# zhuker/lamejs

Hardware: NVIDIA H100
Metric: encoded audio seconds/sec (44.1kHz stereo 128kbps CBR) (higher is better)
Workload: dtype f64

## Files before the change

include/mp3b200.h:

```cpp
#ifndef MP3B200_H
#define MP3B200_H
#include <stdint.h>

#ifdef __cplusplus
extern "C" {
#endif

#define MP3B200_OK 0
#define MP3B200_ERR_CONFIG (-1)
#define MP3B200_ERR_BUFFER (-1)
#define MP3B200_ERR_HANDLE (-3)
#define MP3B200_ERR_CUDA (-100)

typedef struct mp3b200_encoder mp3b200_encoder;

int mp3b200_set_device(int device);

int mp3b200_create(int channels, int samplerate, int kbps, mp3b200_encoder** out);

#define MP3B200_RESAMPLE 1
int mp3b200_create_ex(int channels, int samplerate, int kbps, int flags, mp3b200_encoder** out);
int mp3b200_out_samplerate(int channels, int samplerate, int kbps);

int mp3b200_encode(mp3b200_encoder* h, const int16_t* left, const int16_t* right, int nsamples, uint8_t* out, int cap);

int mp3b200_flush(mp3b200_encoder* h, uint8_t* out, int cap);

void mp3b200_destroy(mp3b200_encoder* h);

int mp3b200_encode_batch(mp3b200_encoder* const* handles, const int16_t* const* left, const int16_t* const* right,
                         const int* nsamples, uint8_t* const* out, const int* cap, int nstreams, int* out_bytes);
int mp3b200_flush_batch(mp3b200_encoder* const* handles, uint8_t* const* out, const int* cap, int nstreams, int* out_bytes);

int mp3b200_encode_device(mp3b200_encoder* h, const int16_t* d_left, const int16_t* d_right, int nsamples, uint8_t* out, int cap);
int mp3b200_encode_device_f32(mp3b200_encoder* h, const float* d_left, const float* d_right, int nsamples, uint8_t* out, int cap);
int mp3b200_encode_batch_device(mp3b200_encoder* const* handles, const int16_t* const* d_left, const int16_t* const* d_right,
                                const int* nsamples, uint8_t* const* out, const int* cap, int nstreams, int* out_bytes);
int mp3b200_encode_batch_device_f32(mp3b200_encoder* const* handles, const float* const* d_left, const float* const* d_right,
                                    const int* nsamples, uint8_t* const* out, const int* cap, int nstreams, int* out_bytes);
int mp3b200_encoder_device(const mp3b200_encoder* h);

int mp3b200_export_state(mp3b200_encoder* h, void* buf, int cap);
int mp3b200_import_state(mp3b200_encoder* h, const void* buf, int len);
int mp3b200_seek(mp3b200_encoder* h, int64_t frame, const int16_t* left_hist, const int16_t* right_hist, int nhist);


int64_t mp3b200_stream_bytes(int channels, int samplerate, int kbps, int64_t nsamples);
int64_t mp3b200_stream_bytes_ex(int channels, int samplerate, int kbps, int flags, int64_t nsamples);
int64_t mp3b200_stream_frames(int64_t nsamples);
int64_t mp3b200_stream_frames_cfg(int channels, int samplerate, int kbps, int64_t nsamples);
int mp3b200_granules_per_frame(int channels, int samplerate, int kbps);
int64_t mp3b200_stream_frames_ex(int channels, int samplerate, int kbps, int flags, int64_t nsamples);
int mp3b200_granules_per_frame_ex(int channels, int samplerate, int kbps, int flags);

int mp3b200_encode_streams(int channels, int samplerate, int kbps, int nstreams, const int16_t* const* left,
                           const int16_t* const* right, const int64_t* nsamples, uint8_t* const* out,
                           const int64_t* cap, int64_t* out_bytes);
int mp3b200_encode_streams_ex(int channels, int samplerate, int kbps, int flags, int nstreams, const int16_t* const* left,
                              const int16_t* const* right, const int64_t* nsamples, uint8_t* const* out,
                              const int64_t* cap, int64_t* out_bytes);

int mp3b200_encode_streams_device(int channels, int samplerate, int kbps, int nstreams, const int16_t* d_pcm,
                                  const int64_t* pcm_off, const int64_t* nsamples, uint8_t* d_out,
                                  const int64_t* out_off, float* timings_ms);
int mp3b200_encode_streams_device_ex(int channels, int samplerate, int kbps, int flags, int nstreams, const int16_t* d_pcm,
                                     const int64_t* pcm_off, const int64_t* nsamples, uint8_t* d_out,
                                     const int64_t* out_off, float* timings_ms);

int mp3b200_set_write_vbr_tag(mp3b200_encoder* h, int on);
int mp3b200_get_lametag_frame(mp3b200_encoder* h, uint8_t* buf, int cap);
int mp3b200_music_crc(mp3b200_encoder* h);
int64_t mp3b200_bytes_written(mp3b200_encoder* h);
int mp3b200_lametag_size(int channels, int samplerate, int kbps);
int mp3b200_lametag_size_ex(int channels, int samplerate, int kbps, int flags);
int mp3b200_lametag_build(int channels, int samplerate, int kbps, int64_t nframes, int64_t music_bytes, int music_crc,
                          int encoder_padding, uint8_t* buf, int cap);
int mp3b200_encode_streams_tagged(int channels, int samplerate, int kbps, int nstreams, const int16_t* const* left,
                                  const int16_t* const* right, const int64_t* nsamples, uint8_t* const* out,
                                  const int64_t* cap, int64_t* out_bytes);

#define MP3B200_REPLAYGAIN 2
int mp3b200_encode_streams_tagged_ex(int channels, int samplerate, int kbps, int flags, int nstreams, const int16_t* const* left,
                                     const int16_t* const* right, const int64_t* nsamples, uint8_t* const* out,
                                     const int64_t* cap, int64_t* out_bytes, double* title_db, double* album_db);
int mp3b200_encode_streams_tagged_device(int channels, int samplerate, int kbps, int flags, int nstreams, const int16_t* d_pcm,
                                         const int64_t* pcm_off, const int64_t* nsamples, uint8_t* d_out, const int64_t* out_off,
                                         int64_t* out_bytes, double* title_db, double* album_db);
int mp3b200_encode_streams_tagged_device_f32(int channels, int samplerate, int kbps, int flags, int nstreams, const float* d_pcm,
                                             const int64_t* pcm_off, const int64_t* nsamples, uint8_t* d_out, const int64_t* out_off,
                                             int64_t* out_bytes, double* title_db, double* album_db);
int mp3b200_set_find_replay_gain(mp3b200_encoder* h, int on);
int mp3b200_get_replay_gain(mp3b200_encoder* h, double* title_db, int* radio_gain);
int mp3b200_album_gain(mp3b200_encoder* const* handles, int n, double* album_db);
int mp3b200_lametag_build_ex(int channels, int samplerate, int kbps, int flags, int64_t nframes, int64_t music_bytes, int music_crc,
                             int encoder_padding, int radio_gain, uint8_t* buf, int cap);
int mp3b200_replaygain_streams(int channels, int samplerate, int kbps, int flags, int nstreams, const int16_t* const* left,
                               const int16_t* const* right, const int64_t* nsamples, double* title_db, double* album_db);
int mp3b200_replaygain_streams_f32(int channels, int samplerate, int kbps, int flags, int nstreams, const float* const* left,
                                   const float* const* right, const int64_t* nsamples, double* title_db, double* album_db);
int mp3b200_replaygain_streams_device(int channels, int samplerate, int kbps, int flags, int nstreams, const int16_t* d_pcm,
                                      const int64_t* pcm_off, const int64_t* nsamples, double* title_db, double* album_db);
int mp3b200_replaygain_streams_device_f32(int channels, int samplerate, int kbps, int flags, int nstreams, const float* d_pcm,
                                          const int64_t* pcm_off, const int64_t* nsamples, double* title_db, double* album_db);
int mp3b200_finish_tags_device(int channels, int samplerate, int kbps, int flags, int nstreams, uint8_t* d_files,
                               const int64_t* file_off, const int64_t* nsamples, const double* title_db, int64_t* file_bytes);
int mp3b200_debug_replaygain(int channels, int samplerate, int kbps, int flags, const int16_t* left, const int16_t* right,
                             int64_t nsamples, double* win_sums, int32_t* win_idx, int64_t nwin_cap, int32_t* hist,
                             double* title_db, int32_t* stats);

typedef struct mp3b200_vbr_tag_data {
  int32_t h_id, samprate, flags, frames, bytes, vbr_scale, headersize, enc_delay, enc_padding;
  uint8_t toc[100];
} mp3b200_vbr_tag_data;
int mp3b200_put_vbr_tag(mp3b200_encoder* h, uint8_t* stream, int64_t len);
int mp3b200_get_vbr_tag(const uint8_t* frame, int64_t len, mp3b200_vbr_tag_data* out);
int mp3b200_crc16_combine(int crc_a, int crc_b, int64_t len_b);

#define MP3B200_ID3_ADD_V2 2
#define MP3B200_ID3_V1_ONLY 4
#define MP3B200_ID3_V2_ONLY 8
#define MP3B200_ID3_SPACE_V1 16
#define MP3B200_ID3_PAD_V2 32
typedef struct mp3b200_id3tag {
  const char *title, *artist, *album, *year, *comment, *track, *genre;
  int flags, padding;
  int64_t num_samples;
  int samplerate;
} mp3b200_id3tag;
int mp3b200_id3v2_tag(const mp3b200_id3tag* t, uint8_t* buf, int cap);
int mp3b200_id3v1_tag(const mp3b200_id3tag* t, uint8_t* buf, int cap);
const char* mp3b200_id3_genre_name(int index);

int mp3b200_debug_music_crc(const uint8_t* d_buf, const int64_t* off, const int64_t* len, int nranges, uint32_t* crc, float* ms);

typedef struct mp3b200_wav_header { int64_t data_offset, data_len; int32_t channels; uint32_t sample_rate; } mp3b200_wav_header;
int mp3b200_wav_read_header(const uint8_t* data, int64_t len, mp3b200_wav_header* out);

int mp3b200_debug_stages(int channels, int samplerate, int kbps, const int16_t* left, const int16_t* right,
                         int64_t nsamples, const int32_t* force_blocktype, float* xr, int32_t* blocktype,
                         float* en_l, float* thm_l, float* en_s, float* thm_s, double* ath_adjust,
                         int32_t* l3_enc, int32_t* ginfo, uint8_t* bytes_out, int64_t bytes_cap);

typedef struct mp3b200_debug_taps {
  int32_t size, channels, samplerate, kbps;
  const int16_t *left, *right;
  int64_t nsamples;
  const int32_t* force_blocktype;
  float* xr; int32_t* blocktype; float *en_l, *thm_l, *en_s, *thm_s; double* ath_adjust;
  int32_t *l3_enc, *ginfo; uint8_t* bytes_out; int64_t bytes_cap;
  int32_t *scalefac, *subblock_gain; float* xmin; int32_t* max_nonzero_coeff; double* xrpow_max;
  int32_t *scfsi, *old_value, *cur_step;
  int32_t flags;
} mp3b200_debug_taps;
int mp3b200_debug_stages_ex(const mp3b200_debug_taps* t);

int mp3b200_debug_resample(int channels, int samplerate, int kbps, const int16_t* left, const int16_t* right, int64_t nsamples,
                           float* y, int64_t ny);

int mp3b200_encode_f32(mp3b200_encoder* h, const float* left, const float* right, int nsamples, uint8_t* out, int cap);
int mp3b200_encode_batch_f32(mp3b200_encoder* const* handles, const float* const* left, const float* const* right,
                             const int* nsamples, uint8_t* const* out, const int* cap, int nstreams, int* out_bytes);
int mp3b200_seek_f32(mp3b200_encoder* h, int64_t frame, const float* left_hist, const float* right_hist, int nhist);
int mp3b200_encode_streams_f32(int channels, int samplerate, int kbps, int flags, int nstreams, const float* const* left,
                               const float* const* right, const int64_t* nsamples, uint8_t* const* out,
                               const int64_t* cap, int64_t* out_bytes);
int mp3b200_encode_streams_tagged_f32(int channels, int samplerate, int kbps, int flags, int nstreams, const float* const* left,
                                      const float* const* right, const int64_t* nsamples, uint8_t* const* out,
                                      const int64_t* cap, int64_t* out_bytes, double* title_db, double* album_db);
int mp3b200_encode_streams_device_f32(int channels, int samplerate, int kbps, int flags, int nstreams, const float* d_pcm,
                                      const int64_t* pcm_off, const int64_t* nsamples, uint8_t* d_out,
                                      const int64_t* out_off, float* timings_ms);
int mp3b200_debug_stages_f32(const mp3b200_debug_taps* t, const float* left, const float* right);
int mp3b200_debug_resample_f32(int channels, int samplerate, int kbps, const float* left, const float* right, int64_t nsamples,
                               float* y, int64_t ny);
int mp3b200_debug_replaygain_f32(int channels, int samplerate, int kbps, int flags, const float* left, const float* right,
                                 int64_t nsamples, double* win_sums, int32_t* win_idx, int64_t nwin_cap, int32_t* hist,
                                 double* title_db, int32_t* stats);

#define MP3B200_SESSION_SLOTS 4
typedef struct mp3b200_session mp3b200_session;
int mp3b200_session_create(void* cuda_stream, mp3b200_session** out);
int mp3b200_session_destroy(mp3b200_session* s);
int mp3b200_encode_streams_async(mp3b200_session* s, int channels, int samplerate, int kbps, int flags, int nstreams,
                                 const int16_t* d_pcm, const int64_t* pcm_off, const int64_t* nsamples, uint8_t* d_out,
                                 const int64_t* out_off, int32_t* d_status);
int mp3b200_encode_streams_async_f32(mp3b200_session* s, int channels, int samplerate, int kbps, int flags, int nstreams,
                                     const float* d_pcm, const int64_t* pcm_off, const int64_t* nsamples, uint8_t* d_out,
                                     const int64_t* out_off, int32_t* d_status);
int mp3b200_check_status(const int32_t* status);

int mp3b200_encode_streams_tagged_async(mp3b200_session* s, int channels, int samplerate, int kbps, int flags, int nstreams,
                                        const int16_t* d_pcm, const int64_t* pcm_off, const int64_t* nsamples, uint8_t* d_out,
                                        const int64_t* out_off, int64_t* out_bytes, double* d_gain, int32_t* d_status);
int mp3b200_encode_streams_tagged_async_f32(mp3b200_session* s, int channels, int samplerate, int kbps, int flags, int nstreams,
                                            const float* d_pcm, const int64_t* pcm_off, const int64_t* nsamples, uint8_t* d_out,
                                            const int64_t* out_off, int64_t* out_bytes, double* d_gain, int32_t* d_status);

int mp3b200_session_encode_batch(mp3b200_session* s, mp3b200_encoder* const* handles, const int16_t* const* d_left,
                                 const int16_t* const* d_right, const int* nsamples, int n, uint8_t* d_out, const int64_t* out_off,
                                 int* out_bytes, int32_t* d_status);
int mp3b200_session_encode_batch_f32(mp3b200_session* s, mp3b200_encoder* const* handles, const float* const* d_left,
                                     const float* const* d_right, const int* nsamples, int n, uint8_t* d_out, const int64_t* out_off,
                                     int* out_bytes, int32_t* d_status);
int mp3b200_session_flush_batch(mp3b200_session* s, mp3b200_encoder* const* handles, int n, uint8_t* d_out, const int64_t* out_off,
                                int* out_bytes, int32_t* d_status);
int mp3b200_encode_bytes(const mp3b200_encoder* h, int nsamples);
int mp3b200_encode_bytes_schedule(int channels, int samplerate, int kbps, int flags, int write_vbr_tag, const int* nsamples, int n,
                                  int* out_bytes);
int mp3b200_session_release(mp3b200_session* s, mp3b200_encoder* const* handles, int n);
int64_t mp3b200_session_tail_capacity(int channels, int samplerate, int kbps, int flags);

int mp3b200_session_encode_batch_tagged(mp3b200_session* s, mp3b200_encoder* const* handles, const int16_t* const* d_left,
                                        const int16_t* const* d_right, const int* nsamples, int n, uint8_t* d_out, const int64_t* out_off,
                                        int* out_bytes, int32_t* d_status);
int mp3b200_session_encode_batch_tagged_f32(mp3b200_session* s, mp3b200_encoder* const* handles, const float* const* d_left,
                                            const float* const* d_right, const int* nsamples, int n, uint8_t* d_out,
                                            const int64_t* out_off, int* out_bytes, int32_t* d_status);
int mp3b200_session_flush_batch_tagged(mp3b200_session* s, mp3b200_encoder* const* handles, int n, uint8_t* d_out,
                                       const int64_t* out_off, int* out_bytes, int32_t* d_status);
int mp3b200_session_lametag_frames(mp3b200_session* s, mp3b200_encoder* const* handles, int n, uint8_t* d_out, const int64_t* out_off,
                                   int* out_bytes, int32_t* d_status);
int mp3b200_session_album_gain(mp3b200_session* s, mp3b200_encoder* const* handles, int n, double* d_album, int32_t* d_status);
int64_t mp3b200_session_graph_instantiations(mp3b200_session* s);

const char* mp3b200_last_error(void);
int64_t mp3b200_launch_count(void);

#ifdef __cplusplus
}
#endif
#endif
```

lamejs_b200/__init__.py:

```python
from .encoder import Mp3Encoder, WavHeader, id3v1_tag, id3v2_tag, ID3_ADD_V2, ID3_V1_ONLY, ID3_V2_ONLY, ID3_SPACE_V1, ID3_PAD_V2, lametag_size, lametag_build, get_vbr_tag, crc16_combine, encode_streams_tagged, debug_music_crc, encode_batch, flush_batch, encode_streams, encode_streams_device, encode_streams_device_tagged, debug_stages, debug_resample, lib, stream_bytes, stream_frames, granules_per_frame, out_samplerate, RESAMPLE, Mp3B200Error
from .encoder import REPLAYGAIN, GAIN_NOT_ENOUGH_SAMPLES, radio_gain, lametag_build_ex, debug_replaygain, encode_streams_replaygain, album_gain
from .encoder import DOMAIN_SITES, debug_domain_hits
from .encoder import EncodeSession, check_status
from .encoder import replay_gain_streams, replay_gain_streams_device, finish_tags_device
```

lamejs_b200/csrc/k_psy.cuh:

```cuda
#ifndef MP3B200_K_PSY_CUH
#define MP3B200_K_PSY_CUH
#include "mp3_device.cuh"
#include "mp3_tables.h"

#ifndef PSY_THREADS
#define PSY_THREADS 128
#endif
#define MASK_THREADS 128

struct PsyUnit {
  double ecb_s[3][MP3_CBANDS];
  float eb_s[3][MP3_CBANDS];
  float eb_l[MP3_CBANDS];
  float peaks[9];
  float loudness;
  unsigned char mask_idx[MP3_CBANDS];
  unsigned char attack[4];
  unsigned char pad_;
};
struct PsyRatioDev { float en_l[22], thm_l[22], en_s[13][3], thm_s[13][3]; };

__constant__ unsigned char c_fft_rv[128];
__device__ double c_tab[9];
__device__ double c_table1[25];
__device__ double c_table2[10];
__device__ double c_table3[14];
__constant__ double c_fircoef[10];

static int psy_upload_constants() {
  static const double tab[9] = {1.0, 0.79433, 0.63096, 0.63096, 0.63096, 0.63096, 0.63096, 0.25119, 0.11749};
  static const double r1[25] = {3.3246, 3.23837, 3.15437, 3.00412, 2.86103, 2.65407, 2.46209, 2.284, 2.11879, 1.96552, 1.82335,
    1.69146, 1.56911, 1.46658, 1.37074, 1.31036, 1.25264, 1.20648, 1.16203, 1.12765, 1.09428, 1.0659, 1.03826, 1.01895, 1};
  static const double r2[10] = {1.33352, 1.35879, 1.38454, 1.39497, 1.40548, 1.3537, 1.30382, 1.22321, 1.14758, 1};
  static const double r3[14] = {2.35364, 2.29259, 2.23313, 2.12675, 2.02545, 1.87894, 1.74303, 1.61695, 1.49999, 1.39148,
    1.29083, 1.19746, 1.11084, 1.03826};
  static const double fir_half[10] = {-8.65163e-18, -0.00851586, -6.74764e-18, 0.0209036, -3.36639e-17, -0.0438162,
    -1.54175e-17, 0.0931738, -5.52212e-17, -0.313819};
  double t1[25], t2[10], t3[14], fir[10];
  for (int i = 0; i < 25; i++) t1[i] = r1[i] * r1[i];
  for (int i = 0; i < 10; i++) t2[i] = r2[i] * r2[i];
  for (int i = 0; i < 14; i++) t3[i] = r3[i] * r3[i];
  for (int i = 0; i < 10; i++) fir[i] = fir_half[i] * 2;
  if (cudaMemcpyToSymbol(c_fft_rv, MP3_FFT_RV, 128) != cudaSuccess) return -100;
  if (cudaMemcpyToSymbol(c_tab, tab, sizeof tab) != cudaSuccess) return -100;
  if (cudaMemcpyToSymbol(c_table1, t1, sizeof t1) != cudaSuccess) return -100;
  if (cudaMemcpyToSymbol(c_table2, t2, sizeof t2) != cudaSuccess) return -100;
  if (cudaMemcpyToSymbol(c_table3, t3, sizeof t3) != cudaSuccess) return -100;
  if (cudaMemcpyToSymbol(c_fircoef, fir, sizeof fir) != cudaSuccess) return -100;
  return 0;
}

struct f32w {
  float v;
  __device__ __forceinline__ operator double() const {
#ifdef PSY_ALU_WIDEN
    const unsigned u = __float_as_uint(v);
    const unsigned hi = (u & 0x7fffffffu) ? ((u & 0x80000000u) | (((u >> 3) & 0x0fffffffu) + 0x38000000u)) : u;
    return __hiloint2double((int)hi, (int)(u << 29));
#else
    return (double)v;
  }
  __device__ __forceinline__ f32w& operator=(double d) { v = (float)d; return *this; }
};
#endif

#define FHT_PAD(i) ((i) + ((i) >> 4))
__device__ __forceinline__ void fht_task(f32w* fz, int stage, int task, const double* __restrict__ tw, const int* tw_off) {
  const int k1 = 4 << (2 * stage);
  const int kx = k1 >> 1, k2 = k1 << 1, k3 = k2 + k1, k4 = k2 << 1;
  const int g = task >> (2 * stage + 1), i = task & (kx - 1);
  if (i == 0) {
    {
      const int fi = g * k4;
      double f0, f1, f2, f3;
      f1 = fz[FHT_PAD(fi + 0)] - fz[FHT_PAD(fi + k1)];
      f0 = fz[FHT_PAD(fi + 0)] + fz[FHT_PAD(fi + k1)];
      f3 = fz[FHT_PAD(fi + k2)] - fz[FHT_PAD(fi + k3)];
      f2 = fz[FHT_PAD(fi + k2)] + fz[FHT_PAD(fi + k3)];
      fz[FHT_PAD(fi + k2)] = f0 - f2;
      fz[FHT_PAD(fi + 0)] = f0 + f2;
      fz[FHT_PAD(fi + k3)] = f1 - f3;
      fz[FHT_PAD(fi + k1)] = f1 + f3;
    }
    {
      const int gi = g * k4 + kx;
      double f0, f1, f2, f3;
      f1 = fz[FHT_PAD(gi + 0)] - fz[FHT_PAD(gi + k1)];
      f0 = fz[FHT_PAD(gi + 0)] + fz[FHT_PAD(gi + k1)];
      f3 = (SQRT2_D * fz[FHT_PAD(gi + k3)]);
      f2 = (SQRT2_D * fz[FHT_PAD(gi + k2)]);
      fz[FHT_PAD(gi + k2)] = f0 - f2;
      fz[FHT_PAD(gi + 0)] = f0 + f2;
      fz[FHT_PAD(gi + k3)] = f1 - f3;
      fz[FHT_PAD(gi + k1)] = f1 + f3;
    }
    return;
  }
  const double* e = tw + 4 * (tw_off[stage] + i);
  const double c1 = e[0], s1 = e[1], c2 = e[2], s2 = e[3];
  const int fi = g * k4 + i, gi = g * k4 + k1 - i;
  double a, b, g0, f0, f1, g1, f2, g2, f3, g3;
  b = s2 * fz[FHT_PAD(fi + k1)] - c2 * fz[FHT_PAD(gi + k1)];
  a = c2 * fz[FHT_PAD(fi + k1)] + s2 * fz[FHT_PAD(gi + k1)];
  f1 = fz[FHT_PAD(fi + 0)] - a;
  f0 = fz[FHT_PAD(fi + 0)] + a;
  g1 = fz[FHT_PAD(gi + 0)] - b;
  g0 = fz[FHT_PAD(gi + 0)] + b;
  b = s2 * fz[FHT_PAD(fi + k3)] - c2 * fz[FHT_PAD(gi + k3)];
  a = c2 * fz[FHT_PAD(fi + k3)] + s2 * fz[FHT_PAD(gi + k3)];
  f3 = fz[FHT_PAD(fi + k2)] - a;
  f2 = fz[FHT_PAD(fi + k2)] + a;
  g3 = fz[FHT_PAD(gi + k2)] - b;
  g2 = fz[FHT_PAD(gi + k2)] + b;
  b = s1 * f2 - c1 * g3;
  a = c1 * f2 + s1 * g3;
  fz[FHT_PAD(fi + k2)] = f0 - a;
  fz[FHT_PAD(fi + 0)] = f0 + a;
  fz[FHT_PAD(gi + k3)] = g1 - b;
  fz[FHT_PAD(gi + k1)] = g1 + b;
  b = c1 * g2 - s1 * f3;
  a = s1 * g2 + c1 * f3;
  fz[FHT_PAD(gi + k2)] = g0 - a;
  fz[FHT_PAD(gi + 0)] = g0 + a;
  fz[FHT_PAD(fi + k3)] = f1 - b;
  fz[FHT_PAD(fi + k1)] = f1 + b;
}

__device__ __forceinline__ size_t psy_row(const StreamDesc& sd, int z, int u) { return (size_t)sd.unit_base + z + u + 1; }

#ifndef PSY_MIN_BLOCKS
#define PSY_MIN_BLOCKS 12
#endif
template <bool F32_PCM>
__global__ void __launch_bounds__(PSY_THREADS, PSY_MIN_BLOCKS)
k_psy_analysis(const Mp3Tables* __restrict__ T, const StreamDesc* __restrict__ streams, PsyUnit* __restrict__ out,
               int chunk, int nchunks, int u_base) {
  const int z = blockIdx.z;
  const StreamDesc& sd = streams[z];
  const int u = (int)blockIdx.x + u_base;
  if (u >= T->mode_gr * sd.nframes) return;
  const int ch = blockIdx.y;
  const int nch = T->nch;
  const long long c = (long long)T->mode_gr * sd.frame0 + u;
  if (nchunks > 1) {
    const long long n = sd.pcm_end - sd.pcm_base;
    long long last = 576 * c - 224 + 1023 - sd.pcm_base;
    if (last > n - 1) last = n - 1;
    int mine = 0;
    while (mine < nchunks - 1 && last >= n * (mine + 1) / nchunks) mine++;
    if (mine != chunk) return;
  }
  PsyUnit* o = out + psy_row(sd, z, u) * nch + ch;
  const int tid = threadIdx.x;

  if (c < 0) {
    for (int i = tid; i < 3 * MP3_CBANDS; i += PSY_THREADS) { (&o->ecb_s[0][0])[i] = 1.0; (&o->eb_s[0][0])[i] = 0.0f; }
    if (tid < MP3_CBANDS) { o->eb_l[tid] = 0.0f; o->mask_idx[tid] = 0; }
    if (tid < 9) o->peaks[tid] = 10.0f;
    if (tid == 0) o->loudness = 0.0f;
    if (tid < 4) o->attack[tid] = 0;
    return;
  }

  __shared__ __align__(16) unsigned char s_u[sizeof(double) * 1024];
  double* const xs = reinterpret_cast<double*>(s_u);
  f32s* const fe = reinterpret_cast<f32s*>(s_u);
  f32s (*const fes)[129] = reinterpret_cast<f32s (*)[129]>(s_u + 2064);
  f32s* const s_max = reinterpret_cast<f32s*>(s_u + 2064 + 1552);
  f32s* const s_avg = s_max + MP3_CBANDS;
  f32s (*const s_ebs)[MP3_CBANDS] = reinterpret_cast<f32s (*)[MP3_CBANDS]>(s_avg + MP3_CBANDS);
  static_assert(2064 + 1552 + 2 * 4 * MP3_CBANDS + 3 * 4 * MP3_CBANDS <= (int)sizeof(s_u), "energies must fit the PCM span");
  constexpr int PROD_HI_OFF = 2064 + 1552 + 2 * 4 * MP3_CBANDS + 3 * 4 * MP3_CBANDS;
  static_assert(PROD_HI_OFF % 8 == 0 && PROD_HI_OFF + 256 * 8 <= (int)sizeof(s_u), "second half of the loudness terms");
  double* const prod_hi = reinterpret_cast<double*>(s_u + PROD_HI_OFF);
  __shared__ f32w wl[1024 + 64];
  __shared__ f32w wsh[3][256 + 16];
  __shared__ __align__(8) f32s hp[576];
  double* const prod_lo = reinterpret_cast<double*>(hp);
  static_assert(sizeof(f32s) * 576 >= 256 * 8, "first half of the loudness terms");
  __shared__ int s_peak[9];
  if (tid < 9) s_peak[tid] = __float_as_int(1.0f);

  const int scale_applied = T->scale_applied;
  const double scale = T->scale;
  const long long x0 = 576 * c - 224;
  {
    using Sample = pcm_sample_t<F32_PCM>;
    const Sample* __restrict__ pbuf = static_cast<const Sample*>(sd.pcm[ch]);
    const long long pbase = sd.pcm_base, pend = sd.pcm_end;
    constexpr int NB = (1024 + PSY_THREADS - 1) / PSY_THREADS;
    Sample v[NB];
#pragma unroll
    for (int k = 0; k < NB; k++) {
      const int j = tid + k * PSY_THREADS;
      const long long i = x0 + j;
      v[k] = (j < 1024 && i >= 0 && i < pend) ? __ldg(&pbuf[i - pbase]) : (Sample)0;
    }
#pragma unroll
    for (int k = 0; k < NB; k++) {
      const int j = tid + k * PSY_THREADS;
      if (j < 1024) xs[j] = pcm_value(v[k], scale_applied, scale);
    }
  }
  __syncthreads();

  for (int i = tid; i < 576; i += PSY_THREADS) {
    const double* fb = xs + 397 + i;
    double sum1 = fb[10], sum2 = 0.0;
#pragma unroll
    for (int j = 0; j < 9; j += 2) {
      sum1 += c_fircoef[j] * (fb[j] + fb[21 - j]);
      sum2 += c_fircoef[j + 1] * (fb[j + 1] + fb[21 - j - 1]);
    }
    hp[i] = sum1 + sum2;
  }
  for (int vt = tid; vt < 128 + 96; vt += PSY_THREADS) {
  if (vt < 128) {
    const int jj = vt, i = c_fft_rv[jj], x = 4 * jj;
    const float* w = T->fft_window;
    double f0, f1, f2, f3, wv;
    f0 = (double)w[i] * (double)xs[i];
    wv = (double)w[i + 0x200] * (double)xs[i + 0x200];
    f1 = f0 - wv; f0 = f0 + wv;
    f2 = (double)w[i + 0x100] * (double)xs[i + 0x100];
    wv = (double)w[i + 0x300] * (double)xs[i + 0x300];
    f3 = f2 - wv; f2 = f2 + wv;
    wl[FHT_PAD(x + 0)] = f0 + f2; wl[FHT_PAD(x + 2)] = f0 - f2; wl[FHT_PAD(x + 1)] = f1 + f3; wl[FHT_PAD(x + 3)] = f1 - f3;
    f0 = (double)w[i + 0x001] * (double)xs[i + 0x001];
    wv = (double)w[i + 0x201] * (double)xs[i + 0x201];
    f1 = f0 - wv; f0 = f0 + wv;
    f2 = (double)w[i + 0x101] * (double)xs[i + 0x101];
    wv = (double)w[i + 0x301] * (double)xs[i + 0x301];
    f3 = f2 - wv; f2 = f2 + wv;
    wl[FHT_PAD(x + 512 + 0)] = f0 + f2; wl[FHT_PAD(x + 512 + 2)] = f0 - f2; wl[FHT_PAD(x + 512 + 1)] = f1 + f3; wl[FHT_PAD(x + 512 + 3)] = f1 - f3;
  } else {
    const int q = vt - 128, b = q >> 5, j = q & 31;
    const int i = c_fft_rv[j << 2], x = 4 * j, k = 192 * (b + 1);
    const float* w = T->fft_window_s;
    const double* bx = xs + i + k;
    double f0, f1, f2, f3, wv;
    f0 = (double)w[i] * (double)bx[0];
    wv = (double)w[0x7f - i] * (double)bx[0x80];
    f1 = f0 - wv; f0 = f0 + wv;
    f2 = (double)w[i + 0x40] * (double)bx[0x40];
    wv = (double)w[0x3f - i] * (double)bx[0xc0];
    f3 = f2 - wv; f2 = f2 + wv;
    wsh[b][FHT_PAD(x + 0)] = f0 + f2; wsh[b][FHT_PAD(x + 2)] = f0 - f2; wsh[b][FHT_PAD(x + 1)] = f1 + f3; wsh[b][FHT_PAD(x + 3)] = f1 - f3;
    f0 = (double)w[i + 0x01] * (double)bx[0x01];
    wv = (double)w[0x7e - i] * (double)bx[0x81];
    f1 = f0 - wv; f0 = f0 + wv;
    f2 = (double)w[i + 0x41] * (double)bx[0x41];
    wv = (double)w[0x3e - i] * (double)bx[0xc1];
    f3 = f2 - wv; f2 = f2 + wv;
    wsh[b][FHT_PAD(x + 128 + 0)] = f0 + f2; wsh[b][FHT_PAD(x + 128 + 2)] = f0 - f2; wsh[b][FHT_PAD(x + 128 + 1)] = f1 + f3; wsh[b][FHT_PAD(x + 128 + 3)] = f1 - f3;
  }
  }
  __syncthreads();

  for (int i = tid; i < 576; i += PSY_THREADS) atomicMax(&s_peak[i >> 6], __float_as_int(fabsf(hp[i].v)));
#pragma unroll
  for (int stage = 0; stage < 4; stage++) {
    const int nt = 128 + (stage < 3 ? 96 : 0);
    for (int t = tid; t < nt; t += PSY_THREADS) {
      if (t < 128) fht_task(wl, stage, t, T->tw, T->tw_off);
      else fht_task(wsh[(t - 128) >> 5], stage, (t - 128) & 31, T->tw, T->tw_off);
    }
    __syncthreads();
  }

  for (int j = tid; j < 512; j += PSY_THREADS) {
    const double re = wl[FHT_PAD(512 - j)], im = wl[FHT_PAD(512 + j)];
    f32s e; e = (re * re + im * im) * 0.5;
    fe[512 - j] = (double)e;
    const int k = 512 - j;
    if (k < 512) { const double p = (double)e * (double)T->eql_w[k]; if (k < 256) prod_lo[k] = p; else prod_hi[k - 256] = p; }
  }
  if (tid == 0) { f32s t0; t0 = (double)wl[0]; t0 *= (double)t0; fe[0] = (double)t0; prod_lo[0] = (double)t0 * (double)T->eql_w[0]; }
  for (int t = tid; t < 3 * 128; t += PSY_THREADS) {
    const int b = t >> 7, j = t & 127;
    const double re = wsh[b][FHT_PAD(128 - j)], im = wsh[b][FHT_PAD(128 + j)];
    fes[b][128 - j] = (re * re + im * im) * 0.5;
  }
  if (tid < 3) { f32s t0; t0 = (double)wsh[tid][0]; t0 *= (double)t0; fes[tid][0] = (double)t0; }
  __syncthreads();

  const int npl = T->npart_l, nps = T->npart_s;
  for (int vt = tid; vt < 256; vt += PSY_THREADS) {
  if (vt < npl) {
    double ebb = 0, m = 0;
    const int l0 = T->line0_l[vt], l1 = T->line0_l[vt + 1];
    for (int j = l0; j < l1; j++) { const double el = fe[j]; ebb += el; if (m < el) m = el; }
    o->eb_l[vt] = (float)ebb;
    s_max[vt] = m;
    s_avg[vt] = ebb * (double)T->rnumlines_l[vt];
  } else if (vt >= 64 && vt < 64 + 3 * 64) {
    const int q = vt - 64, sb = q >> 6, b = q & 63;
    if (b < nps) {
      double ebb = 0;
      const int l0 = T->line0_s[b], l1 = T->line0_s[b + 1];
      for (int j = l0; j < l1; j++) ebb += (double)fes[sb][j];
      s_ebs[sb][b] = ebb;
      o->eb_s[sb][b] = (float)ebb;
    }
  }
  }
  double loud = 0.0;
  if (tid == PSY_THREADS - 1) {
#pragma unroll 8
    for (int i = 0; i < 256; ++i) loud += prod_lo[i];
  }
  if (tid < 9) o->peaks[tid] = __int_as_float(s_peak[tid]);
  __syncthreads();

  for (int vt = tid; vt < 256; vt += PSY_THREADS) {
  if (vt < npl) {
    const int b = vt;
    const int lo = b > 0 ? b - 1 : b, hi = b < npl - 1 ? b + 1 : b;
    double a = 0; double m = 0; int lines = 0;
    for (int q = lo; q <= hi; q++) {
      if (q == lo) { a = (double)s_avg[q]; m = (double)s_max[q]; }
      else { a = a + (double)s_avg[q]; if (m < (double)s_max[q]) m = (double)s_max[q]; }
      lines += T->numlines_l[q];
    }
    int k = 0;
    if (a > 0.0) {
      const double cnt = (double)(hi - lo + 1);
      a = 20.0 * (m * cnt - a) / (a * (lines - 1));
      k = js_trunc<DOM_TRUNC_MASK_IDX>(a);
      if (k > 8) k = 8;
    }
    o->mask_idx[b] = (unsigned char)k;
  } else if (vt >= 64 && vt < 64 + 3 * 64) {
    const int q = vt - 64, sb = q >> 6, b = q & 63;
    if (b < nps) {
      int kk = T->s3lo_s[b];
      int j = T->s3off_s[b];
      double ecb = (double)T->s3_ss[j++] * (double)s_ebs[sb][kk];
      ++kk;
      while (kk <= T->s3hi_s[b]) { ecb += (double)T->s3_ss[j] * (double)s_ebs[sb][kk]; ++j; ++kk; }
      o->ecb_s[sb][b] = ecb;
    }
  }
  }
  if (tid == PSY_THREADS - 1) {
#pragma unroll 8
    for (int i = 0; i < 256; ++i) loud += prod_hi[i];
    loud *= (1. / (14752. * 14752.) / 512);
    o->loudness = (float)loud;
  }
}

struct ScanIn { unsigned attack4; float loudness; };

__global__ void k_attack_prepass(const Mp3Tables* __restrict__ T, const StreamDesc* __restrict__ streams, PsyUnit* __restrict__ psy,
                                 ScanIn* __restrict__ sin) {
  const int z = blockIdx.z;
  const StreamDesc& sd = streams[z];
  const int u = blockIdx.x * blockDim.x + threadIdx.x;
  if (u >= T->mode_gr * sd.nframes) return;
  const int nch = T->nch;
  const double thr = T->attack_threshold;
  for (int ch = 0; ch < nch; ch++) {
    PsyUnit* cur = psy + psy_row(sd, z, u) * nch + ch;
    const PsyUnit* prev = psy + psy_row(sd, z, u - 1) * nch + ch;
    f32s en_subshort[12], attack_intensity[12];
    double en_short[4] = {0, 0, 0, 0};
    int a[4] = {0, 0, 0, 0};
    for (int i = 0; i < 3; i++) {
      en_subshort[i] = (double)prev->peaks[i + 6];
      attack_intensity[i] = (double)en_subshort[i] / (double)prev->peaks[i + 4];
      en_short[0] += (double)en_subshort[i];
    }
    for (int i = 0; i < 9; i++) {
      double p = (double)cur->peaks[i];
      en_subshort[i + 3] = p;
      if (i % 3 == 0) en_short[1 + i / 3] += p;
      if (p > (double)en_subshort[i + 3 - 2]) p = p / (double)en_subshort[i + 3 - 2];
      else if ((double)en_subshort[i + 3 - 2] > p * 10.0) p = (double)en_subshort[i + 3 - 2] / (p * 10.0);
      else p = 0.0;
      attack_intensity[i + 3] = p;
    }
    for (int i = 0; i < 12; i += 3)
      if ((double)attack_intensity[i] > thr) a[i / 3] = 1;
    for (int i = 1; i < 4; i++) {
      double ratio;
      if (en_short[i - 1] > en_short[i]) ratio = en_short[i - 1] / en_short[i];
      else ratio = en_short[i] / en_short[i - 1];
      if (ratio < 1.7) { a[i] = 0; if (i == 1) a[0] = 0; }
    }
    for (int i = 0; i < 4; i++) cur->attack[i] = (unsigned char)a[i];
    ScanIn si;
    si.attack4 = (unsigned)a[0] | ((unsigned)a[1] << 8) | ((unsigned)a[2] << 16) | ((unsigned)a[3] << 24);
    si.loudness = cur->loudness;
    sin[psy_row(sd, z, u) * nch + ch] = si;
    if (u == 0) { si.attack4 = 0; si.loudness = prev->loudness; sin[psy_row(sd, z, -1) * nch + ch] = si; }
  }
}

#define SCAN_FRAMES 16
#define SCAN_THREADS 1024
#ifndef SCAN_GUESS_LA
#define SCAN_GUESS_LA 0
#endif
#ifndef SCAN_GUESS_BT
#define SCAN_GUESS_BT BT_NORM
#endif
#ifndef SCAN_GUESS_ATH
#define SCAN_GUESS_ATH 1.0
#endif
struct ScanChunk { int fsm_in, fsm_out, dirty_fsm, dirty_ath; double ath_in[2], ath_out[2]; };

__device__ __forceinline__ int fsm_pack(int la0, int la1, int o0, int o1) { return la0 | (la1 << 2) | (o0 << 4) | (o1 << 6); }

__device__ void scan_fsm_chunk(const Mp3Tables* T, const StreamDesc& sd, int z, const ScanIn* sin, signed char* bt_final,
                               signed char* bt_prev, int f0, int f1, ScanChunk* ck) {
  const int nch = T->nch, coupled = T->coupled_short_blocks;
  int la[2] = {ck->fsm_in & 3, (ck->fsm_in >> 2) & 3};
  int old[2] = {(ck->fsm_in >> 4) & 3, (ck->fsm_in >> 6) & 3};
  const int G = T->mode_gr;
  for (int u = G * f0; u < G * f1; u++) {
    int uselong[2] = {1, 1};
    for (int ch = 0; ch < nch; ch++) {
      const unsigned av = sin[psy_row(sd, z, u) * nch + ch].attack4;
      int a0 = av & 0xff, a1 = (av >> 8) & 0xff, a2 = (av >> 16) & 0xff, a3 = (av >> 24) & 0xff;
      if (a0 != 0 && la[ch] != 0) a0 = 0;
      if (la[ch] == 3 || (a0 + a1 + a2 + a3) != 0) {
        uselong[ch] = 0;
        if (a1 != 0 && a0 != 0) a1 = 0;
        if (a2 != 0 && a1 != 0) a2 = 0;
        if (a3 != 0 && a2 != 0) a3 = 0;
      }
      la[ch] = a2;
    }
    if (coupled && !(uselong[0] != 0 && uselong[1] != 0)) uselong[0] = uselong[1] = 0;
    const size_t row = (size_t)(sd.unit_base + u) * 2;
    for (int ch = 0; ch < nch; ch++) {
      bt_prev[row + ch] = (signed char)old[ch];
      int bt = BT_NORM;
      if (uselong[ch] != 0) {
        if (old[ch] == BT_SHORT) bt = BT_STOP;
      } else {
        bt = BT_SHORT;
        if (old[ch] == BT_NORM) old[ch] = BT_START;
        if (old[ch] == BT_STOP) old[ch] = BT_SHORT;
      }
      bt_final[row + ch] = (signed char)old[ch];
      old[ch] = bt;
    }
  }
  ck->fsm_out = fsm_pack(la[0], la[1], old[0], old[1]);
}

__device__ void scan_ath_chunk(const Mp3Tables* T, const StreamDesc& sd, int z, const ScanIn* sin, double* ath_psy,
                               double* ath_q, int f0, int f1, ScanChunk* ck) {
  const int nch = T->nch;
  double adjust = ck->ath_in[0], limit = ck->ath_in[1];
  const double sens = T->aa_sensitivity_p;
  const int G = T->mode_gr;
  for (int f = f0; f < f1; f++) {
    ath_psy[sd.frame_base + f] = adjust;
    const ScanIn* r0 = sin + psy_row(sd, z, G * f - 1) * nch;
    double max_pow = (double)r0[0].loudness;
    if (nch == 2) max_pow += (double)r0[1].loudness;
    else max_pow += max_pow;
    if (G == 2) {
      const ScanIn* r1 = sin + psy_row(sd, z, G * f) * nch;
      double gr2_max = (double)r1[0].loudness;
      if (nch == 2) gr2_max += (double)r1[1].loudness;
      else gr2_max += gr2_max;
      max_pow = js_dmax(max_pow, gr2_max);
    }
    max_pow *= 0.5;
    max_pow *= sens;
    if (max_pow > 0.03125) {
      if (adjust >= 1.0) adjust = 1.0;
      else if (adjust < limit) adjust = limit;
      limit = 1.0;
    } else {
      const double adj_lim_new = 31.98 * max_pow + 0.000625;
      if (adjust >= adj_lim_new) {
        adjust *= adj_lim_new * 0.075 + 0.925;
        if (adjust < adj_lim_new) adjust = adj_lim_new;
      } else {
        if (limit >= adj_lim_new) adjust = adj_lim_new;
        else if (adjust < limit) adjust = limit;
      }
      limit = adj_lim_new;
    }
    ath_q[sd.frame_base + f] = adjust;
  }
  ck->ath_out[0] = adjust; ck->ath_out[1] = limit;
}

__global__ void __launch_bounds__(SCAN_THREADS)
k_stream_scan(const Mp3Tables* __restrict__ T, StreamDesc* __restrict__ streams, int nstreams,
              const ScanIn* __restrict__ sin, signed char* __restrict__ bt_final,
              signed char* __restrict__ bt_prev, double* __restrict__ ath_psy, double* __restrict__ ath_q,
              ScanChunk* __restrict__ scratch) {
  asm volatile("griddepcontrol.launch_dependents;" ::: "memory");
  const int z = blockIdx.x;
  if (z >= nstreams) return;
  const StreamDesc& sd = streams[z];
  const int nchunks = (sd.nframes + SCAN_FRAMES - 1) / SCAN_FRAMES;
  ScanChunk* ck = scratch + sd.scan_base;
  const int tid = threadIdx.x;
  for (int c = tid; c < nchunks; c += SCAN_THREADS) {
    ck[c].fsm_in = c == 0 ? fsm_pack(sd.last_attacks[0], sd.last_attacks[1], sd.blocktype_old[0], sd.blocktype_old[1])
                          : fsm_pack(SCAN_GUESS_LA, SCAN_GUESS_LA, SCAN_GUESS_BT, SCAN_GUESS_BT);
    ck[c].ath_in[0] = c == 0 ? sd.ath_adjust : SCAN_GUESS_ATH;
    ck[c].ath_in[1] = c == 0 ? sd.ath_adjust_limit : SCAN_GUESS_ATH;
    ck[c].dirty_fsm = ck[c].dirty_ath = 1;
  }
  for (;;) {
    for (int c = tid; c < nchunks; c += SCAN_THREADS) {
      const int f0 = c * SCAN_FRAMES, f1 = min(sd.nframes, f0 + SCAN_FRAMES);
      if (ck[c].dirty_fsm) scan_fsm_chunk(T, sd, z, sin, bt_final, bt_prev, f0, f1, &ck[c]);
      if (ck[c].dirty_ath) scan_ath_chunk(T, sd, z, sin, ath_psy, ath_q, f0, f1, &ck[c]);
    }
    __syncthreads();
    int any = 0;
    for (int c = tid; c < nchunks; c += SCAN_THREADS) {
      ck[c].dirty_fsm = ck[c].dirty_ath = 0;
      if (c == 0) continue;
      if (ck[c].fsm_in != ck[c - 1].fsm_out) { ck[c].fsm_in = ck[c - 1].fsm_out; ck[c].dirty_fsm = 1; any = 1; }
      if (ck[c].ath_in[0] != ck[c - 1].ath_out[0] || ck[c].ath_in[1] != ck[c - 1].ath_out[1]) {
        ck[c].ath_in[0] = ck[c - 1].ath_out[0]; ck[c].ath_in[1] = ck[c - 1].ath_out[1]; ck[c].dirty_ath = 1; any = 1;
      }
    }
    if (!__syncthreads_or(any)) break;
  }
  if (tid == 0 && nchunks > 0) {
    const ScanChunk& l = ck[nchunks - 1];
    streams[z].last_attacks[0] = l.fsm_out & 3; streams[z].last_attacks[1] = (l.fsm_out >> 2) & 3;
    streams[z].blocktype_old[0] = (l.fsm_out >> 4) & 3; streams[z].blocktype_old[1] = (l.fsm_out >> 6) & 3;
    streams[z].ath_adjust = l.ath_out[0]; streams[z].ath_adjust_limit = l.ath_out[1];
  }
}

__device__ __noinline__ double psy_log10(double x) { return m3_log10(x); }
__device__ __forceinline__ int log10_times16_trunc(const Mp3Tables* T, double ratio) {
  if (!T->l16_ok) return js_trunc<DOM_TRUNC_LOG16>(psy_log10(ratio) * 16.0);
  DOMAIN_MISS(DOM_LOG16_TABLE, !(ratio >= 1.0 && ratio < 31.622776601683793));
  int i = 0;
#pragma unroll
  for (int k = 1; k <= 24; k++) i += ratio >= T->l16_thr[k] ? 1 : 0;
  return i;
}

__device__ __forceinline__ double mask_add_dev(double m1, double m2, int kk, int b, const Mp3Tables* T, double ath_adjust) {
  double ratio;
  if (m2 > m1) {
    if (m2 < (m1 * T->ma_max_i2)) ratio = m2 / m1;
    else return (m1 + m2);
  } else {
    if (m1 >= (m2 * T->ma_max_i2)) return (m1 + m2);
    ratio = m1 / m2;
  }
  m1 += m2;
  if ((b + 3) <= 3 + 3) {
    if (ratio >= T->ma_max_i1) return m1;
    const int i = log10_times16_trunc(T, ratio);
    return m1 * c_table2[i];
  }
  const int i = log10_times16_trunc(T, ratio);
  m2 = (double)T->ath_cb_l[kk] * ath_adjust;
  if (m1 < T->ma_max_m * m2) {
    if (m1 > m2) {
      double f = 1.0, r;
      if (i <= 13) f = c_table3[i];
      r = psy_log10(m1 / m2) * (10.0 / 15.0);
      return m1 * ((c_table1[i] - f) * r + f);
    }
    if (i > 13) return m1;
    return m1 * c_table3[i];
  }
  return m1 * c_table1[i];
}

__global__ void __launch_bounds__(MASK_THREADS)
k_psy_masking(const Mp3Tables* __restrict__ T, const StreamDesc* __restrict__ streams, const PsyUnit* __restrict__ psy,
              const signed char* __restrict__ bt_prev, const double* __restrict__ ath_psy, PsyRatioDev* __restrict__ ratio) {
  const int z = blockIdx.z;
  const StreamDesc& sd = streams[z];
  const int u = (int)blockIdx.x - 1;
  if (u >= T->mode_gr * sd.nframes) return;
  const int nch = T->nch;
  const long long c = (long long)T->mode_gr * sd.frame0 + u;
  const int tid = threadIdx.x, ch = tid >> 6, b = tid & 63;
  PsyRatioDev* out = ratio + psy_row(sd, z, u) * nch;
  if (u < 0) {
    if (c < 0) {
      const float big = (float)1e20;
      for (int i = tid; i < nch * 122; i += MASK_THREADS) (&out[0].en_l[0])[i] = big;
    }
    else if (sd.halo_in) {
      for (int i = tid; i < nch * 122; i += MASK_THREADS) (&out[0].en_l[0])[i] = sd.halo_in[i];
    }
    return;
  }
  __shared__ f32s s_thr[2][MP3_CBANDS + 2], s_eb[2][MP3_CBANDS + 2];
  __shared__ f32s s_thr_s[2][3][MP3_CBANDS + 2];
  __shared__ PsyRatioDev s_out[2];
  const int npl = T->npart_l, nps = T->npart_s;
  const PsyUnit* pu = (ch < nch) ? psy + psy_row(sd, z, u) * nch + ch : nullptr;
  const PsyUnit* pp = (ch < nch) ? psy + psy_row(sd, z, u - 1) * nch + ch : nullptr;
  const double ath_adjust = ath_psy[sd.frame_base + u / T->mode_gr];

  if (ch < nch) {
    if (b < npl) {
      int kk = T->s3lo_l[b];
      int k = T->s3off_l[b];
      double eb2 = (double)pu->eb_l[kk] * c_tab[pu->mask_idx[kk]];
      double ecb = (double)T->s3_ll[k++] * eb2;
      while (++kk <= T->s3hi_l[b]) {
        eb2 = (double)pu->eb_l[kk] * c_tab[pu->mask_idx[kk]];
        ecb = mask_add_dev(ecb, (double)T->s3_ll[k++] * eb2, kk, kk - b, T, ath_adjust);
      }
      ecb *= 0.158489319246111;
      s_thr[ch][b] = ecb;
      s_eb[ch][b] = (double)pu->eb_l[b];
    } else { s_thr[ch][b] = 0.0; s_eb[ch][b] = 0.0; }
    const int prev_short = bt_prev[(size_t)(sd.unit_base + u) * 2 + ch] == BT_SHORT;
    for (int sb = 0; sb < 3; sb++) {
      if (b < nps) {
        const double ecb = pu->ecb_s[sb][b];
        const float nb1 = sb >= 1 ? (float)pu->ecb_s[sb - 1][b] : (float)pp->ecb_s[2][b];
        const float nb2 = sb == 2 ? (float)pu->ecb_s[0][b] : (sb == 1 ? (float)pp->ecb_s[2][b] : (float)pp->ecb_s[1][b]);
        f32s t;
        t = js_dmin(ecb, 2 * (double)nb1);
        if (prev_short) { const double x = 16 * (double)nb2, y = (double)t; t = js_dmin(x, y); }
        s_thr_s[ch][sb][b] = (double)t;
      } else s_thr_s[ch][sb][b] = 0.0;
    }
  }
  __syncthreads();

  if (ch < nch && b < 22) {
    const int sbi = b;
    f32s* en = reinterpret_cast<f32s*>(s_out[ch].en_l);
    f32s* thm = reinterpret_cast<f32s*>(s_out[ch].thm_l);
    const int init = T->conv_l.init[sbi];
    if (init == -2) { en[sbi] = 0.0; thm[sbi] = 0.0; }
    else {
      double enn = 0.0, thmm = 0.0;
      if (init >= 0) {
        const double w_next = 1.0 - (double)T->bo_l_weight[sbi - 1];
        enn = w_next * (double)s_eb[ch][init];
        thmm = w_next * (double)s_thr[ch][init];
      }
      const int p1 = T->conv_l.end[sbi];
      for (int p = T->conv_l.start[sbi]; p < p1; p++) { enn += (double)s_eb[ch][p]; thmm += (double)s_thr[ch][p]; }
      en[sbi] = enn; thm[sbi] = thmm;
      const int bd = T->conv_l.bound[sbi];
      if (bd >= 0) {
        const double w_curr = (double)T->bo_l_weight[sbi];
        en[sbi] += w_curr * (double)s_eb[ch][bd];
        thm[sbi] += w_curr * (double)s_thr[ch][bd];
      }
    }
  } else if (ch < nch && b >= 22 && b < 22 + 39) {
    const int q = b - 22, sbi = q / 3, sblock = q - 3 * sbi;
    f32s(*en)[3] = reinterpret_cast<f32s(*)[3]>(s_out[ch].en_s);
    f32s(*thm)[3] = reinterpret_cast<f32s(*)[3]>(s_out[ch].thm_s);
    const int init = T->conv_s.init[sbi];
    if (init == -2) { en[sbi][sblock] = 0.0; thm[sbi][sblock] = 0.0; }
    else {
      double enn = 0.0, thmm = 0.0;
      if (init >= 0) {
        const double w_next = 1.0 - (double)T->bo_s_weight[sbi - 1];
        enn = w_next * (double)pu->eb_s[sblock][init];
        thmm = w_next * (double)s_thr_s[ch][sblock][init];
      }
      const int p1 = T->conv_s.end[sbi];
      for (int p = T->conv_s.start[sbi]; p < p1; p++) { enn += (double)pu->eb_s[sblock][p]; thmm += (double)s_thr_s[ch][sblock][p]; }
      en[sbi][sblock] = enn; thm[sbi][sblock] = thmm;
      const int bd = T->conv_s.bound[sbi];
      if (bd >= 0) {
        const double w_curr = (double)T->bo_s_weight[sbi];
        en[sbi][sblock] += w_curr * (double)pu->eb_s[sblock][bd];
        thm[sbi][sblock] += w_curr * (double)s_thr_s[ch][sblock][bd];
      }
    }
    const double e3 = (double)pu->peaks[sblock * 3 + 0], e4 = (double)pu->peaks[sblock * 3 + 1], e5 = (double)pu->peaks[sblock * 3 + 2];
    double t = (double)thm[sbi][sblock];
    t *= 0.8;
    const double enn2 = e3 + e4 + e5;
    if (e5 * 6 < enn2) { t *= 0.5; if (e4 * 6 < enn2) t *= 0.5; }
    thm[sbi][sblock] = t;
  }
  __syncthreads();
  if (nch == 2 && T->interch_ratio > 0.0 && tid < 22 + 39) {
    const double r = T->interch_ratio;
    f32s* t0 = reinterpret_cast<f32s*>(tid < 22 ? &s_out[0].thm_l[tid] : &s_out[0].thm_s[0][0] + (tid - 22));
    f32s* t1 = reinterpret_cast<f32s*>(tid < 22 ? &s_out[1].thm_l[tid] : &s_out[1].thm_s[0][0] + (tid - 22));
    const double l = (double)*t0, rr = (double)*t1;
    *t0 += rr * r;
    *t1 += l * r;
  }
  __syncthreads();
  for (int i = tid; i < nch * 122; i += MASK_THREADS) (&out[0].en_l[0])[i] = (&s_out[0].en_l[0])[i];
  if (sd.halo_out && u == T->mode_gr * sd.nframes - 1)
    for (int i = tid; i < nch * 122; i += MASK_THREADS) sd.halo_out[i] = (&s_out[0].en_l[0])[i];
}

#endif
```

lamejs_b200/csrc/mp3_encoder.cu:

```cuda
#include <cuda_runtime.h>
#include <math.h>
#include <stdio.h>
#include <algorithm>
#include <array>
#include <stdlib.h>
#include <string.h>
#include <atomic>
#include <map>
#include <mutex>
#include <string>
#include <tuple>
#include <vector>

#include "../../include/mp3b200.h"
#include "mp3_config.h"
#include "mp3_device.cuh"
#include "mp3_tables.h"
#include "k_filterbank.cuh"
#include "k_psy.cuh"
#include "k_quant.cuh"
#include "k_tag.cuh"
#include "k_resample.cuh"
#include "k_replaygain.cuh"
#include "k_stage.cuh"
#include "k_handle.cuh"
#include "mp3_tag.h"

namespace {

thread_local std::string g_err;
std::mutex g_mu;
int g_device = 0;
std::atomic<long long> g_launches{0};
enum { MP3_MAX_DEVICES = 64 };
bool g_consts_ready[MP3_MAX_DEVICES] = {};
bool g_fb_attr_done[MP3_MAX_DEVICES][2] = {};

#define CK(call)                                                                                  \
  do {                                                                                            \
    cudaError_t e_ = (call);                                                                      \
    if (e_ != cudaSuccess) {                                                                      \
      char b_[512];                                                                               \
      snprintf(b_, sizeof b_, "%s:%d %s -> %s", __FILE__, __LINE__, #call, cudaGetErrorString(e_)); \
      g_err = b_;                                                                                 \
      return MP3B200_ERR_CUDA;                                                                    \
    }                                                                                             \
  } while (0)

struct Config {
  Mp3Tables host;
  Mp3Resample rs;
  Mp3TagParams tag;
  bool encodable;
  Mp3Tables* dev[MP3_MAX_DEVICES];
};
std::map<std::tuple<int, int, int, int>, Config*> g_configs;

Config* find_config(int ch, int sr, int kbps, int flags) {
  if (flags & ~MP3B200_RESAMPLE) { g_err = "unknown flags"; return nullptr; }
  if (flags && mp3_out_samplerate(ch, sr, kbps) == sr) flags = 0;
  const auto key = std::make_tuple(ch, sr, kbps, flags);
  auto it = g_configs.find(key);
  if (it == g_configs.end()) {
    Config* c = new Config();
    if (mp3_build_config(ch, sr, kbps, flags, &c->host, &c->rs, &c->tag) == 0) c->encodable = c->rs.ratio <= RS_MAX_RATIO;
    else { delete c; c = nullptr; }
    it = g_configs.emplace(key, c).first;
  }
  if (!it->second) g_err = "unsupported configuration";
  return it->second;
}

const Config* host_config(int ch, int sr, int kbps, int flags) {
  std::lock_guard<std::mutex> lk(g_mu);
  return find_config(ch, sr, kbps, flags);
}

const Config* encodable_config(int ch, int sr, int kbps, int flags) {
  const Config* c = host_config(ch, sr, kbps, flags);
  return c && c->encodable ? c : nullptr;
}

int ensure_device(int dev) {
  int n = 0;
  cudaError_t e = cudaGetDeviceCount(&n);
  if (e != cudaSuccess || n <= 0) { g_err = "no CUDA device available (libmp3b200 has no CPU fallback)"; return MP3B200_ERR_CUDA; }
  if (dev < 0 || dev >= n || dev >= MP3_MAX_DEVICES) { g_err = "invalid CUDA device"; return MP3B200_ERR_CUDA; }
  CK(cudaSetDevice(dev));
  if (!g_consts_ready[dev]) {
    CK(cudaMemcpyToSymbol(c_enwindow, MP3_ENWINDOW, sizeof(double) * 285));
    CK(cudaMemcpyToSymbol(c_mdct_win, MP3_MDCT_WIN, sizeof(double) * 144));
    CK(cudaMemcpyToSymbol(c_sb_order, MP3_SB_ORDER, sizeof(int) * 32));
    CK(cudaMemcpyToSymbol(c_rg_yule, RG_YULE, sizeof RG_YULE));
    CK(cudaMemcpyToSymbol(c_rg_butter, RG_BUTTER, sizeof RG_BUTTER));
    int rc = psy_upload_constants();
    if (rc) return rc;
    rc = quant_upload_constants();
    if (rc) return rc;
    g_consts_ready[dev] = true;
  }
  return 0;
}

struct FifoFlush { long long frames, zeros; int end_padding; };
struct LameFifo {
  static constexpr long long ENC_POST_DELAY = 576 + 1152;
  long long framesize, mf_size = 576 - 48, mf_samples_to_encode = ENC_POST_DELAY;
  int ratio = 1;
  long long in_fed = 0;
  std::vector<long long>* pieces = nullptr;
  explicit LameFifo(int mode_gr, int r = 1) : framesize(576LL * mode_gr), ratio(r) {}
  long long outputs(long long p) const {
    if (ratio == 1) return p;
    return p > MP3_RS_HALF ? (p - MP3_RS_HALF + ratio - 1) / ratio : 0;
  }
  long long feed(long long n) {
    if (n <= 0) return 0;
    const long long k = outputs(in_fed + n) - outputs(in_fed);
    in_fed += n;
    if (pieces)
      for (long long i = 0; i < k; i += framesize) pieces->push_back(k - i < framesize ? k - i : framesize);
    const long long need = framesize + 752;
    const long long frames = mf_size + k >= need ? (mf_size + k - need) / framesize + 1 : 0;
    if (mf_samples_to_encode < 1) mf_samples_to_encode = ENC_POST_DELAY;
    mf_size += k - frames * framesize;
    mf_samples_to_encode += k - frames * framesize;
    return frames;
  }
  FifoFlush flush() {
    FifoFlush r = {0, 0, 0};
    if (mf_samples_to_encode < 1) return r;
    double samples_to_encode = (double)(mf_samples_to_encode - 1152);
    if (ratio > 1) samples_to_encode += 16. / ratio;
    double end_padding = framesize - fmod(samples_to_encode, (double)framesize);
    if (end_padding < 576) end_padding += framesize;
    r.end_padding = (int)end_padding;
    double frames_left = (samples_to_encode + end_padding) / framesize;
    while (frames_left > 0) {
      double bunch = (double)(framesize + 752 - mf_size);
      bunch *= ratio;
      if (bunch > 1152) bunch = 1152;
      if (bunch < 1) bunch = 1;
      const long long got = feed((long long)bunch);
      r.zeros += (long long)bunch;
      r.frames += got;
      frames_left -= got > 0 ? 1 : 0;
    }
    mf_samples_to_encode = 0;
    return r;
  }
};

long long frames_for(long long n, int mode_gr, int ratio = 1) {
  LameFifo f(mode_gr, ratio);
  const long long fed = f.feed(n);
  return fed + f.flush().frames;
}

long long bytes_of_frames(const Mp3Tables& g, long long k0, long long n) {
  return n * g.frame_bytes_nopad + pad_count(k0 + n - 1, g.frac_SpF, g.samplerate) - pad_count(k0 - 1, g.frac_SpF, g.samplerate);
}

template <class T, bool Pinned = false> struct Buf {
  T* p = nullptr;
  size_t cap = 0;
  void release() {
    if (Pinned) cudaFreeHost(p); else cudaFree(p);
    p = nullptr; cap = 0;
  }
  int fit(size_t n) {
    if (n <= cap) return 0;
    if (n < 2 * cap) n = 2 * cap;
    release();
    CK(Pinned ? cudaMallocHost((void**)&p, sizeof(T) * n) : cudaMalloc((void**)&p, sizeof(T) * n));
    cap = n;
    return 0;
  }
};

struct Workspace {
  Buf<StreamDesc> streams;
  Buf<signed char> bt_final;
  Buf<signed char> bt_prev;
  Buf<float> xr;
  Buf<float> slab;
  Buf<PsyUnit> psy;
  Buf<ScanIn> scan_in;
  Buf<PsyRatioDev> ratio;
  Buf<double> ath_psy;
  Buf<double> ath_q;
  Buf<QuantFrameState> qstate;
  Buf<GranuleInfoDev> ginfo;
  Buf<short> l3enc;
  Buf<float> xrq;
  Buf<float> xrpow;
  Buf<unsigned> neg;
  Buf<GcPrep> prep;
  Buf<int> dirty;
  Buf<int> counter;
  Buf<ScanChunk> scan;
  Buf<ResampleDesc> rs_desc;
  Buf<float> rs_y;
  Buf<StageDesc> st_desc;
  Buf<float> st_y;
  Buf<int> refusals;
  int fit(int S, int nch, long long U, long long F) {
    const size_t gc = (size_t)U * nch, rows = (size_t)(U + S) * nch, f = (size_t)F + 1;
    const bool failed = streams.fit(S) || bt_final.fit((size_t)U * 2 + 16) || bt_prev.fit((size_t)U * 2 + 16) ||
                        xr.fit(gc * 576) || slab.fit(rows * 576) || psy.fit(rows) || scan_in.fit(rows) || ratio.fit(rows) ||
                        ath_psy.fit(f) || ath_q.fit(f) || qstate.fit(f) || ginfo.fit(gc) || l3enc.fit(gc * 576) ||
                        xrq.fit(gc * 576) || xrpow.fit(gc * 576) || neg.fit(gc * 18) || prep.fit(gc) || dirty.fit(3 * f) ||
                        counter.fit(Q_NCOUNTERS) || scan.fit((size_t)(F / SCAN_FRAMES + S + 1));
    return failed ? MP3B200_ERR_CUDA : 0;
  }
  size_t generation() const {
    return streams.cap + qstate.cap + ginfo.cap + l3enc.cap + xrq.cap + xrpow.cap + neg.cap + prep.cap + dirty.cap + counter.cap +
           refusals.cap;
  }
  void release() {
    streams.release(); bt_final.release(); bt_prev.release(); xr.release(); slab.release(); psy.release(); scan_in.release();
    ratio.release(); ath_psy.release(); ath_q.release(); qstate.release(); ginfo.release(); l3enc.release(); xrq.release();
    xrpow.release(); neg.release(); prep.release(); dirty.release(); counter.release(); scan.release();
    rs_desc.release(); rs_y.release(); st_desc.release(); st_y.release(); refusals.release();
  }
};

struct PinnedArena { uint8_t* p = nullptr; size_t cap = 0, used = 0; };

enum { MP3_MAX_PCM_CHUNKS = 8 };
enum { MP3_MAX_LAUNCH_STREAMS = 65535 };
struct ThreadCtx {
  int device = -1;
  bool session = false;
  PinnedArena* arena = nullptr;
  cudaStream_t st = nullptr, up_st = nullptr, aux_st = nullptr;
  cudaEvent_t ev[8] = {}, evq[QE_COUNT] = {}, ev_in = nullptr, ev_fork = nullptr, ev_join = nullptr, ready[MP3_MAX_PCM_CHUNKS] = {};
  cudaEvent_t ev_rs[2] = {};
  Workspace ws;
  int evq_pred[QE_COUNT] = {};
  Buf<uint8_t> pcm;
  Buf<uint8_t> out;
  Buf<uint8_t, true> pin;
  Buf<long long> crc_ranges;
  Buf<unsigned> crc;
  Buf<uint8_t> tags;
  cudaStream_t rg_st = nullptr;
  cudaEvent_t ev_rg[3] = {};
  Buf<RgTitle> rg_titles;
  Buf<long long> rg_piece;
  Buf<double> rg_sum, rg_gain;
  Buf<RgState> rg_wstate, rg_cstart;
  Buf<RgEnd> rg_end_a, rg_end_b;
  Buf<RgCarry> rg_carry;
  Buf<int> rg_idx, rg_hist, rg_count;
  size_t rg_generation() const {
    return rg_titles.cap + rg_sum.cap + rg_wstate.cap + rg_cstart.cap + rg_end_a.cap + rg_end_b.cap + rg_count.cap + ws.refusals.cap;
  }
  void release() {
    if (device < 0) return;
    cudaSetDevice(device);
    ws.release(); pcm.release(); out.release(); pin.release(); crc_ranges.release(); crc.release(); tags.release();
    rg_titles.release(); rg_piece.release(); rg_sum.release(); rg_gain.release(); rg_wstate.release(); rg_cstart.release();
    rg_end_a.release(); rg_end_b.release(); rg_carry.release(); rg_idx.release(); rg_hist.release(); rg_count.release();
    for (auto& e : ev_rg) if (e) { cudaEventDestroy(e); e = nullptr; }
    if (rg_st) { cudaStreamDestroy(rg_st); rg_st = nullptr; }
    for (auto& e : ev) if (e) { cudaEventDestroy(e); e = nullptr; }
    for (auto& e : evq) if (e) { cudaEventDestroy(e); e = nullptr; }
    for (auto& e : ready) if (e) { cudaEventDestroy(e); e = nullptr; }
    for (auto& e : ev_rs) if (e) { cudaEventDestroy(e); e = nullptr; }
    if (ev_in) { cudaEventDestroy(ev_in); ev_in = nullptr; }
    if (ev_fork) { cudaEventDestroy(ev_fork); ev_fork = nullptr; }
    if (ev_join) { cudaEventDestroy(ev_join); ev_join = nullptr; }
    if (aux_st) { cudaStreamDestroy(aux_st); aux_st = nullptr; }
    if (st && !session) cudaStreamDestroy(st);
    st = nullptr;
    if (up_st) { cudaStreamDestroy(up_st); up_st = nullptr; }
    device = -1;
  }
  ~ThreadCtx() { release(); }
  int use(int dev) {
    CK(cudaSetDevice(dev));
    if (device == dev) return 0;
    release();
    CK(cudaStreamCreateWithFlags(&st, cudaStreamNonBlocking));
    return create(dev);
  }
  int bind(int dev, cudaStream_t s) {
    release();
    session = true;
    st = s;
    return create(dev);
  }
  int create(int dev) {
    CK(cudaStreamCreateWithFlags(&up_st, cudaStreamNonBlocking));
    CK(cudaStreamCreateWithFlags(&rg_st, cudaStreamNonBlocking));
    for (auto& e : ev_rg) CK(cudaEventCreate(&e));
    for (auto& e : ev) CK(cudaEventCreate(&e));
    for (auto& e : evq) CK(cudaEventCreate(&e));
    for (auto& e : ready) CK(cudaEventCreateWithFlags(&e, cudaEventDisableTiming));
    for (auto& e : ev_rs) CK(cudaEventCreate(&e));
    CK(cudaEventCreateWithFlags(&ev_in, cudaEventDisableTiming));
    CK(cudaEventCreateWithFlags(&ev_fork, cudaEventDisableTiming));
    CK(cudaEventCreateWithFlags(&ev_join, cudaEventDisableTiming));
    {
      int lo = 0, hi = 0;
      CK(cudaDeviceGetStreamPriorityRange(&lo, &hi));
      CK(cudaStreamCreateWithPriority(&aux_st, cudaStreamNonBlocking, hi));
    }
    device = dev;
    return 0;
  }
};
thread_local ThreadCtx t_ctx;

int config_on(int dev, int ch, int sr, int kbps, int flags, Config** out);

int get_config(int ch, int sr, int kbps, int flags, Config** out) {
  int dev = 0;
  {
    std::lock_guard<std::mutex> lk(g_mu);
    dev = g_device;
  }
  const int rc = config_on(dev, ch, sr, kbps, flags, out);
  return rc ? rc : t_ctx.use(dev);
}

int config_on(int dev, int ch, int sr, int kbps, int flags, Config** out) {
  if (flags & ~MP3B200_RESAMPLE) { g_err = "unknown flags"; return MP3B200_ERR_CONFIG; }
  {
    std::lock_guard<std::mutex> lk(g_mu);
    int rc = ensure_device(dev);
    if (rc) return rc;
    Config* c = find_config(ch, sr, kbps, flags);
    if (!c || !c->encodable) { g_err = "unsupported configuration"; return MP3B200_ERR_CONFIG; }
    if (!c->dev[dev]) {
      if (c->rs.ratio > 1)
        CK(cudaMemcpyToSymbol(c_rs_h, c->rs.h, sizeof(float) * MP3_RS_TAPS, sizeof(float) * MP3_RS_TAPS * c->rs.ratio));
      Mp3Tables* d = nullptr;
      CK(cudaMalloc(&d, sizeof(Mp3Tables)));
      CK(cudaMemcpy(d, &c->host, sizeof(Mp3Tables), cudaMemcpyHostToDevice));
      c->dev[dev] = d;
    }
    *out = c;
  }
  return 0;
}

bool debug_sync() { static int v = -1; if (v < 0) { const char* e = getenv("MP3B200_DEBUG_SYNC"); v = (e && e[0] == '1') ? 1 : 0; } return v == 1; }
#define DBG(name)                                                                           \
  do {                                                                                      \
    if (debug_sync()) {                                                                     \
      cudaError_t e_ = cudaStreamSynchronize(st);                                           \
      if (e_ == cudaSuccess) e_ = cudaGetLastError();                                       \
      if (e_ != cudaSuccess) { g_err = std::string(name) + ": " + cudaGetErrorString(e_); return MP3B200_ERR_CUDA; } \
    }                                                                                       \
  } while (0)

struct Timings { float psy = 0, scan = 0, mask = 0, fb = 0, q1 = 0, qn = 0, total = 0; int passes = 0;
                 float q_prepare = 0, q_search = 0, q_outer = 0, q_finish = 0, q_pack = 0, q_mid = 0; };

struct PcmArrival { int chunks = 1; cudaEvent_t* ready = nullptr; };

thread_local bool t_over_budget = false;

int refusal_error(int refused, int over_budget, int fault) {
  if (refused) { g_err = "non-finite input sample (or one beyond 2^40 once scaled)"; return MP3B200_ERR_CONFIG; }
  if (over_budget) { g_err = "frame over its bit budget (input too loud to encode)"; return MP3B200_ERR_CONFIG; }
  if (fault == RG_FAULT) { g_err = "ReplayGain repair did not converge"; return MP3B200_ERR_CUDA; }
  if (fault) { g_err = "quantizer stage failed: the fixed-point loop did not converge"; return MP3B200_ERR_CUDA; }
  return 0;
}

int check_refusals(ThreadCtx& c) {
  int r[2] = {0, 0};
  CK(cudaMemcpyAsync(r, c.ws.refusals.p, sizeof r, cudaMemcpyDeviceToHost, c.st));
  CK(cudaStreamSynchronize(c.st));
  if (!r[0] && r[1]) t_over_budget = true;
  return refusal_error(r[0], r[1], 0);
}

struct LaunchOpts {
  const int32_t* force_bt = nullptr;
  bool stop_after_mdct = false;
  const PcmArrival* arrival = nullptr;
  float* timings_ms = nullptr;
  bool sync = true;
  StreamDesc* committed = nullptr;
  struct RgJob* rg = nullptr;
  bool f32_in = false;
  struct LoopGraphs* loops = nullptr;
  const struct HandleCarry* carry = nullptr;
  int* rg_loop = nullptr;
  bool analyse_only = false;
};

struct HandleCarry { HandleRecord* const* recs; float* halo_scratch; };

enum { MP3_RG_GRAPHS = 32 };
struct LoopGraphs {
  cudaStream_t capture = nullptr;
  size_t generation = 0, rg_generation = 0;
  long long instantiated = 0;
  unsigned long long rg_tick = 0;
  std::map<std::tuple<const Config*, int, long long, int>, cudaGraphExec_t> exec;
  struct RgGraph { cudaGraphExec_t exec = nullptr; unsigned long long used = 0; };
  std::map<std::tuple<const Config*, bool, int, int, long long, const int*>, RgGraph> rg_exec;
  void clear_rg() { for (auto& e : rg_exec) cudaGraphExecDestroy(e.second.exec); rg_exec.clear(); }
  void clear() { for (auto& e : exec) cudaGraphExecDestroy(e.second); exec.clear(); }
};

int upload(ThreadCtx& c, void* dst, const void* src, size_t n, cudaStream_t on = nullptr) {
  if (c.arena) {
    PinnedArena& a = *c.arena;
    const size_t at = (a.used + 255) & ~(size_t)255;
    if (at + n > a.cap) { g_err = "descriptor staging overflow"; return MP3B200_ERR_CUDA; }
    memcpy(a.p + at, src, n);
    a.used = at + n;
    src = a.p + at;
  }
  CK(cudaMemcpyAsync(dst, src, n, cudaMemcpyHostToDevice, on ? on : c.st));
  return 0;
}

int wait_legacy(ThreadCtx& c) {
  if (c.session) return 0;
  CK(cudaEventRecord(c.ev_in, cudaStreamLegacy));
  CK(cudaStreamWaitEvent(c.st, c.ev_in, 0));
  return 0;
}

struct Rows { bool f32; int scale_applied; };
constexpr Rows SCALED_F32 = {true, 0};

int run_pipeline(ThreadCtx& c, Config* cfg, StreamDesc* h_streams, int S, uint8_t* d_out, const LaunchOpts& o,
                 const PcmArrival* arrival, Rows rows, Timings* tm) {
  cudaStream_t st = c.st;
  cudaEvent_t* ev = c.ev;
  Workspace& ws = c.ws;

  const Mp3Tables* const tab = cfg->dev[c.device];
  const int nch = cfg->host.nch;
  const bool f32_pcm = rows.f32;
  int max_frames = 0;
  long long total_frames = 0;
  int scan_rows = 0;
  int streams_with_frames = 0;
  for (int i = 0; i < S; i++) {
    StreamDesc& s = h_streams[i];
    max_frames = s.nframes > max_frames ? s.nframes : max_frames;
    total_frames += s.nframes;
    streams_with_frames += s.nframes > 0 ? 1 : 0;
    s.scan_base = scan_rows;
    scan_rows += (s.nframes + SCAN_FRAMES - 1) / SCAN_FRAMES;
  }
  int rc = wait_legacy(c);
  if (rc || (rc = upload(c, ws.streams.p, h_streams, sizeof(StreamDesc) * S))) return rc;
  if (o.carry) {
    k_handle_carry_in<<<(S + 127) / 128, 128, 0, st>>>(ws.streams.p, S, o.carry->recs, o.carry->halo_scratch);
    g_launches++;
    DBG("k_handle_carry_in");
  }
  CK(cudaEventRecord(ev[0], st));

  {
    const int nchunks = arrival ? arrival->chunks : 1;
    int u_lo[MP3_MAX_PCM_CHUNKS], u_hi[MP3_MAX_PCM_CHUNKS];
    const int G = cfg->host.mode_gr;
    for (int j = 0; j < nchunks; j++) { u_lo[j] = G * max_frames; u_hi[j] = -1; }
    if (nchunks > 1) {
      for (int s = 0; s < S; s++) {
        const StreamDesc& sd = h_streams[s];
        const long long n = sd.pcm_end - sd.pcm_base;
        for (int u = -1; u < G * sd.nframes; u++) {
          long long last = 576 * ((long long)G * sd.frame0 + u) - 224 + 1023 - sd.pcm_base;
          if (last > n - 1) last = n - 1;
          int mine = 0;
          while (mine < nchunks - 1 && last >= n * (mine + 1) / nchunks) mine++;
          if (u < u_lo[mine]) u_lo[mine] = u;
          if (u + 1 > u_hi[mine]) u_hi[mine] = u + 1;
        }
      }
    } else { u_lo[0] = -1; u_hi[0] = G * max_frames; }
    for (int j = 0; j < nchunks; j++) {
      if (arrival) CK(cudaStreamWaitEvent(st, arrival->ready[j], 0));
      if (u_hi[j] <= u_lo[j]) continue;
      dim3 gridj(u_hi[j] - u_lo[j], nch, S);
      if (f32_pcm) k_psy_analysis<true><<<gridj, PSY_THREADS, 0, st>>>(tab, ws.streams.p, ws.psy.p, j, nchunks, u_lo[j]);
      else k_psy_analysis<false><<<gridj, PSY_THREADS, 0, st>>>(tab, ws.streams.p, ws.psy.p, j, nchunks, u_lo[j]);
      g_launches++;
      DBG("k_psy_analysis");
    }
  }
  CK(cudaEventRecord(ev[1], st));
  {
    dim3 grid((cfg->host.mode_gr * max_frames + 127) / 128, 1, S);
    k_attack_prepass<<<grid, 128, 0, st>>>(tab, ws.streams.p, ws.psy.p, ws.scan_in.p);
    DBG("k_attack_prepass");
    k_stream_scan<<<S, SCAN_THREADS, 0, st>>>(tab, ws.streams.p, S, ws.scan_in.p, ws.bt_final.p, ws.bt_prev.p, ws.ath_psy.p, ws.ath_q.p, ws.scan.p);
    g_launches += 2;
    DBG("k_stream_scan");
    {
      const int G = cfg->host.mode_gr;
      const size_t smem = sizeof(double) * FB_PCM_WORDS + sizeof(float) * (FB_SLABS * 18 * FB_SLAB_STRIDE);
      void (*const k_fb)(const Mp3Tables*, const StreamDesc*, float*) = f32_pcm ? k_subband_analysis<true> : k_subband_analysis<false>;
      {
        std::lock_guard<std::mutex> lk(g_mu);
        if (!g_fb_attr_done[c.device][f32_pcm]) { CK(cudaFuncSetAttribute(k_fb, cudaFuncAttributeMaxDynamicSharedMemorySize, (int)smem)); g_fb_attr_done[c.device][f32_pcm] = true; }
      }
      cudaLaunchConfig_t lc = {};
      lc.gridDim = dim3((G * max_frames + 1 + FB_SLABS - 1) / FB_SLABS, nch, S);
      lc.blockDim = dim3(FB_THREADS); lc.dynamicSmemBytes = smem; lc.stream = st;
      cudaLaunchAttribute at[1];
      at[0].id = cudaLaunchAttributeProgrammaticStreamSerialization;
      at[0].val.programmaticStreamSerializationAllowed = 1;
      lc.attrs = at; lc.numAttrs = 1;
      CK(cudaLaunchKernelEx(&lc, k_fb, tab, (const StreamDesc*)ws.streams.p, ws.slab.p));
      g_launches++;
      DBG("k_subband_analysis");
    }
  }
  CK(cudaEventRecord(ev[2], st));
  if (o.force_bt) {
    const long long units = (long long)cfg->host.mode_gr * total_frames;
    std::vector<signed char> bt((size_t)units * 2, 0);
    for (long long u = 0; u < units; u++)
      for (int c = 0; c < nch; c++) bt[u * 2 + c] = (signed char)o.force_bt[u * nch + c];
    CK(cudaMemcpyAsync(ws.bt_final.p, bt.data(), bt.size(), cudaMemcpyHostToDevice, st));
    CK(cudaStreamSynchronize(st));
  }
  {
    dim3 grid(cfg->host.mode_gr * max_frames + 1, 1, S);
    k_psy_masking<<<grid, MASK_THREADS, 0, st>>>(tab, ws.streams.p, ws.psy.p, ws.bt_prev.p, ws.ath_psy.p, ws.ratio.p);
    g_launches++;
    DBG("k_psy_masking");
  }
  CK(cudaEventRecord(ev[3], st));
  {
    dim3 grid((cfg->host.mode_gr * max_frames + FB_G - 1) / FB_G, nch, S);
    k_mdct<<<grid, FB_G * 32, 0, st>>>(tab, ws.streams.p, ws.slab.p, ws.bt_final.p, ws.xr.p);
    g_launches++;
    DBG("k_mdct");
  }
  CK(cudaEventRecord(ev[4], st));
  int passes = 0;
  if (!o.stop_after_mdct) {
    QuantBuffers qb;
    qb.xr = ws.xr.p; qb.ratio = ws.ratio.p; qb.bt = ws.bt_final.p; qb.ath_q = ws.ath_q.p; qb.qs = ws.qstate.p; qb.ginfo = ws.ginfo.p;
    qb.l3enc = ws.l3enc.p; qb.xrq = ws.xrq.p; qb.xrpow = ws.xrpow.p; qb.neg = ws.neg.p; qb.prep = ws.prep.p; qb.list = ws.dirty.p; qb.counter = ws.counter.p;
    qb.over_budget = ws.refusals.p + 1;
    QuantLoop dloop;
    cudaGraphExec_t* cached = nullptr;
    if (o.loops) {
      LoopGraphs& lg = *o.loops;
      if (lg.generation != ws.generation()) { lg.clear(); lg.generation = ws.generation(); }
      cached = &lg.exec[std::make_tuple((const Config*)cfg, S, total_frames, max_frames)];
      dloop.capture = lg.capture; dloop.st = ws.refusals.p + 2; dloop.exec = *cached;
    }
    rc = quant_run(tab, cfg->host, ws.streams.p, S, streams_with_frames, max_frames, total_frames, qb, d_out, st, c.aux_st, c.ev_fork, c.ev_join, ev[5], c.evq, c.evq_pred, &passes, &g_launches,
                   o.loops ? &dloop : nullptr);
    if (cached) {
      if (!*cached && dloop.exec) o.loops->instantiated++;
      *cached = dloop.exec;
      if (!dloop.exec) o.loops->exec.erase(std::make_tuple((const Config*)cfg, S, total_frames, max_frames));
    }
    if (rc) { g_err = "quantizer stage failed: " + std::string(cudaGetErrorString(cudaGetLastError())); return rc; }
  } else {
    CK(cudaEventRecord(ev[5], st));
  }
  CK(cudaEventRecord(ev[6], st));
  if (!o.sync) return 0;
  CK(cudaStreamSynchronize(st));
  CK(cudaGetLastError());
  if (tm) {
    cudaEventElapsedTime(&tm->psy, ev[0], ev[1]);
    cudaEventElapsedTime(&tm->scan, ev[1], ev[2]);
    cudaEventElapsedTime(&tm->mask, ev[2], ev[3]);
    cudaEventElapsedTime(&tm->fb, ev[3], ev[4]);
    cudaEventElapsedTime(&tm->q1, ev[4], ev[5]);
    cudaEventElapsedTime(&tm->qn, ev[5], ev[6]);
    cudaEventElapsedTime(&tm->total, ev[0], ev[6]);
    tm->passes = passes;
    if (!o.stop_after_mdct && passes > 0) {
      auto span = [&](int slot) { float v = 0; const int p = c.evq_pred[slot]; if (p >= 0) cudaEventElapsedTime(&v, c.evq[p], c.evq[slot]); return v; };
      tm->q_prepare = span(QE_PREP);
      tm->q_search = span(QE_S0) + span(QE_S1);
      tm->q_outer = span(QE_O0) + span(QE_O1);
      tm->q_finish = span(QE_F0) + span(QE_F1);
      tm->q_pack = span(QE_PK);
      tm->q_mid = span(QE_MID);
    }
  }
  return 0;
}

void init_stream_state(StreamDesc& sd) {
  sd.ath_adjust = 0.01; sd.ath_adjust_limit = 1.0;
  sd.blocktype_old[0] = sd.blocktype_old[1] = BT_NORM;
  sd.last_attacks[0] = sd.last_attacks[1] = 0;
  sd.old_value[0] = sd.old_value[1] = 180;
  sd.current_step[0] = sd.current_step[1] = 4;
}

long long hist_base_at(int mode_gr, long long frame) {
  const long long b = 576LL * mode_gr * frame - 1104;
  return b > 0 ? b : 0;
}

int stage_streams(ThreadCtx& c, Config* cfg, StreamDesc* sds, int S) {
  const int nch = cfg->host.nch;
  Workspace& ws = c.ws;
  std::vector<StageDesc> d((size_t)S);
  long long tot = 0, max_n = 0;
  for (int i = 0; i < S; i++) {
    const long long n = sds[i].pcm_end > sds[i].pcm_base ? sds[i].pcm_end - sds[i].pcm_base : 0;
    for (int c = 0; c < 2; c++) d[i].x[c] = static_cast<const float*>(sds[i].pcm[c]);
    d[i].n = n;
    tot += n * nch;
    max_n = n > max_n ? n : max_n;
  }
  int rc = ws.st_desc.fit((size_t)S);
  if (rc) return rc;
  rc = ws.st_y.fit((size_t)tot + 1);
  if (rc) return rc;
  long long off = 0;
  for (int i = 0; i < S; i++) {
    d[i].y[0] = ws.st_y.p + off; d[i].y[1] = nch == 2 ? d[i].y[0] + d[i].n : d[i].y[0];
    off += d[i].n * nch;
    for (int c = 0; c < 2; c++) sds[i].pcm[c] = d[i].y[c];
  }
  cudaStream_t st = c.st;
  if ((rc = wait_legacy(c)) || (rc = upload(c, ws.st_desc.p, d.data(), sizeof(StageDesc) * S))) return rc;
  if (max_n > 0) {
    const long long per = (long long)STAGE_THREADS * STAGE_PER_THREAD;
    dim3 grid((unsigned)((max_n + per - 1) / per), nch, S);
    k_stage_f32<<<grid, STAGE_THREADS, 0, st>>>(ws.st_desc.p, cfg->host.scale_applied, cfg->host.scale, ws.refusals.p);
    g_launches++;
    DBG("k_stage_f32");
  }
  return 0;
}

int queue_resample(ThreadCtx& c, const Config* cfg, const ResampleDesc* rd, int S, long long max_ny, Rows in) {
  Workspace& ws = c.ws;
  cudaStream_t st = c.st;
  int rc = ws.rs_desc.fit((size_t)S);
  if (rc || (rc = upload(c, ws.rs_desc.p, rd, sizeof(ResampleDesc) * S))) return rc;
  CK(cudaEventRecord(c.ev_rs[0], st));
  if (max_ny > 0) {
    dim3 grid((unsigned)((max_ny + RS_THREADS - 1) / RS_THREADS), cfg->host.nch, S);
    if (in.f32) k_resample<float><<<grid, RS_THREADS, 0, st>>>(ws.rs_desc.p, cfg->rs.ratio, in.scale_applied, cfg->host.scale);
    else k_resample<int16_t><<<grid, RS_THREADS, 0, st>>>(ws.rs_desc.p, cfg->rs.ratio, in.scale_applied, cfg->host.scale);
    g_launches++;
    DBG("k_resample");
  }
  CK(cudaEventRecord(c.ev_rs[1], st));
  return 0;
}

int resample_streams(ThreadCtx& c, Config* cfg, StreamDesc* sds, int S, Rows in) {
  const int r = cfg->rs.ratio, nch = cfg->host.nch;
  Workspace& ws = c.ws;
  std::vector<ResampleDesc> rd((size_t)S);
  long long tot = 0, max_ny = 0;
  for (int i = 0; i < S; i++) {
    const StreamDesc& sd = sds[i];
    const long long yb = hist_base_at(cfg->host.mode_gr, sd.frame0);
    const long long xb = r * yb - MP3_RS_HALF > 0 ? r * yb - MP3_RS_HALF : 0;
    if (sd.pcm_base > xb) { g_err = "resampler input starts after the first sample it reads"; return MP3B200_ERR_HANDLE; }
    long long ye = (sd.pcm_end + MP3_RS_HALF - 1) / r + 1;
    if (sd.nframes == 0 || ye < yb) ye = yb;
    ResampleDesc& d = rd[i];
    d.x[0] = sd.pcm[0]; d.x[1] = sd.pcm[1]; d.x_base = sd.pcm_base; d.x_end = sd.pcm_end;
    d.y_base = yb; d.ny = ye - yb;
    tot += d.ny * nch;
    max_ny = d.ny > max_ny ? d.ny : max_ny;
  }
  int rc = ws.rs_y.fit((size_t)tot + 1);
  if (rc) return rc;
  long long off = 0;
  for (int i = 0; i < S; i++) {
    ResampleDesc& d = rd[i];
    d.y[0] = ws.rs_y.p + off; d.y[1] = nch == 2 ? d.y[0] + d.ny : d.y[0];
    off += d.ny * nch;
    for (int c = 0; c < 2; c++) sds[i].pcm[c] = d.y[c];
    sds[i].pcm_base = d.y_base; sds[i].pcm_end = d.y_base + d.ny;
  }
  if ((rc = wait_legacy(c))) return rc;
  return queue_resample(c, cfg, rd.data(), S, max_ny, in);
}

struct RgSpec {
  int stream = 0;
  std::vector<long long> pieces;
  long long t0 = 0, g0 = 0;
  RgCarry* carry = nullptr;
  int* hist = nullptr;
  int* hist_b = nullptr;
  int title_end = 1;
};
struct RgJob {
  std::vector<RgSpec> specs;
  std::vector<double> title_db;
  double album_db = 0;
  int passes = 0, reruns = 0;
  float ms = 0;
  bool want_windows = false;
  std::vector<double> win_sum;
  std::vector<int> win_idx;
  std::vector<int> hist0;
  long long chunk_rows = 0;
  int max_chunks = 0, max_win = 0, nwin0 = 0;
  RgParams prm;
};

int rg_req_index(int sr) {
  static const int rates[9] = {48000, 44100, 32000, 24000, 22050, 16000, 12000, 11025, 8000};
  for (int i = 0; i < 9; i++) if (rates[i] == sr) return i;
  return -1;
}

int rg_queue(ThreadCtx& c, Config* cfg, const StreamDesc* sds, RgJob& job, const PcmArrival* arrival, Rows rows) {
  const int sr = cfg->host.samplerate, W = (sr + 19) / 20, nch = cfg->host.nch, req = rg_req_index(sr);
  if (req < 0) { g_err = "no ReplayGain filter for this rate"; return MP3B200_ERR_CONFIG; }
  const int T = (int)job.specs.size();
  std::vector<RgTitle> t((size_t)T);
  long long npiece = 0, nwin = 0, nchunk = 0;
  for (const RgSpec& sp : job.specs) npiece += (long long)sp.pieces.size();
  int rc = 0;
  if ((rc = c.rg_piece.fit((size_t)npiece + 1)) || (rc = c.rg_carry.fit((size_t)T + 1)) || (rc = c.rg_hist.fit((size_t)(T + 1) * RG_HIST)))
    return rc;
  std::vector<long long> starts((size_t)npiece + 1);
  long long po = 0;
  job.max_chunks = job.max_win = 0;
  for (int i = 0; i < T; i++) {
    const RgSpec& sp = job.specs[i];
    const StreamDesc& sd = sds[sp.stream];
    RgTitle& ti = t[i];
    ti.x[0] = sd.pcm[0]; ti.x[1] = sd.pcm[1];
    ti.x_base = sd.pcm_base; ti.x_end = sd.pcm_end;
    long long at = sp.g0;
    ti.piece = c.rg_piece.p + po;
    for (long long k : sp.pieces) { starts[po++] = at; at += k; }
    ti.npieces = (int)sp.pieces.size();
    ti.t0 = sp.t0; ti.g0 = sp.g0; ti.g1 = at;
    ti.wa = (int)((sp.g0 - sp.t0) / W);
    ti.nwin = (int)((at - sp.t0) / W) - ti.wa;
    const int pseudo = ti.nwin + (at > sp.t0 + (long long)(ti.wa + ti.nwin) * W ? 1 : 0);
    ti.win0 = (int)nwin;
    ti.nchunks = (pseudo + RG_CHUNK_WINDOWS - 1) / RG_CHUNK_WINDOWS;
    ti.chunk0 = (int)nchunk;
    ti.carry = sp.carry ? sp.carry : c.rg_carry.p + i;
    ti.hist = sp.hist ? sp.hist : c.rg_hist.p + (size_t)i * RG_HIST;
    ti.hist_b = sp.hist_b;
    ti.title_end = sp.title_end;
    nwin += ti.nwin; nchunk += ti.nchunks;
    job.max_chunks = ti.nchunks > job.max_chunks ? ti.nchunks : job.max_chunks;
    job.max_win = ti.nwin > job.max_win ? ti.nwin : job.max_win;
  }
  job.nwin0 = T > 0 ? t[0].nwin : 0;
  job.chunk_rows = nchunk * nch;
  const int max_passes = job.max_chunks + RG_QUEUED_PASSES + 2;
  if ((rc = c.rg_titles.fit((size_t)T + 1)) || (rc = c.rg_sum.fit((size_t)nwin * 2 + 2)) || (rc = c.rg_wstate.fit((size_t)nwin * nch + 1)) ||
      (rc = c.rg_cstart.fit((size_t)job.chunk_rows + 1)) || (rc = c.rg_end_a.fit((size_t)job.chunk_rows + 1)) ||
      (rc = c.rg_end_b.fit((size_t)job.chunk_rows + 1)) || (rc = c.rg_idx.fit((size_t)nwin + 1)) ||
      (rc = c.rg_count.fit((size_t)max_passes + 2)) || (rc = c.rg_gain.fit((size_t)T + 1)))
    return rc;
  cudaStream_t st = c.rg_st;
  if (arrival) for (int j = 0; j < arrival->chunks; j++) CK(cudaStreamWaitEvent(st, arrival->ready[j], 0));
  CK(cudaEventRecord(c.ev_rg[0], c.st));
  CK(cudaStreamWaitEvent(st, c.ev_rg[0], 0));
  CK(cudaEventRecord(c.ev_rg[1], st));
  if ((rc = upload(c, c.rg_piece.p, starts.data(), sizeof(long long) * (size_t)(npiece + 1), st)) ||
      (rc = upload(c, c.rg_titles.p, t.data(), sizeof(RgTitle) * (size_t)T, st)))
    return rc;
  CK(cudaMemsetAsync(c.rg_count.p, 0, sizeof(int) * (size_t)(max_passes + 2), st));
  CK(cudaMemsetAsync(c.rg_hist.p, 0, sizeof(int) * (size_t)(T + 1) * RG_HIST, st));
  CK(cudaMemsetAsync(c.rg_carry.p, 0, sizeof(RgCarry) * (size_t)(T + 1), st));
  RgParams& p = job.prm;
  p.titles = c.rg_titles.p; p.nch = nch; p.W = W; p.req = req; p.f32 = rows.f32;
  p.scale_applied = rows.scale_applied;
  p.scale = cfg->host.scale;
  p.win_sum = c.rg_sum.p; p.win_state = c.rg_wstate.p; p.chunk_start = c.rg_cstart.p; p.end_in = c.rg_end_a.p; p.end_out = c.rg_end_b.p;
  p.done = c.rg_count.p; p.reruns = c.rg_count.p + 1; p.pass_changed = c.rg_count.p + 2;
  job.passes = 0;
  if (job.max_chunks > 0) {
    dim3 grid((unsigned)((job.max_chunks * nch + RG_THREADS - 1) / RG_THREADS), (unsigned)T);
    k_rg_pass1<<<grid, RG_THREADS, 0, st>>>(p);
    g_launches++;
    for (int q = 0; q < RG_QUEUED_PASSES; q++) {
      k_rg_repair<<<grid, RG_THREADS, 0, st>>>(p, job.passes);
      k_rg_check<<<(unsigned)((job.chunk_rows + 255) / 256), 256, 0, st>>>(p, job.passes, job.chunk_rows);
      job.passes++;
      g_launches += 2;
    }
  }
  CK(cudaGetLastError());
  return 0;
}

int rg_queue_results(ThreadCtx& c, RgJob& job) {
  cudaStream_t st = c.rg_st;
  const RgParams& p = job.prm;
  const int T = (int)job.specs.size();
  if (job.max_win > 0) {
    k_rg_hist<<<dim3((unsigned)((job.max_win + 255) / 256), (unsigned)T), 256, 0, st>>>(p.titles, p.W, p.win_sum, c.rg_idx.p);
    g_launches++;
  }
  int* album = c.rg_hist.p + (size_t)T * RG_HIST;
  k_rg_album<<<(RG_HIST + 255) / 256, 256, 0, st>>>(p.titles, T, album);
  CK(cudaMemsetAsync(c.rg_gain.p, 0, sizeof(double) * (size_t)(T + 1), st));
  k_rg_result<<<T + 1, 256, 0, st>>>(p.titles, T, album, c.rg_gain.p);
  g_launches += 2;
  return 0;
}

int rg_finish_queued(ThreadCtx& c, Config* cfg, RgJob& job, LoopGraphs& lg, int* loop, int* fault) {
  cudaStream_t st = c.rg_st;
  RgParams& p = job.prm;
  const int nch = cfg->host.nch, T = (int)job.specs.size();
  if (job.max_chunks > 0) {
    if (lg.rg_generation != c.rg_generation()) { lg.clear_rg(); lg.rg_generation = c.rg_generation(); }
    const auto key = std::make_tuple((const Config*)cfg, p.f32 != 0, T, job.max_chunks, job.chunk_rows, (const int*)loop);
    if (!lg.rg_exec.count(key) && lg.rg_exec.size() >= MP3_RG_GRAPHS) {
      auto lru = lg.rg_exec.begin();
      for (auto e = lg.rg_exec.begin(); e != lg.rg_exec.end(); ++e) if (e->second.used < lru->second.used) lru = e;
      cudaGraphExecDestroy(lru->second.exec);
      lg.rg_exec.erase(lru);
    }
    LoopGraphs::RgGraph& slot = lg.rg_exec[key];
    slot.used = ++lg.rg_tick;
    cudaGraphExec_t& exec = slot.exec;
    if (!exec) {
      cudaGraph_t g = nullptr;
      cudaGraphConditionalHandle cond;
      cudaGraphNode_t node;
      cudaGraphNodeParams cp = {};
      cp.type = cudaGraphNodeTypeConditional;
      bool ok = cudaGraphCreate(&g, 0) == cudaSuccess;
      ok = ok && cudaGraphConditionalHandleCreate(&cond, g, 1, cudaGraphCondAssignDefault) == cudaSuccess;
      cp.conditional.handle = cond; cp.conditional.type = cudaGraphCondTypeWhile; cp.conditional.size = 1;
      ok = ok && cudaGraphAddNode(&node, g, nullptr, 0, &cp) == cudaSuccess;
      cudaGraph_t body = ok ? cp.conditional.phGraph_out[0] : nullptr;
      if (ok && cudaStreamBeginCaptureToGraph(lg.capture, body, nullptr, nullptr, 0, cudaStreamCaptureModeThreadLocal) == cudaSuccess) {
        dim3 grid((unsigned)((job.max_chunks * nch + RG_THREADS - 1) / RG_THREADS), (unsigned)T);
        k_rg_repair_at<<<grid, RG_THREADS, 0, lg.capture>>>(p, loop);
        k_rg_check_at<<<(unsigned)((job.chunk_rows + 255) / 256), 256, 0, lg.capture>>>(p, loop, job.chunk_rows);
        k_rg_loop_cond<<<1, 1, 0, lg.capture>>>(cond, loop, p.done, job.max_chunks + RG_QUEUED_PASSES + 1, fault);
        cudaGraph_t captured = nullptr;
        ok = cudaStreamEndCapture(lg.capture, &captured) == cudaSuccess && captured == body &&
             cudaGraphInstantiate(&exec, g, 0) == cudaSuccess;
      } else {
        ok = false;
      }
      if (g) cudaGraphDestroy(g);
      if (!ok) {
        exec = nullptr;
        lg.rg_exec.erase(key);
        g_err = "ReplayGain loop graph failed: " + std::string(cudaGetErrorString(cudaGetLastError()));
        return MP3B200_ERR_CUDA;
      }
      lg.instantiated++;
    }
    const int first = RG_QUEUED_PASSES;
    int rc = upload(c, loop, &first, sizeof first, st);
    if (rc) return rc;
    CK(cudaGraphLaunch(exec, st));
    k_rg_report<<<1, 1, 0, st>>>(loop, p.pass_changed, p.reruns);
    g_launches += 2;
  }
  const int rc = rg_queue_results(c, job);
  if (rc) return rc;
  k_rg_finish<<<T, 256, 0, st>>>(p.titles, p.end_in, nch);
  g_launches++;
  CK(cudaGetLastError());
  return 0;
}

int rg_finish(ThreadCtx& c, Config* cfg, RgJob& job) {
  cudaStream_t st = c.rg_st;
  RgParams& p = job.prm;
  const int nch = cfg->host.nch, T = (int)job.specs.size();
  int rc = 0;
  if (job.max_chunks > 0) {
    dim3 grid((unsigned)((job.max_chunks * nch + RG_THREADS - 1) / RG_THREADS), (unsigned)T);
    for (;;) {
      int done = 0;
      CK(cudaMemcpyAsync(&done, p.done, sizeof(int), cudaMemcpyDeviceToHost, st));
      CK(cudaStreamSynchronize(st));
      if (done) break;
      if (job.passes >= job.max_chunks + RG_QUEUED_PASSES + 1) { g_err = "ReplayGain repair did not converge"; return MP3B200_ERR_CUDA; }
      k_rg_repair<<<grid, RG_THREADS, 0, st>>>(p, job.passes);
      k_rg_check<<<(unsigned)((job.chunk_rows + 255) / 256), 256, 0, st>>>(p, job.passes, job.chunk_rows);
      job.passes++;
      g_launches += 2;
    }
    CK(cudaMemcpyAsync(&job.reruns, p.reruns, sizeof(int), cudaMemcpyDeviceToHost, st));
    std::vector<int> pc((size_t)job.passes);
    CK(cudaMemcpyAsync(pc.data(), p.pass_changed, sizeof(int) * (size_t)job.passes, cudaMemcpyDeviceToHost, st));
    CK(cudaStreamSynchronize(st));
    int used = 0;
    while (used < job.passes && pc[used] != 0) used++;
    job.passes = used + 1;
  }
  rc = rg_queue_results(c, job);
  if (rc) return rc;
  std::vector<int> hist0;
  if (job.want_windows && T > 0) {
    job.hist0.assign(RG_HIST, 0);
    RgTitle t0;
    CK(cudaMemcpyAsync(&t0, p.titles, sizeof t0, cudaMemcpyDeviceToHost, st));
    CK(cudaStreamSynchronize(st));
    CK(cudaMemcpyAsync(job.hist0.data(), t0.hist, sizeof(int) * RG_HIST, cudaMemcpyDeviceToHost, st));
  }
  k_rg_finish<<<T, 256, 0, st>>>(p.titles, p.end_in, nch);
  g_launches++;
  CK(cudaEventRecord(c.ev_rg[2], st));
  std::vector<double> g((size_t)T + 1);
  CK(cudaMemcpyAsync(g.data(), c.rg_gain.p, sizeof(double) * (size_t)(T + 1), cudaMemcpyDeviceToHost, st));
  if (job.want_windows) {
    job.win_sum.assign((size_t)job.nwin0 * 2, 0.0);
    job.win_idx.assign((size_t)job.nwin0, 0);
    if (job.nwin0 > 0) {
      CK(cudaMemcpyAsync(job.win_sum.data(), c.rg_sum.p, sizeof(double) * 2 * (size_t)job.nwin0, cudaMemcpyDeviceToHost, st));
      CK(cudaMemcpyAsync(job.win_idx.data(), c.rg_idx.p, sizeof(int) * (size_t)job.nwin0, cudaMemcpyDeviceToHost, st));
    }
  }
  CK(cudaStreamSynchronize(st));
  CK(cudaGetLastError());
  CK(cudaEventElapsedTime(&job.ms, c.ev_rg[1], c.ev_rg[2]));
  job.title_db.assign((size_t)T, (double)RG_NOT_ENOUGH_SAMPLES);
  for (int i = 0; i < T; i++) if (job.specs[i].title_end) job.title_db[i] = g[i];
  job.album_db = g[T];
  return 0;
}

int launch_streams(ThreadCtx& c, Config* cfg, std::vector<StreamDesc>& sds, uint8_t* d_out, const LaunchOpts& o) {
  if (o.timings_ms) for (int i = 0; i < 16; i++) o.timings_ms[i] = 0.0f;
  const PcmArrival* arrival = o.arrival;
  const int nstreams = (int)sds.size();
  if (o.rg && nstreams > MP3_MAX_LAUNCH_STREAMS) { g_err = "ReplayGain batches hold at most 65535 streams"; return MP3B200_ERR_HANDLE; }
  {
    int rc = c.ws.refusals.fit(2);
    if (rc) return rc;
    CK(cudaMemsetAsync(c.ws.refusals.p, 0, 2 * sizeof(int), c.st));
  }
  {
    const int rc = wait_legacy(c);
    if (rc) return rc;
  }
  for (int g0 = 0; g0 < nstreams; g0 += MP3_MAX_LAUNCH_STREAMS) {
    const int n = nstreams - g0 < MP3_MAX_LAUNCH_STREAMS ? nstreams - g0 : MP3_MAX_LAUNCH_STREAMS;
    StreamDesc* group = sds.data() + g0;
    long long U = 0, F = 0;
    for (int i = 0; i < n; i++) {
      group[i].unit_base = (int)U; group[i].frame_base = (int)F;
      U += (long long)cfg->host.mode_gr * group[i].nframes; F += group[i].nframes;
    }
    if (F == 0) continue;
    int rc = o.analyse_only ? 0 : c.ws.fit(n, cfg->host.nch, U, F);
    if (rc) return rc;
    const bool resampled = cfg->rs.ratio > 1;
    if (resampled || o.f32_in) {
      if (arrival)
        for (int j = 0; j < arrival->chunks; j++) CK(cudaStreamWaitEvent(c.st, arrival->ready[j], 0));
      arrival = nullptr;
    }
    Rows rows = {false, cfg->host.scale_applied};
    if (o.f32_in) {
      rc = stage_streams(c, cfg, group, n);
      if (rc) return rc;
      rows = SCALED_F32;
    }
    if (resampled) {
      rc = resample_streams(c, cfg, group, n, rows);
      if (rc) return rc;
      rows = SCALED_F32;
    }
    if (o.rg) {
      rc = rg_queue(c, cfg, group, *o.rg, arrival, rows);
      if (rc) return rc;
    }
    Timings tm;
    rc = o.analyse_only ? 0 : run_pipeline(c, cfg, group, n, d_out, o, arrival, rows, &tm);
    if (rc) return rc;
    if (o.rg) {
      rc = o.loops ? rg_finish_queued(c, cfg, *o.rg, *o.loops, o.rg_loop ? o.rg_loop : c.ws.refusals.p + 5, c.ws.refusals.p + 3)
                   : rg_finish(c, cfg, *o.rg);
      if (rc) return rc;
    }
    arrival = nullptr;
    float rs_ms = 0.0f;
    if (resampled && o.timings_ms && o.sync) CK(cudaEventElapsedTime(&rs_ms, c.ev_rs[0], c.ev_rs[1]));
    if (o.committed)
      CK(cudaMemcpyAsync(o.committed + g0, c.ws.streams.p, sizeof(StreamDesc) * n, cudaMemcpyDeviceToHost, c.st));
    if (o.timings_ms) {
      const float t[16] = {tm.psy, tm.scan, tm.mask, tm.fb, tm.q1, tm.qn, tm.total, 0.0f,
                           tm.q_prepare, tm.q_search, tm.q_outer, tm.q_finish, tm.q_pack, tm.q_mid, rs_ms, 0.0f};
      for (int i = 0; i < 16; i++) o.timings_ms[i] += t[i];
      if ((float)tm.passes > o.timings_ms[7]) o.timings_ms[7] = (float)tm.passes;
    }
  }
  return o.sync && (o.f32_in || !o.stop_after_mdct) ? check_refusals(c) : 0;
}

}

extern "C" {

const char* mp3b200_last_error(void) { return g_err.c_str(); }
#ifdef Q_STATS
int mp3b200_debug_qstats(unsigned long long* out16, int reset) {
  if (cudaMemcpyFromSymbol(out16, g_qstats, sizeof(unsigned long long) * 16) != cudaSuccess) return MP3B200_ERR_CUDA;
  if (reset) { unsigned long long z[16] = {0}; cudaMemcpyToSymbol(g_qstats, z, sizeof z); }
  return 0;
}
#endif
int64_t mp3b200_launch_count(void) { return g_launches; }

int mp3b200_set_device(int device) {
  int n = 0;
  if (cudaGetDeviceCount(&n) != cudaSuccess || device < 0 || device >= n || device >= MP3_MAX_DEVICES) { g_err = "invalid CUDA device"; return MP3B200_ERR_CUDA; }
  std::lock_guard<std::mutex> lk(g_mu);
  g_device = device;
  return 0;
}

int64_t mp3b200_stream_frames(int64_t nsamples) { return frames_for(nsamples, 2); }

int64_t mp3b200_stream_bytes(int channels, int samplerate, int kbps, int64_t nsamples) {
  return mp3b200_stream_bytes_ex(channels, samplerate, kbps, 0, nsamples);
}

int64_t mp3b200_stream_bytes_ex(int channels, int samplerate, int kbps, int flags, int64_t nsamples) {
  const Config* c = encodable_config(channels, samplerate, kbps, flags);
  if (!c || nsamples < 0) return -1;
  return bytes_of_frames(c->host, 0, frames_for(nsamples, c->host.mode_gr, c->rs.ratio));
}

int64_t mp3b200_stream_frames_cfg(int channels, int samplerate, int kbps, int64_t nsamples) {
  return mp3b200_stream_frames_ex(channels, samplerate, kbps, 0, nsamples);
}

int64_t mp3b200_stream_frames_ex(int channels, int samplerate, int kbps, int flags, int64_t nsamples) {
  const Config* c = encodable_config(channels, samplerate, kbps, flags);
  if (!c || nsamples < 0) return -1;
  return frames_for(nsamples, c->host.mode_gr, c->rs.ratio);
}

int mp3b200_granules_per_frame(int channels, int samplerate, int kbps) {
  return mp3b200_granules_per_frame_ex(channels, samplerate, kbps, 0);
}

int mp3b200_granules_per_frame_ex(int channels, int samplerate, int kbps, int flags) {
  const Config* c = encodable_config(channels, samplerate, kbps, flags);
  return c ? c->host.mode_gr : -1;
}

int mp3b200_out_samplerate(int channels, int samplerate, int kbps) { return mp3_out_samplerate(channels, samplerate, kbps); }

}

namespace {
template <class T>
std::vector<StreamDesc> whole_streams(Config* cfg, int nstreams, const T* d_pcm, const int64_t* pcm_off,
                                      const int64_t* nsamples, const int64_t* out_off) {
  std::vector<StreamDesc> sds(nstreams);
  for (int s = 0; s < nstreams; s++) {
    StreamDesc& sd = sds[s];
    memset(&sd, 0, sizeof sd);
    const T* x = d_pcm + pcm_off[s];
    sd.pcm[0] = x;
    sd.pcm[1] = cfg->host.nch == 2 ? x + nsamples[s] : x;
    sd.pcm_base = 0; sd.pcm_end = nsamples[s];
    sd.frame0 = 0; sd.nframes = (int)frames_for(nsamples[s], cfg->host.mode_gr, cfg->rs.ratio);
    sd.out_base = out_off[s];
    init_stream_state(sd);
  }
  return sds;
}

template <class T> T* staging_pcm(size_t n) { return t_ctx.pcm.fit(sizeof(T) * n) ? nullptr : reinterpret_cast<T*>(t_ctx.pcm.p); }

template <class T> const T* right_row(const T* const* left, const T* const* right, int s) { return right && right[s] ? right[s] : left[s]; }

bool finite_after_scale(const Mp3Tables& T, const float* x, long long n) {
  for (long long i = 0; i < n; i++) {
    float v = x[i];
    if (T.scale_applied) v = (float)((double)v * T.scale);
    if (!(std::fabs(v) <= MP3_F32_MAX_SAMPLE)) return false;
  }
  return true;
}

int check_input(const Config*, int, const int16_t* const*, const int16_t* const*, const int64_t*) { return MP3B200_OK; }
int check_input(const Config* cfg, int nstreams, const float* const* left, const float* const* right, const int64_t* nsamples) {
  for (int s = 0; s < nstreams; s++)
    if (!finite_after_scale(cfg->host, left[s], nsamples[s]) ||
        (cfg->host.nch == 2 && !finite_after_scale(cfg->host, right_row(left, right, s), nsamples[s]))) {
      g_err = "non-finite input sample (or one beyond 2^40 once scaled)"; return MP3B200_ERR_CONFIG;
    }
  return MP3B200_OK;
}

template <class T>
int upload_host_rows(const Config* cfg, int nstreams, const T* const* left, const T* const* right, const int64_t* nsamples,
                     std::vector<int64_t>& pcm_off, T*& d_pcm, PcmArrival& arr) {
  const int nch = cfg->host.nch;
  pcm_off.assign(nstreams, 0);
  long long tot_samples = 0;
  for (int s = 0; s < nstreams; s++) {
    pcm_off[s] = tot_samples;
    tot_samples += nsamples[s] * nch;
  }
  d_pcm = staging_pcm<T>((size_t)tot_samples + 8);
  if (!d_pcm) return MP3B200_ERR_CUDA;
  arr.chunks = (nstreams <= 8 && tot_samples >= (1 << 20)) ? MP3_MAX_PCM_CHUNKS : 1;
  arr.ready = t_ctx.ready;
  for (int j = 0; j < arr.chunks; j++) {
    for (int s = 0; s < nstreams; s++) {
      const int64_t lo = nsamples[s] * j / arr.chunks, hi = nsamples[s] * (j + 1) / arr.chunks;
      if (hi <= lo) continue;
      CK(cudaMemcpyAsync(d_pcm + pcm_off[s] + lo, left[s] + lo, sizeof(T) * (hi - lo), cudaMemcpyHostToDevice, t_ctx.up_st));
      if (nch == 2)
        CK(cudaMemcpyAsync(d_pcm + pcm_off[s] + nsamples[s] + lo, right_row(left, right, s) + lo, sizeof(T) * (hi - lo),
                           cudaMemcpyHostToDevice, t_ctx.up_st));
    }
    CK(cudaEventRecord(t_ctx.ready[j], t_ctx.up_st));
  }
  return MP3B200_OK;
}

template <class T>
int stage_host_streams(Config* cfg, int nstreams, const T* const* left, const T* const* right, const int64_t* nsamples,
                       const int64_t* cap, const int* room, int64_t* out_bytes, std::vector<int64_t>& out_off,
                       std::vector<StreamDesc>& sds, PcmArrival& arr) {
  out_off.assign(nstreams, 0);
  long long tot_bytes = 0;
  for (int s = 0; s < nstreams; s++) {
    out_off[s] = tot_bytes;
    const long long n = bytes_of_frames(cfg->host, 0, frames_for(nsamples[s], cfg->host.mode_gr, cfg->rs.ratio)) + (room ? room[s] : 0);
    if (cap[s] < n) { g_err = "output buffer too small"; return MP3B200_ERR_BUFFER; }
    out_bytes[s] = n;
    tot_bytes += n;
  }
  if (nstreams == 0) return MP3B200_OK;
  std::vector<int64_t> pcm_off;
  T* d_pcm = nullptr;
  int rc = upload_host_rows(cfg, nstreams, left, right, nsamples, pcm_off, d_pcm, arr);
  if (rc || (rc = t_ctx.out.fit((size_t)tot_bytes + 8))) return rc;
  sds = whole_streams(cfg, nstreams, d_pcm, pcm_off.data(), nsamples, out_off.data());
  return MP3B200_OK;
}

}

extern "C" {

int mp3b200_encode_streams_device(int channels, int samplerate, int kbps, int nstreams, const int16_t* d_pcm,
                                  const int64_t* pcm_off, const int64_t* nsamples, uint8_t* d_out,
                                  const int64_t* out_off, float* timings_ms) {
  return mp3b200_encode_streams_device_ex(channels, samplerate, kbps, 0, nstreams, d_pcm, pcm_off, nsamples, d_out, out_off, timings_ms);
}

}

namespace {
template <class T>
int encode_device(int channels, int samplerate, int kbps, int flags, int nstreams, const T* d_pcm, const int64_t* pcm_off,
                  const int64_t* nsamples, uint8_t* d_out, const int64_t* out_off, float* timings_ms) {
  if (nstreams < 0) { g_err = "negative stream count"; return MP3B200_ERR_HANDLE; }
  Config* cfg;
  const int rc = get_config(channels, samplerate, kbps, flags, &cfg);
  if (rc) return rc;
  std::vector<StreamDesc> sds = whole_streams(cfg, nstreams, d_pcm, pcm_off, nsamples, out_off);
  LaunchOpts o;
  o.timings_ms = timings_ms;
  o.f32_in = std::is_same_v<T, float>;
  return launch_streams(t_ctx, cfg, sds, d_out, o);
}

template <class T>
int encode_host(int channels, int samplerate, int kbps, int flags, int nstreams, const T* const* left, const T* const* right,
                const int64_t* nsamples, uint8_t* const* out, const int64_t* cap, int64_t* out_bytes) {
  if (nstreams < 0) { g_err = "negative stream count"; return MP3B200_ERR_HANDLE; }
  Config* cfg;
  int rc = get_config(channels, samplerate, kbps, flags, &cfg);
  if (rc || (rc = check_input(cfg, nstreams, left, right, nsamples))) return rc;
  std::vector<int64_t> out_off;
  std::vector<StreamDesc> sds;
  PcmArrival arr;
  rc = stage_host_streams(cfg, nstreams, left, right, nsamples, cap, nullptr, out_bytes, out_off, sds, arr);
  if (rc || nstreams == 0) return rc;
  LaunchOpts o;
  o.arrival = &arr;
  o.f32_in = std::is_same_v<T, float>;
  if ((rc = launch_streams(t_ctx, cfg, sds, t_ctx.out.p, o))) return rc;
  for (int s = 0; s < nstreams; s++)
    if (cudaMemcpyAsync(out[s], t_ctx.out.p + out_off[s], (size_t)out_bytes[s], cudaMemcpyDeviceToHost, t_ctx.st) != cudaSuccess) rc = MP3B200_ERR_CUDA;
  if (cudaStreamSynchronize(t_ctx.st) != cudaSuccess) rc = MP3B200_ERR_CUDA;
  return rc;
}
}

extern "C" {

int mp3b200_encode_streams_device_ex(int channels, int samplerate, int kbps, int flags, int nstreams, const int16_t* d_pcm,
                                     const int64_t* pcm_off, const int64_t* nsamples, uint8_t* d_out,
                                     const int64_t* out_off, float* timings_ms) {
  return encode_device(channels, samplerate, kbps, flags, nstreams, d_pcm, pcm_off, nsamples, d_out, out_off, timings_ms);
}

int mp3b200_encode_streams_device_f32(int channels, int samplerate, int kbps, int flags, int nstreams, const float* d_pcm,
                                      const int64_t* pcm_off, const int64_t* nsamples, uint8_t* d_out,
                                      const int64_t* out_off, float* timings_ms) {
  return encode_device(channels, samplerate, kbps, flags, nstreams, d_pcm, pcm_off, nsamples, d_out, out_off, timings_ms);
}

int mp3b200_encode_streams(int channels, int samplerate, int kbps, int nstreams, const int16_t* const* left,
                           const int16_t* const* right, const int64_t* nsamples, uint8_t* const* out,
                           const int64_t* cap, int64_t* out_bytes) {
  return mp3b200_encode_streams_ex(channels, samplerate, kbps, 0, nstreams, left, right, nsamples, out, cap, out_bytes);
}

int mp3b200_encode_streams_ex(int channels, int samplerate, int kbps, int flags, int nstreams, const int16_t* const* left,
                              const int16_t* const* right, const int64_t* nsamples, uint8_t* const* out,
                              const int64_t* cap, int64_t* out_bytes) {
  return encode_host(channels, samplerate, kbps, flags, nstreams, left, right, nsamples, out, cap, out_bytes);
}

int mp3b200_encode_streams_f32(int channels, int samplerate, int kbps, int flags, int nstreams, const float* const* left,
                               const float* const* right, const int64_t* nsamples, uint8_t* const* out,
                               const int64_t* cap, int64_t* out_bytes) {
  return encode_host(channels, samplerate, kbps, flags, nstreams, left, right, nsamples, out, cap, out_bytes);
}

int mp3b200_debug_stages(int channels, int samplerate, int kbps, const int16_t* left, const int16_t* right,
                         int64_t nsamples, const int32_t* force_blocktype, float* xr, int32_t* blocktype,
                         float* en_l, float* thm_l, float* en_s, float* thm_s, double* ath_adjust,
                         int32_t* l3_enc, int32_t* ginfo, uint8_t* bytes_out, int64_t bytes_cap) {
  mp3b200_debug_taps t;
  memset(&t, 0, sizeof t);
  t.size = (int32_t)sizeof t; t.channels = channels; t.samplerate = samplerate; t.kbps = kbps;
  t.left = left; t.right = right; t.nsamples = nsamples; t.force_blocktype = force_blocktype;
  t.xr = xr; t.blocktype = blocktype; t.en_l = en_l; t.thm_l = thm_l; t.en_s = en_s; t.thm_s = thm_s; t.ath_adjust = ath_adjust;
  t.l3_enc = l3_enc; t.ginfo = ginfo; t.bytes_out = bytes_out; t.bytes_cap = bytes_cap;
  return mp3b200_debug_stages_ex(&t);
}

}

namespace {
template <class T>
int debug_stages(const mp3b200_debug_taps* tp, const T* left, const T* right) {
  if (!tp || tp->size != (int32_t)sizeof(mp3b200_debug_taps)) { g_err = "mp3b200_debug_taps: size must be sizeof(mp3b200_debug_taps)"; return MP3B200_ERR_HANDLE; }
  const int channels = tp->channels;
  const int64_t nsamples = tp->nsamples;
  const int32_t* force_blocktype = tp->force_blocktype;
  float *xr = tp->xr, *en_l = tp->en_l, *thm_l = tp->thm_l, *en_s = tp->en_s, *thm_s = tp->thm_s;
  int32_t *blocktype = tp->blocktype, *l3_enc = tp->l3_enc, *ginfo = tp->ginfo;
  double* ath_adjust = tp->ath_adjust;
  uint8_t* bytes_out = tp->bytes_out;
  const int64_t bytes_cap = tp->bytes_cap;
  Config* cfg;
  int rc = get_config(channels, tp->samplerate, tp->kbps, tp->flags, &cfg);
  if (rc || (rc = check_input(cfg, 1, &left, &right, &nsamples))) return rc;
  if (!right) right = left;
  const int nch = cfg->host.nch;
  const int G = cfg->host.mode_gr;
  const long long F = frames_for(nsamples, G, cfg->rs.ratio), U = G * F;
  const long long nbytes = bytes_of_frames(cfg->host, 0, F);
  T* d_pcm = staging_pcm<T>((size_t)(nsamples * nch + 8));
  if (!d_pcm) return MP3B200_ERR_CUDA;
  rc = t_ctx.out.fit((size_t)nbytes + 8);
  if (rc) return rc;
  uint8_t* d_out = t_ctx.out.p;
  CK(cudaMemcpyAsync(d_pcm, left, sizeof(T) * nsamples, cudaMemcpyHostToDevice, t_ctx.st));
  if (nch == 2) CK(cudaMemcpyAsync(d_pcm + nsamples, right, sizeof(T) * nsamples, cudaMemcpyHostToDevice, t_ctx.st));
  const int64_t zero = 0;
  std::vector<StreamDesc> sds = whole_streams(cfg, 1, d_pcm, &zero, &nsamples, &zero);
  const bool want_gi = ginfo || tp->scalefac || tp->subblock_gain;
  const bool want_prep = tp->xmin || tp->max_nonzero_coeff || tp->xrpow_max;
  const bool want_q = tp->scfsi || tp->old_value || tp->cur_step;
  LaunchOpts opts;
  opts.f32_in = std::is_same_v<T, float>;
  opts.force_bt = force_blocktype;
  opts.stop_after_mdct = !(l3_enc || bytes_out || want_gi || want_prep || want_q);
  rc = launch_streams(t_ctx, cfg, sds, d_out, opts);
  auto fetch = [](void* dst, const void* src, size_t bytes) {
    const cudaError_t e = cudaMemcpyAsync(dst, src, bytes, cudaMemcpyDeviceToHost, t_ctx.st);
    return e != cudaSuccess ? e : cudaStreamSynchronize(t_ctx.st);
  };
  const Workspace& ws = t_ctx.ws;
  if (rc == 0) {
    if (xr) CK(fetch(xr, ws.xr.p, sizeof(float) * (size_t)U * nch * 576));
    if (blocktype) {
      std::vector<signed char> bt((size_t)U * 2);
      CK(fetch(bt.data(), ws.bt_final.p, bt.size()));
      for (long long u = 0; u < U; u++) for (int c = 0; c < nch; c++) blocktype[u * nch + c] = bt[u * 2 + c];
    }
    if (en_l || thm_l || en_s || thm_s) {
      std::vector<PsyRatioDev> r((size_t)(U + 1) * nch);
      CK(fetch(r.data(), ws.ratio.p, sizeof(PsyRatioDev) * r.size()));
      for (long long u = 0; u < U; u++) for (int c = 0; c < nch; c++) {
        const PsyRatioDev& q = r[(size_t)u * nch + c];
        if (en_l) memcpy(en_l + (u * nch + c) * 22, q.en_l, sizeof q.en_l);
        if (thm_l) memcpy(thm_l + (u * nch + c) * 22, q.thm_l, sizeof q.thm_l);
        if (en_s) memcpy(en_s + (u * nch + c) * 39, q.en_s, sizeof q.en_s);
        if (thm_s) memcpy(thm_s + (u * nch + c) * 39, q.thm_s, sizeof q.thm_s);
      }
    }
    if (ath_adjust) CK(fetch(ath_adjust, ws.ath_q.p, sizeof(double) * (size_t)F));
    if (l3_enc) {
      std::vector<short> t((size_t)U * nch * 576);
      CK(fetch(t.data(), ws.l3enc.p, sizeof(short) * t.size()));
      for (size_t i = 0; i < t.size(); i++) l3_enc[i] = t[i];
    }
    if (want_gi) {
      std::vector<GranuleInfoDev> g((size_t)U * nch);
      CK(fetch(g.data(), ws.ginfo.p, sizeof(GranuleInfoDev) * g.size()));
      for (size_t i = 0; i < g.size(); i++) {
        if (ginfo) {
          int32_t* o = ginfo + i * 16;
          o[0] = g[i].global_gain; o[1] = g[i].part2_3_length; o[2] = g[i].part2_length; o[3] = g[i].big_values;
          o[4] = g[i].count1; o[5] = g[i].scalefac_compress; o[6] = g[i].table_select[0]; o[7] = g[i].table_select[1];
          o[8] = g[i].table_select[2]; o[9] = g[i].region0_count; o[10] = g[i].region1_count; o[11] = g[i].preflag;
          o[12] = g[i].scalefac_scale; o[13] = g[i].count1table_select; o[14] = g[i].block_type; o[15] = 0;
        }
        if (tp->scalefac) memcpy(tp->scalefac + i * MP3_SFBMAX, g[i].scalefac, sizeof(int32_t) * MP3_SFBMAX);
        if (tp->subblock_gain) for (int k = 0; k < 3; k++) tp->subblock_gain[i * 3 + k] = g[i].subblock_gain[k];
      }
    }
    if (want_prep) {
      std::vector<GcPrep> p((size_t)U * nch);
      CK(fetch(p.data(), ws.prep.p, sizeof(GcPrep) * p.size()));
      for (size_t i = 0; i < p.size(); i++) {
        if (tp->xmin) {
          const int psymax = p[i].block_type == BT_SHORT ? 36 : 21;
          for (int k = 0; k < MP3_SFBMAX; k++) tp->xmin[i * MP3_SFBMAX + k] = (p[i].have && k < psymax) ? p[i].xmin[k] : 0.0f;
        }
        if (tp->max_nonzero_coeff) tp->max_nonzero_coeff[i] = p[i].mnz;
        if (tp->xrpow_max) tp->xrpow_max[i] = p[i].xrpow_max;
      }
    }
    if (want_q) {
      std::vector<QuantFrameState> q((size_t)F);
      CK(fetch(q.data(), ws.qstate.p, sizeof(QuantFrameState) * q.size()));
      for (long long f = 0; f < F; f++) {
        const QuantFrameState& s = q[(size_t)f];
        for (int c = 0; c < nch; c++) {
          if (tp->scfsi) for (int b = 0; b < 4; b++) tp->scfsi[(f * nch + c) * 4 + b] = s.scfsi[c][b];
          const int ov[3] = {s.in_old[c], G == 2 ? s.bs_gain0[c] : 0, s.out_old[c]};
          const int cs[3] = {s.in_step[c], G == 2 ? s.bs_step0[c] : 0, s.out_step[c]};
          for (int k = 0; k < 3; k++) {
            if (tp->old_value) tp->old_value[(f * 3 + k) * nch + c] = ov[k];
            if (tp->cur_step) tp->cur_step[(f * 3 + k) * nch + c] = cs[k];
          }
        }
      }
    }
    if (bytes_out) {
      if (bytes_cap < nbytes) { g_err = "output buffer too small"; rc = MP3B200_ERR_BUFFER; }
      else CK(fetch(bytes_out, d_out, (size_t)nbytes));
    }
  }
  return rc;
}

template <class T>
int debug_resample(int channels, int samplerate, int kbps, const T* left, const T* right, int64_t nsamples, float* y, int64_t ny) {
  if (nsamples < 0 || ny < 0 || (nsamples > 0 && !left) || (ny > 0 && !y)) { g_err = "bad buffers"; return MP3B200_ERR_HANDLE; }
  Config* cfg;
  int rc = get_config(channels, samplerate, kbps, MP3B200_RESAMPLE, &cfg);
  if (rc) return rc;
  if (cfg->rs.ratio == 1) { g_err = "this configuration does not resample"; return MP3B200_ERR_CONFIG; }
  if ((rc = check_input(cfg, 1, &left, &right, &nsamples))) return rc;
  if (!right) right = left;
  if (ny == 0) return 0;
  const int nch = cfg->host.nch;
  T* d_pcm = staging_pcm<T>((size_t)(nsamples * nch + 8));
  if (!d_pcm) return MP3B200_ERR_CUDA;
  rc = t_ctx.ws.rs_y.fit((size_t)(ny * nch));
  if (rc) return rc;
  if (nsamples > 0) {
    CK(cudaMemcpyAsync(d_pcm, left, sizeof(T) * nsamples, cudaMemcpyHostToDevice, t_ctx.st));
    if (nch == 2) CK(cudaMemcpyAsync(d_pcm + nsamples, right, sizeof(T) * nsamples, cudaMemcpyHostToDevice, t_ctx.st));
  }
  StreamDesc sd;
  memset(&sd, 0, sizeof sd);
  sd.pcm[0] = d_pcm;
  sd.pcm[1] = nch == 2 ? d_pcm + nsamples : d_pcm;
  sd.pcm_end = nsamples;
  Rows rows = {false, cfg->host.scale_applied};
  if (std::is_same_v<T, float>) {
    rc = t_ctx.ws.refusals.fit(2);
    if (rc) return rc;
    rc = stage_streams(t_ctx, cfg, &sd, 1);
    if (rc) return rc;
    rows = SCALED_F32;
  }
  ResampleDesc d;
  d.x[0] = sd.pcm[0]; d.x[1] = sd.pcm[1]; d.x_base = 0; d.x_end = nsamples;
  d.y[0] = t_ctx.ws.rs_y.p; d.y[1] = d.y[0] + (nch == 2 ? ny : 0); d.y_base = 0; d.ny = ny;
  rc = queue_resample(t_ctx, cfg, &d, 1, ny, rows);
  if (rc) return rc;
  CK(cudaGetLastError());
  CK(cudaMemcpyAsync(y, t_ctx.ws.rs_y.p, sizeof(float) * (size_t)(ny * nch), cudaMemcpyDeviceToHost, t_ctx.st));
  CK(cudaStreamSynchronize(t_ctx.st));
  return 0;
}
}

extern "C" {

int mp3b200_debug_stages_ex(const mp3b200_debug_taps* tp) { return debug_stages(tp, tp ? tp->left : nullptr, tp ? tp->right : nullptr); }
int mp3b200_debug_stages_f32(const mp3b200_debug_taps* tp, const float* left, const float* right) { return debug_stages(tp, left, right); }

int mp3b200_debug_resample(int channels, int samplerate, int kbps, const int16_t* left, const int16_t* right, int64_t nsamples,
                           float* y, int64_t ny) {
  return debug_resample(channels, samplerate, kbps, left, right, nsamples, y, ny);
}
int mp3b200_debug_resample_f32(int channels, int samplerate, int kbps, const float* left, const float* right, int64_t nsamples,
                               float* y, int64_t ny) {
  return debug_resample(channels, samplerate, kbps, left, right, nsamples, y, ny);
}

}

namespace {
CrcTables g_crc_host;
bool g_crc_host_ready = false;
CrcTables* g_crc_dev[MP3_MAX_DEVICES] = {};

const CrcTables& crc_host() {
  std::lock_guard<std::mutex> lk(g_mu);
  if (!g_crc_host_ready) { crc_host_tables(&g_crc_host); g_crc_host_ready = true; }
  return g_crc_host;
}

int crc_tables_on(int device) {
  const CrcTables& ht = crc_host();
  std::lock_guard<std::mutex> lk(g_mu);
  if (!g_crc_dev[device]) {
    CK(cudaMalloc(&g_crc_dev[device], sizeof(CrcTables)));
    CK(cudaMemcpy(g_crc_dev[device], &ht, sizeof(CrcTables), cudaMemcpyHostToDevice));
  }
  return 0;
}

int queue_music_crc(ThreadCtx& c, const std::vector<long long>& at, const std::vector<long long>& len) {
  const int R = (int)at.size();
  if (R == 0) return 0;
  std::vector<long long> ranges((size_t)2 * R);
  long long longest = 0;
  for (int i = 0; i < R; i++) { ranges[i] = at[i]; ranges[(size_t)R + i] = len[i]; longest = len[i] > longest ? len[i] : longest; }
  int rc = 0;
  if ((rc = c.crc_ranges.fit((size_t)2 * R)) || (rc = c.crc.fit((size_t)R)) ||
      (rc = upload(c, c.crc_ranges.p, ranges.data(), sizeof(long long) * ranges.size())))
    return rc;
  CK(cudaMemsetAsync(c.crc.p, 0, sizeof(unsigned) * (size_t)R, c.st));
  const long long pieces = (longest + CRC_PIECE_BYTES - 1) / CRC_PIECE_BYTES;
  for (int r0 = 0; r0 < R && longest > 0; r0 += 65535) {
    const int nr = R - r0 < 65535 ? R - r0 : 65535;
    dim3 grid((unsigned)((pieces + CRC_WARPS - 1) / CRC_WARPS), (unsigned)nr);
    k_music_crc<<<grid, CRC_WARPS * 32, 0, c.st>>>(nullptr, c.crc_ranges.p + r0, c.crc_ranges.p + R + r0, g_crc_dev[c.device], c.crc.p + r0);
    g_launches++;
  }
  return 0;
}

int build_lametag(int channels, int samplerate, int kbps, int flags, int64_t nframes, int64_t music_bytes, int music_crc,
                  int encoder_padding, int field, uint8_t* buf, int cap) {
  const Config* c = host_config(channels, samplerate, kbps, flags);
  if (!c) return MP3B200_ERR_CONFIG;
  const Mp3TagParams& p = c->tag;
  if (!p.fits || nframes <= 0) return 0;
  if (!buf || cap < p.frame_bytes) return p.frame_bytes;
  Mp3SeekBag* bag = new Mp3SeekBag();
  bag->reset();
  bag->add_frames(nframes, p.kbps);
  const int n = mp3_tag_frame(p, *bag, music_bytes, (unsigned)music_crc, encoder_padding, buf, field);
  delete bag;
  return n;
}
}

extern "C" {

int mp3b200_wav_read_header(const uint8_t* data, int64_t len, mp3b200_wav_header* out) {
  if (!out || len < 0 || (len > 0 && !data)) return MP3B200_ERR_HANDLE;
  long long off = 0, dl = 0; int ch = 0; unsigned sr = 0;
  const int rc = mp3_wav_read_header(data, len, &off, &dl, &ch, &sr);
  out->data_offset = off; out->data_len = dl; out->channels = ch; out->sample_rate = sr;
  return rc;
}

int mp3b200_debug_music_crc(const uint8_t* d_buf, const int64_t* off, const int64_t* len, int nranges, uint32_t* crc, float* ms) {
  if (nranges < 0 || (nranges > 0 && (!d_buf || !off || !len || !crc))) return MP3B200_ERR_HANDLE;
  int dev = 0;
  { std::lock_guard<std::mutex> lk(g_mu); dev = g_device; int rc = ensure_device(dev); if (rc) return rc; }
  int rc = t_ctx.use(dev);
  if (rc || (rc = crc_tables_on(dev)) || (rc = wait_legacy(t_ctx))) return rc;
  std::vector<long long> at(off, off + nranges), l(len, len + nranges);
  for (long long& a : at) a += (long long)(uintptr_t)d_buf;
  for (int run = 0; run < (ms ? 2 : 1); run++) {
    if (run) CK(cudaEventRecord(t_ctx.ev[0], t_ctx.st));
    if ((rc = queue_music_crc(t_ctx, at, l))) return rc;
    if (nranges > 0) CK(cudaMemcpyAsync(crc, t_ctx.crc.p, sizeof(uint32_t) * (size_t)nranges, cudaMemcpyDeviceToHost, t_ctx.st));
    if (run) CK(cudaEventRecord(t_ctx.ev[1], t_ctx.st));
    CK(cudaStreamSynchronize(t_ctx.st));
    CK(cudaGetLastError());
  }
  if (ms) CK(cudaEventElapsedTime(ms, t_ctx.ev[0], t_ctx.ev[1]));
  return 0;
}

int mp3b200_get_vbr_tag(const uint8_t* frame, int64_t len, mp3b200_vbr_tag_data* out) {
  if (!out || len < 0 || (len > 0 && !frame)) return MP3B200_ERR_HANDLE;
  Mp3VbrTagData t;
  const int rc = mp3_tag_parse(frame, len, &t);
  out->h_id = t.h_id; out->samprate = t.samprate; out->flags = t.flags; out->frames = t.frames; out->bytes = t.bytes;
  out->vbr_scale = t.vbr_scale; out->headersize = t.headersize; out->enc_delay = t.enc_delay; out->enc_padding = t.enc_padding;
  memcpy(out->toc, t.toc, 100);
  return rc;
}

int mp3b200_crc16_combine(int crc_a, int crc_b, int64_t len_b) {
  if (len_b < 0) return MP3B200_ERR_HANDLE;
  return (int)crc_append((unsigned)crc_a & 0xffffu, (unsigned)crc_b & 0xffffu, (unsigned long long)len_b, crc_host().pow);
}

int mp3b200_lametag_size(int channels, int samplerate, int kbps) {
  return mp3b200_lametag_size_ex(channels, samplerate, kbps, 0);
}

int mp3b200_lametag_size_ex(int channels, int samplerate, int kbps, int flags) {
  const Config* c = host_config(channels, samplerate, kbps, flags);
  if (!c) return MP3B200_ERR_CONFIG;
  return c->tag.fits ? c->tag.frame_bytes : 0;
}

int mp3b200_lametag_build(int channels, int samplerate, int kbps, int64_t nframes, int64_t music_bytes, int music_crc, int encoder_padding,
                          uint8_t* buf, int cap) {
  return build_lametag(channels, samplerate, kbps, 0, nframes, music_bytes, music_crc, encoder_padding, 0, buf, cap);
}

int mp3b200_encode_streams_tagged(int channels, int samplerate, int kbps, int nstreams, const int16_t* const* left,
                                  const int16_t* const* right, const int64_t* nsamples, uint8_t* const* out,
                                  const int64_t* cap, int64_t* out_bytes) {
  return mp3b200_encode_streams_tagged_ex(channels, samplerate, kbps, 0, nstreams, left, right, nsamples, out, cap, out_bytes,
                                          nullptr, nullptr);
}

}

namespace {
struct TaggedPlan {
  int tfs = 0;
  std::vector<long long> frames;
  std::vector<int> padding, tag;
};
TaggedPlan stream_plan(const Config* cfg, int nstreams, const int64_t* nsamples, RgJob* rg) {
  TaggedPlan pl;
  pl.tfs = cfg->tag.fits ? cfg->tag.frame_bytes : 0;
  if (rg) rg->specs.assign((size_t)nstreams, RgSpec());
  pl.frames.resize((size_t)nstreams); pl.padding.resize((size_t)nstreams); pl.tag.resize((size_t)nstreams);
  for (int s = 0; s < nstreams; s++) {
    LameFifo fifo(cfg->host.mode_gr, cfg->rs.ratio);
    if (rg) { rg->specs[s].stream = s; fifo.pieces = &rg->specs[s].pieces; }
    const long long fed = fifo.feed(nsamples[s]);
    const FifoFlush fl = fifo.flush();
    pl.frames[s] = fed + fl.frames;
    pl.padding[s] = fl.end_padding;
    pl.tag[s] = pl.tfs > 0 && pl.frames[s] > 0 ? pl.tfs : 0;
  }
  return pl;
}

TaggedPlan tagged_plan(const Config* cfg, int nstreams, const int64_t* nsamples, RgJob*& rg) {
  if (rg && !cfg->tag.fits) rg = nullptr;
  return stream_plan(cfg, nstreams, nsamples, rg);
}

int finish_tagged(ThreadCtx& c, Config* cfg, const TaggedPlan& plan, const std::vector<StreamDesc>& sds, const std::vector<long long>& audio,
                  uint8_t* d_out, const int64_t* out_off, const double* gain) {
  const int S = (int)sds.size();
  const Mp3TagParams& p = cfg->tag;
  int ntags = 0;
  for (int i = 0; i < S; i++) ntags += plan.tag[i] ? 1 : 0;
// ... 302 lines not shown
```

lamejs_b200/encoder.py:

```python
import ctypes
import os

import numpy as np

from . import build as _build

_HERE = os.path.dirname(os.path.abspath(__file__))
_lib = None


class Mp3B200Error(RuntimeError):
    pass


class DebugTaps(ctypes.Structure):
    _vp = ctypes.c_void_p
    _fields_ = [("size", ctypes.c_int32), ("channels", ctypes.c_int32), ("samplerate", ctypes.c_int32), ("kbps", ctypes.c_int32),
                ("left", _vp), ("right", _vp), ("nsamples", ctypes.c_int64), ("force_blocktype", _vp),
                ("xr", _vp), ("blocktype", _vp), ("en_l", _vp), ("thm_l", _vp), ("en_s", _vp), ("thm_s", _vp), ("ath_adjust", _vp),
                ("l3_enc", _vp), ("ginfo", _vp), ("bytes_out", _vp), ("bytes_cap", ctypes.c_int64),
                ("scalefac", _vp), ("subblock_gain", _vp), ("xmin", _vp), ("max_nonzero_coeff", _vp), ("xrpow_max", _vp),
                ("scfsi", _vp), ("old_value", _vp), ("cur_step", _vp), ("flags", ctypes.c_int32)]


# ... 501 lines not shown

GAIN_NOT_ENOUGH_SAMPLES = -24601


def radio_gain(title_db):
    return int(np.floor(title_db * 10.0 + 0.5))


def lametag_build_ex(channels, samplerate, kbps, nframes, music_bytes, music_crc, encoder_padding, radio_gain, resample=False):
    buf = np.zeros(2880, dtype=np.uint8)
    n = lib().mp3b200_lametag_build_ex(channels, samplerate, kbps, RESAMPLE if resample else 0, nframes, music_bytes, music_crc,
                                       encoder_padding, radio_gain, buf.ctypes.data, len(buf))
    _check(min(n, 0))
    return buf[:n].tobytes()


def debug_replaygain(channels, samplerate, kbps, left, right=None, resample=False):
    (left,), (right,), f32 = _rows([left], [None if channels == 1 else right])
    cap = len(left) // 400 + 64
    sums = np.zeros((cap, 2), dtype=np.float64)
    idx = np.zeros(cap, dtype=np.int32)
    hist = np.zeros(12000, dtype=np.int32)
    title = ctypes.c_double(0.0)
    stats = np.zeros(4, dtype=np.int32)
    _check(_entry("mp3b200_debug_replaygain", f32)(channels, samplerate, kbps, RESAMPLE if resample else 0, left.ctypes.data,
                                                   right.ctypes.data, len(left), sums.ctypes.data, idx.ctypes.data, cap,
                                                   hist.ctypes.data, ctypes.byref(title), stats.ctypes.data))
    n = int(stats[0])
    assert n <= cap
    return {"sums": sums[:n].copy(), "idx": idx[:n].copy(), "hist": hist, "title_db": float(title.value), "passes": int(stats[1]),
            "reruns": int(stats[2]), "ms": float(stats[3:4].view(np.float32)[0])}


DOMAIN_SITES = ("trunc_mask_idx", "trunc_log16", "trunc_quant", "trunc_noise", "dmax", "dmin", "pack_search", "pack_outer",
                "region_mx", "bitsum_field", "log16_table", "f32_overflow")


def debug_domain_hits():
    fn = getattr(lib(), "mp3b200_debug_domain_hits", None)
    if fn is None:
        raise Mp3B200Error("the library was built without MP3_DOMAIN_CHECK")
    out = np.zeros(len(DOMAIN_SITES), dtype=np.uint64)
    fn.argtypes = [ctypes.c_void_p, ctypes.c_int]
    n = _check(fn(out.ctypes.data, len(out)))
    assert n == len(DOMAIN_SITES), n
    return out.astype(np.int64)


def debug_music_crc(d_buf_ptr, offsets, lengths, timed=False):
    off = np.ascontiguousarray(offsets, dtype=np.int64)
    ln = np.ascontiguousarray(lengths, dtype=np.int64)
    crc = np.zeros(len(off), dtype=np.uint32)
    ms = ctypes.c_float(0)
    _check(lib().mp3b200_debug_music_crc(d_buf_ptr, off.ctypes.data, ln.ctypes.data, len(off), crc.ctypes.data, ctypes.byref(ms) if timed else None))
    return ([int(c) for c in crc], float(ms.value)) if timed else [int(c) for c in crc]


def encode_streams_device(channels, samplerate, kbps, d_pcm_ptr, pcm_off, nsamples, d_out_ptr, out_off, resample=False, float32=False):
    pcm_off = np.ascontiguousarray(pcm_off, dtype=np.int64)
    nsamples = np.ascontiguousarray(nsamples, dtype=np.int64)
    out_off = np.ascontiguousarray(out_off, dtype=np.int64)
    tm = np.zeros(16, dtype=np.float32)
    _check(_entry("mp3b200_encode_streams_device_ex", float32)(channels, samplerate, kbps, RESAMPLE if resample else 0, len(nsamples),
                                                                d_pcm_ptr, pcm_off.ctypes.data, nsamples.ctypes.data, d_out_ptr,
                                                                out_off.ctypes.data, tm.ctypes.data))
    return tm


def encode_streams_device_tagged(channels, samplerate, kbps, d_pcm_ptr, pcm_off, nsamples, d_out_ptr, out_off, resample=False,
                                 float32=False, find_replay_gain=False):
    pcm_off = np.ascontiguousarray(pcm_off, dtype=np.int64)
    nsamples = np.ascontiguousarray(nsamples, dtype=np.int64)
    out_off = np.ascontiguousarray(out_off, dtype=np.int64)
    S = len(nsamples)
    got = np.zeros(max(S, 1), dtype=np.int64)
    title = np.zeros(max(S, 1), dtype=np.float64)
    album = ctypes.c_double(0.0)
    flags = (REPLAYGAIN if find_replay_gain else 0) | (RESAMPLE if resample else 0)
    _check(_entry("mp3b200_encode_streams_tagged_device", float32)(channels, samplerate, kbps, flags, S, d_pcm_ptr, pcm_off.ctypes.data,
                                                                    nsamples.ctypes.data, d_out_ptr, out_off.ctypes.data,
                                                                    got.ctypes.data, title.ctypes.data, ctypes.byref(album)))
    return ([int(g) for g in got[:S]], [float(t) for t in title[:S]],
            float(album.value) if S else float(GAIN_NOT_ENOUGH_SAMPLES))


class EncodeSession:

    def __init__(self, stream=None):
        import torch
        self.stream = torch.cuda.current_stream() if stream is None else stream
        self.device = self.stream.device
        h = ctypes.c_void_p()
        with torch.cuda.device(self.device):
            _check(lib().mp3b200_session_create(ctypes.c_void_p(self.stream.cuda_stream or None), ctypes.byref(h)))
        self._h = h

    def _checked(self, channels, samplerate, kbps, pcm, pcm_off, nsamples, out, out_off, resample, tag_bytes):
        import torch
        if self._h is None:
            raise ValueError("the session is closed")
        if pcm.dtype not in (torch.int16, torch.float32):
            raise TypeError("pcm must be int16 or float32, not %s" % pcm.dtype)
        if out.dtype != torch.uint8:
            raise TypeError("out must be uint8, not %s" % out.dtype)
        for name, t in (("pcm", pcm), ("out", out)):
            if not _on_cuda(t) or t.device != self.device:
                raise ValueError("%s must be a CUDA tensor on the session's device (%s)" % (name, self.device))
            if t.dim() != 1 or not t.is_contiguous():
                raise ValueError("%s must be a contiguous 1-D tensor" % name)
        pcm_off = np.ascontiguousarray(pcm_off, dtype=np.int64)
        nsamples = np.ascontiguousarray(nsamples, dtype=np.int64)
        out_off = np.ascontiguousarray(out_off, dtype=np.int64)
        S = len(nsamples)
        if len(pcm_off) != S or len(out_off) != S:
            raise ValueError("pcm_off, nsamples and out_off must have one entry per stream")
        if S:
            nb = {int(n): stream_bytes(channels, samplerate, kbps, int(n), resample) for n in np.unique(nsamples) if n >= 0}
            if all(b >= 0 for b in nb.values()) and (nsamples >= 0).all():
                room = np.array([nb[int(n)] + tag_bytes for n in nsamples], dtype=np.int64)
                if ((pcm_off < 0) | (pcm_off + nsamples * channels > pcm.numel()) | (out_off < 0) |
                        (out_off + room > out.numel())).any():
                    raise ValueError("a stream lies outside pcm or out")
        return pcm_off, nsamples, out_off

    def encode_streams(self, channels, samplerate, kbps, pcm, pcm_off, nsamples, out, out_off, resample=False):
        import torch
        pcm_off, nsamples, out_off = self._checked(channels, samplerate, kbps, pcm, pcm_off, nsamples, out, out_off, resample, 0)
        with torch.cuda.stream(self.stream):
            status = torch.empty(4, dtype=torch.int32, device=self.device)
        fn = lib().mp3b200_encode_streams_async_f32 if pcm.dtype == torch.float32 else lib().mp3b200_encode_streams_async
        _check(fn(self._h, channels, samplerate, kbps, RESAMPLE if resample else 0, len(nsamples), pcm.data_ptr(), pcm_off.ctypes.data,
                  nsamples.ctypes.data, out.data_ptr(), out_off.ctypes.data, status.data_ptr()))
        for t in (pcm, out, status):
            t.record_stream(self.stream)
        return status

    def encode_streams_tagged(self, channels, samplerate, kbps, pcm, pcm_off, nsamples, out, out_off, resample=False,
                              find_replay_gain=False):
        import torch
        tfs = lametag_size(channels, samplerate, kbps, resample)
        pcm_off, nsamples, out_off = self._checked(channels, samplerate, kbps, pcm, pcm_off, nsamples, out, out_off, resample,
                                                   max(tfs, 0))
        S = len(nsamples)
        got = np.zeros(max(S, 1), dtype=np.int64)
        with torch.cuda.stream(self.stream):
            status = torch.empty(8, dtype=torch.int32, device=self.device)
            gains = torch.empty(S + 1, dtype=torch.float64, device=self.device) if find_replay_gain else None
        flags = (REPLAYGAIN if find_replay_gain else 0) | (RESAMPLE if resample else 0)
        fn = _entry("mp3b200_encode_streams_tagged_async", pcm.dtype == torch.float32)
        _check(fn(self._h, channels, samplerate, kbps, flags, S, pcm.data_ptr(), pcm_off.ctypes.data, nsamples.ctypes.data,
                  out.data_ptr(), out_off.ctypes.data, got.ctypes.data, gains.data_ptr() if find_replay_gain else None,
                  status.data_ptr()))
        for t in (pcm, out, status) + ((gains,) if find_replay_gain else ()):
            t.record_stream(self.stream)
        return [int(g) for g in got[:S]], gains, status

    def _handles(self, encoders):
        if self._h is None:
            raise ValueError("the session is closed")
        if any(not isinstance(e, Mp3Encoder) or not e._h for e in encoders):
            raise ValueError("encoders must be open Mp3Encoder objects")
        if len({id(e) for e in encoders}) != len(encoders):
            raise ValueError("a session call names each encoder once (make two calls instead)")
        return (ctypes.c_void_p * max(len(encoders), 1))(*[e._h for e in encoders])

    def _queue(self, encoders, lengths, call, *tensors, status_words=4):
        import torch
        S = len(encoders)
        hp = self._handles(encoders)
        lengths = [_check(int(lib().mp3b200_encode_bytes(e._h, n))) for e, n in zip(encoders, lengths)]
        offsets = np.zeros(max(S, 1), dtype=np.int64)
        if S > 1:
            offsets[1:S] = np.cumsum(lengths[:-1])
        with torch.cuda.stream(self.stream):
            out = torch.empty(max(sum(lengths), 1), dtype=torch.uint8, device=self.device)
            status = torch.empty(status_words, dtype=torch.int32, device=self.device)
        got = np.zeros(max(S, 1), dtype=np.int32)
        _check(call(hp, out.data_ptr(), offsets.ctypes.data, got.ctypes.data, status.data_ptr()))
        for t in (out, status) + tensors:
            t.record_stream(self.stream)
        assert [int(g) for g in got[:S]] == lengths
        return out, [int(o) for o in offsets[:S]], lengths, status

    def encode_batch(self, encoders, lefts, rights=None):
        return self._encode(encoders, lefts, rights, False)

    def encode_batch_tagged(self, encoders, lefts, rights=None):
        return self._encode(encoders, lefts, rights, True)

    def _encode(self, encoders, lefts, rights, tagged):
        import torch
        if self._h is None:
            raise ValueError("the session is closed")
        S = len(encoders)
        if len(lefts) != S or (rights is not None and len(rights) != S):
            raise ValueError("one row (pair) per encoder")
        rights = [None] * S if rights is None else list(rights)
        rows = [x for x in (*lefts, *rights) if x is not None]
        if not all(_on_cuda(x) and x.device == self.device for x in rows):
            raise ValueError("rows must be CUDA tensors on the session's device (%s)" % self.device)
        if any(x.dim() != 1 for x in rows):
            raise ValueError("rows must be 1-D")
        f32 = any(x.dtype.is_floating_point for x in rows)
        dt = torch.float32 if f32 else torch.int16
        with torch.cuda.stream(self.stream):
            lefts = [x.to(dt).contiguous() for x in lefts]
            rights = [l if (r is None or e.channels == 1) else r.to(dt).contiguous() for e, l, r in zip(encoders, lefts, rights)]
        if any(len(l) != len(r) for l, r in zip(lefts, rights)):
            raise ValueError("left and right rows differ in length")
        ns = np.array([len(x) for x in lefts] or [0], dtype=np.int32)
        lp = (ctypes.c_void_p * max(S, 1))(*[x.data_ptr() for x in lefts])
        rp = (ctypes.c_void_p * max(S, 1))(*[x.data_ptr() for x in rights])
        fn = _entry("mp3b200_session_encode_batch_tagged" if tagged else "mp3b200_session_encode_batch", f32)
        return self._queue(encoders, [int(n) for n in ns[:S]],
                           lambda hp, o, off, got, st: fn(self._h, hp, lp, rp, ns.ctypes.data, S, o, off, got, st),
                           *lefts, *rights, status_words=8 if tagged else 4)

    def flush_batch(self, encoders):
        S = len(encoders)
        return self._queue(encoders, [-1] * S,
                           lambda hp, o, off, got, st: lib().mp3b200_session_flush_batch(self._h, hp, S, o, off, got, st))

    def flush_batch_tagged(self, encoders):
        S = len(encoders)
        return self._queue(encoders, [-1] * S,
                           lambda hp, o, off, got, st: lib().mp3b200_session_flush_batch_tagged(self._h, hp, S, o, off, got, st),
                           status_words=8)

    def lametag_frames(self, encoders):
        import torch
        S = len(encoders)
        hp = self._handles(encoders)
        room = [e._tag_room if e.tag_on else 0 for e in encoders]
        offsets = np.zeros(max(S, 1), dtype=np.int64)
        if S > 1:
            offsets[1:S] = np.cumsum(room[:-1])
        with torch.cuda.stream(self.stream):
            out = torch.empty(max(sum(room), 1), dtype=torch.uint8, device=self.device)
            status = torch.empty(4, dtype=torch.int32, device=self.device)
        got = np.zeros(max(S, 1), dtype=np.int32)
        _check(lib().mp3b200_session_lametag_frames(self._h, hp, S, out.data_ptr(), offsets.ctypes.data, got.ctypes.data,
                                                    status.data_ptr()))
        for t in (out, status):
            t.record_stream(self.stream)
        return out, [int(o) for o in offsets[:S]], [int(g) for g in got[:S]], status

    def album_gain(self, encoders):
        import torch
        hp = self._handles(encoders)
        with torch.cuda.stream(self.stream):
            album = torch.empty(1, dtype=torch.float64, device=self.device)
            status = torch.empty(4, dtype=torch.int32, device=self.device)
        _check(lib().mp3b200_session_album_gain(self._h, hp, len(encoders), album.data_ptr(), status.data_ptr()))
        for t in (album, status):
            t.record_stream(self.stream)
        return album, status

    def graph_instantiations(self):
        if self._h is None:
            raise ValueError("the session is closed")
        return int(lib().mp3b200_session_graph_instantiations(self._h))

    def release(self, encoders):
        hp = self._handles(encoders)
        _check(lib().mp3b200_session_release(self._h, hp, len(encoders)))

    def close(self):
        if self._h is not None:
            h, self._h = self._h, None
            _check(lib().mp3b200_session_destroy(h))

    def __enter__(self):
        return self

    def __exit__(self, *exc):
        self.close()

    def __del__(self):
        try:
            self.close()
        except Exception:
            pass


def check_status(status):
    import torch
    torch.cuda.synchronize(status.device)
    words = np.ascontiguousarray(status.cpu().numpy(), dtype=np.int32)
    _check(lib().mp3b200_check_status(words.ctypes.data))
    return int(words[2])


def debug_resample(channels, samplerate, kbps, left, right=None, ny=None):
    (left,), (right,), f32 = _rows([left], [None if channels == 1 else right])
    r = samplerate // out_samplerate(channels, samplerate, kbps)
    if ny is None:
        ny = (len(left) + 15) // r + 1
    y = np.zeros((channels, ny), dtype=np.float32)
    _check(_entry("mp3b200_debug_resample", f32)(channels, samplerate, kbps, left.ctypes.data, right.ctypes.data, len(left),
                                                 y.ctypes.data, ny))
    return y


def debug_stages(channels, samplerate, kbps, left, right=None, force_blocktype=None, want=("xr",), resample=False):
    L = lib()
    (left,), (right,), f32 = _rows([left], [None if channels == 1 else right])
    n = len(left)
    F = stream_frames(n, channels, samplerate, kbps, resample)
    G = granules_per_frame(channels, samplerate, kbps, resample)
    if F < 0 or G < 0:
        raise Mp3B200Error("unsupported configuration: channels=%d samplerate=%d kbps=%d" % (channels, samplerate, kbps))
    nch = channels
    res = {}

    def alloc(name, shape, dt):
        if name in want:
            res[name] = np.zeros(shape, dtype=dt)
            return res[name].ctypes.data
        return None

    fb = None
    if force_blocktype is not None:
        fb = np.ascontiguousarray(force_blocktype, dtype=np.int32)
        assert fb.shape == (F, G, nch)
    p_xr = alloc("xr", (F, G, nch, 576), np.float32)
    p_bt = alloc("blocktype", (F, G, nch), np.int32)
    p_enl = alloc("en_l", (F, G, nch, 22), np.float32)
    p_thl = alloc("thm_l", (F, G, nch, 22), np.float32)
    p_ens = alloc("en_s", (F, G, nch, 13, 3), np.float32)
    p_ths = alloc("thm_s", (F, G, nch, 13, 3), np.float32)
    p_ath = alloc("ath_adjust", (F,), np.float64)
    p_l3 = alloc("l3_enc", (F, G, nch, 576), np.int32)
    p_gi = alloc("ginfo", (F, G, nch, 16), np.int32)
    nb = stream_bytes(channels, samplerate, kbps, n, resample)
    if nb < 0:
        raise Mp3B200Error("unsupported configuration: channels=%d samplerate=%d kbps=%d" % (channels, samplerate, kbps))
    p_by = alloc("bytes", (nb,), np.uint8)
    t = DebugTaps(size=ctypes.sizeof(DebugTaps), channels=channels, samplerate=samplerate, kbps=kbps, left=left.ctypes.data,
                  right=right.ctypes.data, nsamples=n, force_blocktype=fb.ctypes.data if fb is not None else None,
                  xr=p_xr, blocktype=p_bt, en_l=p_enl, thm_l=p_thl, en_s=p_ens, thm_s=p_ths, ath_adjust=p_ath,
                  l3_enc=p_l3, ginfo=p_gi, bytes_out=p_by, bytes_cap=nb,
                  scalefac=alloc("scalefac", (F, G, nch, 39), np.int32), subblock_gain=alloc("subblock_gain", (F, G, nch, 3), np.int32),
                  xmin=alloc("xmin", (F, G, nch, 39), np.float32), max_nonzero_coeff=alloc("max_nonzero_coeff", (F, G, nch), np.int32),
                  xrpow_max=alloc("xrpow_max", (F, G, nch), np.float64), scfsi=alloc("scfsi", (F, nch, 4), np.int32),
                  old_value=alloc("old_value", (F, 3, nch), np.int32), cur_step=alloc("cur_step", (F, 3, nch), np.int32),
                  flags=RESAMPLE if resample else 0)
    if f32:
        _check(L.mp3b200_debug_stages_f32(ctypes.byref(t), left.ctypes.data, right.ctypes.data))
    else:
        _check(L.mp3b200_debug_stages_ex(ctypes.byref(t)))
    return res
```

Before: 53930.

## Compute short-block psychoacoustics only for granules that need short blocks

The short-window FFT, energy and spreading work moves out of the main psy kernel into a separate persistent kernel. That kernel runs only over a compacted list of granules whose final block type (or the next granule's) is short, built by a small list kernel with atomics. The masking kernel skips short-block ratio computation and output when short data is not read. This removes three short FHTs and their spreading from most granules of typical music, at the cost of two extra launches, an atomic work queue, and a separate PsyShort buffer.

```diff
diff --git a/include/mp3b200.h b/include/mp3b200.h
--- a/include/mp3b200.h
+++ b/include/mp3b200.h
@@ -141,6 +141,7 @@
                          float* en_l, float* thm_l, float* en_s, float* thm_s, double* ath_adjust,
                          int32_t* l3_enc, int32_t* ginfo, uint8_t* bytes_out, int64_t bytes_cap);
 
+#define MP3B200_DEBUG_SKIP_SHORT 0x10000
 typedef struct mp3b200_debug_taps {
   int32_t size, channels, samplerate, kbps;
   const int16_t *left, *right;
@@ -153,6 +154,7 @@
   int32_t flags;
 } mp3b200_debug_taps;
 int mp3b200_debug_stages_ex(const mp3b200_debug_taps* t);
+int64_t mp3b200_debug_short_units(void);
 
 int mp3b200_debug_resample(int channels, int samplerate, int kbps, const int16_t* left, const int16_t* right, int64_t nsamples,
                            float* y, int64_t ny);
diff --git a/lamejs_b200/__init__.py b/lamejs_b200/__init__.py
--- a/lamejs_b200/__init__.py
+++ b/lamejs_b200/__init__.py
@@ -1,4 +1,4 @@
-from .encoder import Mp3Encoder, WavHeader, id3v1_tag, id3v2_tag, ID3_ADD_V2, ID3_V1_ONLY, ID3_V2_ONLY, ID3_SPACE_V1, ID3_PAD_V2, lametag_size, lametag_build, get_vbr_tag, crc16_combine, encode_streams_tagged, debug_music_crc, encode_batch, flush_batch, encode_streams, encode_streams_device, encode_streams_device_tagged, debug_stages, debug_resample, lib, stream_bytes, stream_frames, granules_per_frame, out_samplerate, RESAMPLE, Mp3B200Error
+from .encoder import Mp3Encoder, WavHeader, id3v1_tag, id3v2_tag, ID3_ADD_V2, ID3_V1_ONLY, ID3_V2_ONLY, ID3_SPACE_V1, ID3_PAD_V2, lametag_size, lametag_build, get_vbr_tag, crc16_combine, encode_streams_tagged, debug_music_crc, encode_batch, flush_batch, encode_streams, encode_streams_device, encode_streams_device_tagged, debug_stages, debug_short_units, debug_resample, lib, stream_bytes, stream_frames, granules_per_frame, out_samplerate, RESAMPLE, Mp3B200Error
 from .encoder import REPLAYGAIN, GAIN_NOT_ENOUGH_SAMPLES, radio_gain, lametag_build_ex, debug_replaygain, encode_streams_replaygain, album_gain
 from .encoder import DOMAIN_SITES, debug_domain_hits
 from .encoder import EncodeSession, check_status
diff --git a/lamejs_b200/csrc/k_psy.cuh b/lamejs_b200/csrc/k_psy.cuh
--- a/lamejs_b200/csrc/k_psy.cuh
+++ b/lamejs_b200/csrc/k_psy.cuh
@@ -9,14 +9,16 @@
 #define MASK_THREADS 128
 
 struct PsyUnit {
-  double ecb_s[3][MP3_CBANDS];
-  float eb_s[3][MP3_CBANDS];
   float eb_l[MP3_CBANDS];
   float peaks[9];
   float loudness;
   unsigned char mask_idx[MP3_CBANDS];
   unsigned char attack[4];
   unsigned char pad_;
+};
+struct PsyShort {
+  double ecb_s[3][MP3_CBANDS];
+  float eb_s[3][MP3_CBANDS];
 };
 struct PsyRatioDev { float en_l[22], thm_l[22], en_s[13][3], thm_s[13][3]; };
 
@@ -128,6 +130,29 @@
 
 __device__ __forceinline__ size_t psy_row(const StreamDesc& sd, int z, int u) { return (size_t)sd.unit_base + z + u + 1; }
 
+template <bool F32_PCM, int NT>
+__device__ __forceinline__ void psy_load_span(const Mp3Tables* __restrict__ T, const StreamDesc& sd, int ch, long long x0, double* xs) {
+  using Sample = pcm_sample_t<F32_PCM>;
+  const int tid = threadIdx.x;
+  const int scale_applied = T->scale_applied;
+  const double scale = T->scale;
+  const Sample* __restrict__ pbuf = static_cast<const Sample*>(sd.pcm[ch]);
+  const long long pbase = sd.pcm_base, pend = sd.pcm_end;
+  constexpr int NB = (1024 + NT - 1) / NT;
+  Sample v[NB];
+#pragma unroll
+  for (int k = 0; k < NB; k++) {
+    const int j = tid + k * NT;
+    const long long i = x0 + j;
+    v[k] = (j < 1024 && i >= 0 && i < pend) ? __ldg(&pbuf[i - pbase]) : (Sample)0;
+  }
+#pragma unroll
+  for (int k = 0; k < NB; k++) {
+    const int j = tid + k * NT;
+    if (j < 1024) xs[j] = pcm_value(v[k], scale_applied, scale);
+  }
+}
+
 #ifndef PSY_MIN_BLOCKS
 #define PSY_MIN_BLOCKS 12
 #endif
@@ -154,7 +179,6 @@
   const int tid = threadIdx.x;
 
   if (c < 0) {
-    for (int i = tid; i < 3 * MP3_CBANDS; i += PSY_THREADS) { (&o->ecb_s[0][0])[i] = 1.0; (&o->eb_s[0][0])[i] = 0.0f; }
     if (tid < MP3_CBANDS) { o->eb_l[tid] = 0.0f; o->mask_idx[tid] = 0; }
     if (tid < 9) o->peaks[tid] = 10.0f;
     if (tid == 0) o->loudness = 0.0f;
@@ -165,43 +189,19 @@
   __shared__ __align__(16) unsigned char s_u[sizeof(double) * 1024];
   double* const xs = reinterpret_cast<double*>(s_u);
   f32s* const fe = reinterpret_cast<f32s*>(s_u);
-  f32s (*const fes)[129] = reinterpret_cast<f32s (*)[129]>(s_u + 2064);
-  f32s* const s_max = reinterpret_cast<f32s*>(s_u + 2064 + 1552);
+  f32s* const s_max = reinterpret_cast<f32s*>(s_u + 2064);
   f32s* const s_avg = s_max + MP3_CBANDS;
-  f32s (*const s_ebs)[MP3_CBANDS] = reinterpret_cast<f32s (*)[MP3_CBANDS]>(s_avg + MP3_CBANDS);
-  static_assert(2064 + 1552 + 2 * 4 * MP3_CBANDS + 3 * 4 * MP3_CBANDS <= (int)sizeof(s_u), "energies must fit the PCM span");
-  constexpr int PROD_HI_OFF = 2064 + 1552 + 2 * 4 * MP3_CBANDS + 3 * 4 * MP3_CBANDS;
+  constexpr int PROD_HI_OFF = 2064 + 2 * 4 * MP3_CBANDS;
   static_assert(PROD_HI_OFF % 8 == 0 && PROD_HI_OFF + 256 * 8 <= (int)sizeof(s_u), "second half of the loudness terms");
   double* const prod_hi = reinterpret_cast<double*>(s_u + PROD_HI_OFF);
   __shared__ f32w wl[1024 + 64];
-  __shared__ f32w wsh[3][256 + 16];
   __shared__ __align__(8) f32s hp[576];
   double* const prod_lo = reinterpret_cast<double*>(hp);
   static_assert(sizeof(f32s) * 576 >= 256 * 8, "first half of the loudness terms");
   __shared__ int s_peak[9];
   if (tid < 9) s_peak[tid] = __float_as_int(1.0f);
 
-  const int scale_applied = T->scale_applied;
-  const double scale = T->scale;
-  const long long x0 = 576 * c - 224;
-  {
-    using Sample = pcm_sample_t<F32_PCM>;
-    const Sample* __restrict__ pbuf = static_cast<const Sample*>(sd.pcm[ch]);
-    const long long pbase = sd.pcm_base, pend = sd.pcm_end;
-    constexpr int NB = (1024 + PSY_THREADS - 1) / PSY_THREADS;
-    Sample v[NB];
-#pragma unroll
-    for (int k = 0; k < NB; k++) {
-      const int j = tid + k * PSY_THREADS;
-      const long long i = x0 + j;
-      v[k] = (j < 1024 && i >= 0 && i < pend) ? __ldg(&pbuf[i - pbase]) : (Sample)0;
-    }
-#pragma unroll
-    for (int k = 0; k < NB; k++) {
-      const int j = tid + k * PSY_THREADS;
-      if (j < 1024) xs[j] = pcm_value(v[k], scale_applied, scale);
-    }
-  }
+  psy_load_span<F32_PCM, PSY_THREADS>(T, sd, ch, 576 * c - 224, xs);
   __syncthreads();
 
   for (int i = tid; i < 576; i += PSY_THREADS) {
@@ -214,9 +214,8 @@
     }
     hp[i] = sum1 + sum2;
   }
-  for (int vt = tid; vt < 128 + 96; vt += PSY_THREADS) {
-  if (vt < 128) {
-    const int jj = vt, i = c_fft_rv[jj], x = 4 * jj;
+  for (int jj = tid; jj < 128; jj += PSY_THREADS) {
+    const int i = c_fft_rv[jj], x = 4 * jj;
     const float* w = T->fft_window;
     double f0, f1, f2, f3, wv;
     f0 = (double)w[i] * (double)xs[i];
@@ -233,38 +232,13 @@
     wv = (double)w[i + 0x301] * (double)xs[i + 0x301];
     f3 = f2 - wv; f2 = f2 + wv;
     wl[FHT_PAD(x + 512 + 0)] = f0 + f2; wl[FHT_PAD(x + 512 + 2)] = f0 - f2; wl[FHT_PAD(x + 512 + 1)] = f1 + f3; wl[FHT_PAD(x + 512 + 3)] = f1 - f3;
-  } else {
-    const int q = vt - 128, b = q >> 5, j = q & 31;
-    const int i = c_fft_rv[j << 2], x = 4 * j, k = 192 * (b + 1);
-    const float* w = T->fft_window_s;
-    const double* bx = xs + i + k;
-    double f0, f1, f2, f3, wv;
-    f0 = (double)w[i] * (double)bx[0];
-    wv = (double)w[0x7f - i] * (double)bx[0x80];
-    f1 = f0 - wv; f0 = f0 + wv;
-    f2 = (double)w[i + 0x40] * (double)bx[0x40];
-    wv = (double)w[0x3f - i] * (double)bx[0xc0];
-    f3 = f2 - wv; f2 = f2 + wv;
-    wsh[b][FHT_PAD(x + 0)] = f0 + f2; wsh[b][FHT_PAD(x + 2)] = f0 - f2; wsh[b][FHT_PAD(x + 1)] = f1 + f3; wsh[b][FHT_PAD(x + 3)] = f1 - f3;
-    f0 = (double)w[i + 0x01] * (double)bx[0x01];
-    wv = (double)w[0x7e - i] * (double)bx[0x81];
-    f1 = f0 - wv; f0 = f0 + wv;
-    f2 = (double)w[i + 0x41] * (double)bx[0x41];
-    wv = (double)w[0x3e - i] * (double)bx[0xc1];
-    f3 = f2 - wv; f2 = f2 + wv;
-    wsh[b][FHT_PAD(x + 128 + 0)] = f0 + f2; wsh[b][FHT_PAD(x + 128 + 2)] = f0 - f2; wsh[b][FHT_PAD(x + 128 + 1)] = f1 + f3; wsh[b][FHT_PAD(x + 128 + 3)] = f1 - f3;
-  }
   }
   __syncthreads();
 
   for (int i = tid; i < 576; i += PSY_THREADS) atomicMax(&s_peak[i >> 6], __float_as_int(fabsf(hp[i].v)));
 #pragma unroll
   for (int stage = 0; stage < 4; stage++) {
-    const int nt = 128 + (stage < 3 ? 96 : 0);
-    for (int t = tid; t < nt; t += PSY_THREADS) {
-      if (t < 128) fht_task(wl, stage, t, T->tw, T->tw_off);
-      else fht_task(wsh[(t - 128) >> 5], stage, (t - 128) & 31, T->tw, T->tw_off);
-    }
+    for (int t = tid; t < 128; t += PSY_THREADS) fht_task(wl, stage, t, T->tw, T->tw_off);
     __syncthreads();
   }
 
@@ -276,33 +250,16 @@
     if (k < 512) { const double p = (double)e * (double)T->eql_w[k]; if (k < 256) prod_lo[k] = p; else prod_hi[k - 256] = p; }
   }
   if (tid == 0) { f32s t0; t0 = (double)wl[0]; t0 *= (double)t0; fe[0] = (double)t0; prod_lo[0] = (double)t0 * (double)T->eql_w[0]; }
-  for (int t = tid; t < 3 * 128; t += PSY_THREADS) {
-    const int b = t >> 7, j = t & 127;
-    const double re = wsh[b][FHT_PAD(128 - j)], im = wsh[b][FHT_PAD(128 + j)];
-    fes[b][128 - j] = (re * re + im * im) * 0.5;
-  }
-  if (tid < 3) { f32s t0; t0 = (double)wsh[tid][0]; t0 *= (double)t0; fes[tid][0] = (double)t0; }
   __syncthreads();
 
-  const int npl = T->npart_l, nps = T->npart_s;
-  for (int vt = tid; vt < 256; vt += PSY_THREADS) {
-  if (vt < npl) {
+  const int npl = T->npart_l;
+  for (int b = tid; b < npl; b += PSY_THREADS) {
     double ebb = 0, m = 0;
-    const int l0 = T->line0_l[vt], l1 = T->line0_l[vt + 1];
+    const int l0 = T->line0_l[b], l1 = T->line0_l[b + 1];
     for (int j = l0; j < l1; j++) { const double el = fe[j]; ebb += el; if (m < el) m = el; }
-    o->eb_l[vt] = (float)ebb;
-    s_max[vt] = m;
-    s_avg[vt] = ebb * (double)T->rnumlines_l[vt];
-  } else if (vt >= 64 && vt < 64 + 3 * 64) {
-    const int q = vt - 64, sb = q >> 6, b = q & 63;
-    if (b < nps) {
-      double ebb = 0;
-      const int l0 = T->line0_s[b], l1 = T->line0_s[b + 1];
-      for (int j = l0; j < l1; j++) ebb += (double)fes[sb][j];
-      s_ebs[sb][b] = ebb;
-      o->eb_s[sb][b] = (float)ebb;
-    }
-  }
+    o->eb_l[b] = (float)ebb;
+    s_max[b] = m;
+    s_avg[b] = ebb * (double)T->rnumlines_l[b];
   }
   double loud = 0.0;
   if (tid == PSY_THREADS - 1) {
@@ -312,9 +269,7 @@
   if (tid < 9) o->peaks[tid] = __int_as_float(s_peak[tid]);
   __syncthreads();
 
-  for (int vt = tid; vt < 256; vt += PSY_THREADS) {
-  if (vt < npl) {
-    const int b = vt;
+  for (int b = tid; b < npl; b += PSY_THREADS) {
     const int lo = b > 0 ? b - 1 : b, hi = b < npl - 1 ? b + 1 : b;
     double a = 0; double m = 0; int lines = 0;
     for (int q = lo; q <= hi; q++) {
@@ -330,23 +285,128 @@
       if (k > 8) k = 8;
     }
     o->mask_idx[b] = (unsigned char)k;
-  } else if (vt >= 64 && vt < 64 + 3 * 64) {
-    const int q = vt - 64, sb = q >> 6, b = q & 63;
-    if (b < nps) {
-      int kk = T->s3lo_s[b];
-      int j = T->s3off_s[b];
-      double ecb = (double)T->s3_ss[j++] * (double)s_ebs[sb][kk];
-      ++kk;
-      while (kk <= T->s3hi_s[b]) { ecb += (double)T->s3_ss[j] * (double)s_ebs[sb][kk]; ++j; ++kk; }
-      o->ecb_s[sb][b] = ecb;
-    }
-  }
   }
   if (tid == PSY_THREADS - 1) {
 #pragma unroll 8
     for (int i = 0; i < 256; ++i) loud += prod_hi[i];
     loud *= (1. / (14752. * 14752.) / 512);
     o->loudness = (float)loud;
+  }
+}
+
+
+__device__ __forceinline__ bool psy_short_read(const Mp3Tables* __restrict__ T, const StreamDesc& sd,
+                                               const signed char* __restrict__ bt_final, int u, int all) {
+  const int n = T->mode_gr * sd.nframes;
+  if (u < 0 || u >= n) return false;
+  if (all || u == n - 1) return true;
+  const size_t row = (size_t)(sd.unit_base + u + 1) * 2;
+  return bt_final[row] == BT_SHORT || (T->nch == 2 && bt_final[row + 1] == BT_SHORT);
+}
+
+__global__ void __launch_bounds__(128)
+k_psy_short_list(const Mp3Tables* __restrict__ T, const StreamDesc* __restrict__ streams, const signed char* __restrict__ bt_final,
+                 int all, int2* __restrict__ list, int* __restrict__ count) {
+  const int z = blockIdx.y;
+  const StreamDesc& sd = streams[z];
+  const int u = (int)(blockIdx.x * blockDim.x + threadIdx.x) - 1;
+  if (u >= T->mode_gr * sd.nframes) return;
+  if (!psy_short_read(T, sd, bt_final, u, all) && !psy_short_read(T, sd, bt_final, u + 1, all)) return;
+  const int nch = T->nch;
+  const int at = atomicAdd(count, nch);
+  for (int ch = 0; ch < nch; ch++) list[at + ch] = make_int2(z, ((u + 1) << 1) | ch);
+}
+
+#ifndef PSY_SHORT_BLOCKS
+#define PSY_SHORT_BLOCKS 8
+#endif
+template <bool F32_PCM>
+__global__ void __launch_bounds__(PSY_THREADS)
+k_psy_short(const Mp3Tables* __restrict__ T, const StreamDesc* __restrict__ streams, PsyShort* __restrict__ out,
+            const int2* __restrict__ list, int* __restrict__ count) {
+  const int ntasks = count[0];
+  if (ntasks == 0) return;
+  const int tid = threadIdx.x;
+  const int nch = T->nch, nps = T->npart_s;
+  __shared__ double xs[1024];
+  __shared__ f32w wsh[3][256 + 16];
+  __shared__ f32s fes[3][129];
+  __shared__ f32s s_ebs[3][MP3_CBANDS];
+  __shared__ int s_task;
+  for (;;) {
+    if (tid == 0) s_task = atomicAdd(count + 1, 1);
+    __syncthreads();
+    const int t = s_task;
+    if (t >= ntasks) return;
+    const int2 e = list[t];
+    const int z = e.x, u = (e.y >> 1) - 1, ch = e.y & 1;
+    const StreamDesc& sd = streams[z];
+    const long long c = (long long)T->mode_gr * sd.frame0 + u;
+    PsyShort* o = out + psy_row(sd, z, u) * nch + ch;
+    if (c < 0) {
+      for (int i = tid; i < 3 * MP3_CBANDS; i += PSY_THREADS) { (&o->ecb_s[0][0])[i] = 1.0; (&o->eb_s[0][0])[i] = 0.0f; }
+      __syncthreads();
+      continue;
+    }
+    psy_load_span<F32_PCM, PSY_THREADS>(T, sd, ch, 576 * c - 224, xs);
+    __syncthreads();
+    for (int q = tid; q < 96; q += PSY_THREADS) {
+      const int b = q >> 5, j = q & 31;
+      const int i = c_fft_rv[j << 2], x = 4 * j, k = 192 * (b + 1);
+      const float* w = T->fft_window_s;
+      const double* bx = xs + i + k;
+      double f0, f1, f2, f3, wv;
+      f0 = (double)w[i] * (double)bx[0];
+      wv = (double)w[0x7f - i] * (double)bx[0x80];
+      f1 = f0 - wv; f0 = f0 + wv;
+      f2 = (double)w[i + 0x40] * (double)bx[0x40];
+      wv = (double)w[0x3f - i] * (double)bx[0xc0];
+      f3 = f2 - wv; f2 = f2 + wv;
+      wsh[b][FHT_PAD(x + 0)] = f0 + f2; wsh[b][FHT_PAD(x + 2)] = f0 - f2; wsh[b][FHT_PAD(x + 1)] = f1 + f3; wsh[b][FHT_PAD(x + 3)] = f1 - f3;
+      f0 = (double)w[i + 0x01] * (double)bx[0x01];
+      wv = (double)w[0x7e - i] * (double)bx[0x81];
+      f1 = f0 - wv; f0 = f0 + wv;
+      f2 = (double)w[i + 0x41] * (double)bx[0x41];
+      wv = (double)w[0x3e - i] * (double)bx[0xc1];
+      f3 = f2 - wv; f2 = f2 + wv;
+      wsh[b][FHT_PAD(x + 128 + 0)] = f0 + f2; wsh[b][FHT_PAD(x + 128 + 2)] = f0 - f2; wsh[b][FHT_PAD(x + 128 + 1)] = f1 + f3; wsh[b][FHT_PAD(x + 128 + 3)] = f1 - f3;
+    }
+    __syncthreads();
+#pragma unroll
+    for (int stage = 0; stage < 3; stage++) {
+      for (int q = tid; q < 96; q += PSY_THREADS) fht_task(wsh[q >> 5], stage, q & 31, T->tw, T->tw_off);
+      __syncthreads();
+    }
+    for (int q = tid; q < 3 * 128; q += PSY_THREADS) {
+      const int b = q >> 7, j = q & 127;
+      const double re = wsh[b][FHT_PAD(128 - j)], im = wsh[b][FHT_PAD(128 + j)];
+      fes[b][128 - j] = (re * re + im * im) * 0.5;
+    }
+    if (tid < 3) { f32s t0; t0 = (double)wsh[tid][0]; t0 *= (double)t0; fes[tid][0] = (double)t0; }
+    __syncthreads();
+    for (int q = tid; q < 3 * MP3_CBANDS; q += PSY_THREADS) {
+      const int sb = q >> 6, b = q & 63;
+      if (b < nps) {
+        double ebb = 0;
+        const int l0 = T->line0_s[b], l1 = T->line0_s[b + 1];
+        for (int j = l0; j < l1; j++) ebb += (double)fes[sb][j];
+        s_ebs[sb][b] = ebb;
+        o->eb_s[sb][b] = (float)ebb;
+      }
+    }
+    __syncthreads();
+    for (int q = tid; q < 3 * MP3_CBANDS; q += PSY_THREADS) {
+      const int sb = q >> 6, b = q & 63;
+      if (b < nps) {
+        int kk = T->s3lo_s[b];
+        int j = T->s3off_s[b];
+        double ecb = (double)T->s3_ss[j++] * (double)s_ebs[sb][kk];
+        ++kk;
+        while (kk <= T->s3hi_s[b]) { ecb += (double)T->s3_ss[j] * (double)s_ebs[sb][kk]; ++j; ++kk; }
+        o->ecb_s[sb][b] = ecb;
+      }
+    }
+    __syncthreads();
   }
 }
 
@@ -579,7 +639,8 @@
 
 __global__ void __launch_bounds__(MASK_THREADS)
 k_psy_masking(const Mp3Tables* __restrict__ T, const StreamDesc* __restrict__ streams, const PsyUnit* __restrict__ psy,
-              const signed char* __restrict__ bt_prev, const double* __restrict__ ath_psy, PsyRatioDev* __restrict__ ratio) {
+              const PsyShort* __restrict__ psy_s, const signed char* __restrict__ bt_prev, const signed char* __restrict__ bt_final,
+              int all_short, const double* __restrict__ ath_psy, PsyRatioDev* __restrict__ ratio) {
   const int z = blockIdx.z;
   const StreamDesc& sd = streams[z];
   const int u = (int)blockIdx.x - 1;
@@ -603,7 +664,9 @@
   __shared__ PsyRatioDev s_out[2];
   const int npl = T->npart_l, nps = T->npart_s;
   const PsyUnit* pu = (ch < nch) ? psy + psy_row(sd, z, u) * nch + ch : nullptr;
-  const PsyUnit* pp = (ch < nch) ? psy + psy_row(sd, z, u - 1) * nch + ch : nullptr;
+  const PsyShort* ps = (ch < nch) ? psy_s + psy_row(sd, z, u) * nch + ch : nullptr;
+  const PsyShort* pp = (ch < nch) ? psy_s + psy_row(sd, z, u - 1) * nch + ch : nullptr;
+  const bool short_read = psy_short_read(T, sd, bt_final, u, all_short);
   const double ath_adjust = ath_psy[sd.frame_base + u / T->mode_gr];
 
   if (ch < nch) {
@@ -621,11 +684,11 @@
       s_eb[ch][b] = (double)pu->eb_l[b];
     } else { s_thr[ch][b] = 0.0; s_eb[ch][b] = 0.0; }
     const int prev_short = bt_prev[(size_t)(sd.unit_base + u) * 2 + ch] == BT_SHORT;
-    for (int sb = 0; sb < 3; sb++) {
+    for (int sb = 0; short_read && sb < 3; sb++) {
       if (b < nps) {
-        const double ecb = pu->ecb_s[sb][b];
-        const float nb1 = sb >= 1 ? (float)pu->ecb_s[sb - 1][b] : (float)pp->ecb_s[2][b];
-        const float nb2 = sb == 2 ? (float)pu->ecb_s[0][b] : (sb == 1 ? (float)pp->ecb_s[2][b] : (float)pp->ecb_s[1][b]);
+        const double ecb = ps->ecb_s[sb][b];
+        const float nb1 = sb >= 1 ? (float)ps->ecb_s[sb - 1][b] : (float)pp->ecb_s[2][b];
+        const float nb2 = sb == 2 ? (float)ps->ecb_s[0][b] : (sb == 1 ? (float)pp->ecb_s[2][b] : (float)pp->ecb_s[1][b]);
         f32s t;
         t = js_dmin(ecb, 2 * (double)nb1);
         if (prev_short) { const double x = 16 * (double)nb2, y = (double)t; t = js_dmin(x, y); }
@@ -658,7 +721,7 @@
         thm[sbi] += w_curr * (double)s_thr[ch][bd];
       }
     }
-  } else if (ch < nch && b >= 22 && b < 22 + 39) {
+  } else if (short_read && ch < nch && b >= 22 && b < 22 + 39) {
     const int q = b - 22, sbi = q / 3, sblock = q - 3 * sbi;
     f32s(*en)[3] = reinterpret_cast<f32s(*)[3]>(s_out[ch].en_s);
     f32s(*thm)[3] = reinterpret_cast<f32s(*)[3]>(s_out[ch].thm_s);
@@ -668,16 +731,16 @@
       double enn = 0.0, thmm = 0.0;
       if (init >= 0) {
         const double w_next = 1.0 - (double)T->bo_s_weight[sbi - 1];
-        enn = w_next * (double)pu->eb_s[sblock][init];
+        enn = w_next * (double)ps->eb_s[sblock][init];
         thmm = w_next * (double)s_thr_s[ch][sblock][init];
       }
       const int p1 = T->conv_s.end[sbi];
-      for (int p = T->conv_s.start[sbi]; p < p1; p++) { enn += (double)pu->eb_s[sblock][p]; thmm += (double)s_thr_s[ch][sblock][p]; }
+      for (int p = T->conv_s.start[sbi]; p < p1; p++) { enn += (double)ps->eb_s[sblock][p]; thmm += (double)s_thr_s[ch][sblock][p]; }
       en[sbi][sblock] = enn; thm[sbi][sblock] = thmm;
       const int bd = T->conv_s.bound[sbi];
       if (bd >= 0) {
         const double w_curr = (double)T->bo_s_weight[sbi];
-        en[sbi][sblock] += w_curr * (double)pu->eb_s[sblock][bd];
+        en[sbi][sblock] += w_curr * (double)ps->eb_s[sblock][bd];
         thm[sbi][sblock] += w_curr * (double)s_thr_s[ch][sblock][bd];
       }
     }
@@ -689,7 +752,7 @@
     thm[sbi][sblock] = t;
   }
   __syncthreads();
-  if (nch == 2 && T->interch_ratio > 0.0 && tid < 22 + 39) {
+  if (nch == 2 && T->interch_ratio > 0.0 && tid < (short_read ? 22 + 39 : 22)) {
     const double r = T->interch_ratio;
     f32s* t0 = reinterpret_cast<f32s*>(tid < 22 ? &s_out[0].thm_l[tid] : &s_out[0].thm_s[0][0] + (tid - 22));
     f32s* t1 = reinterpret_cast<f32s*>(tid < 22 ? &s_out[1].thm_l[tid] : &s_out[1].thm_s[0][0] + (tid - 22));
@@ -698,7 +761,8 @@
     *t1 += l * r;
   }
   __syncthreads();
-  for (int i = tid; i < nch * 122; i += MASK_THREADS) (&out[0].en_l[0])[i] = (&s_out[0].en_l[0])[i];
+  for (int i = tid; i < nch * 122; i += MASK_THREADS)
+    if (short_read || i % 122 < 44) (&out[0].en_l[0])[i] = (&s_out[0].en_l[0])[i];
   if (sd.halo_out && u == T->mode_gr * sd.nframes - 1)
     for (int i = tid; i < nch * 122; i += MASK_THREADS) sd.halo_out[i] = (&s_out[0].en_l[0])[i];
 }
diff --git a/lamejs_b200/csrc/mp3_encoder.cu b/lamejs_b200/csrc/mp3_encoder.cu
--- a/lamejs_b200/csrc/mp3_encoder.cu
+++ b/lamejs_b200/csrc/mp3_encoder.cu
@@ -185,6 +185,9 @@
   Buf<float> xr;
   Buf<float> slab;
   Buf<PsyUnit> psy;
+  Buf<PsyShort> psy_s;
+  Buf<int2> short_list;
+  Buf<int> short_count;
   Buf<ScanIn> scan_in;
   Buf<PsyRatioDev> ratio;
   Buf<double> ath_psy;
@@ -207,7 +210,8 @@
   int fit(int S, int nch, long long U, long long F) {
     const size_t gc = (size_t)U * nch, rows = (size_t)(U + S) * nch, f = (size_t)F + 1;
     const bool failed = streams.fit(S) || bt_final.fit((size_t)U * 2 + 16) || bt_prev.fit((size_t)U * 2 + 16) ||
-                        xr.fit(gc * 576) || slab.fit(rows * 576) || psy.fit(rows) || scan_in.fit(rows) || ratio.fit(rows) ||
+                        xr.fit(gc * 576) || slab.fit(rows * 576) || psy.fit(rows) || psy_s.fit(rows) || short_list.fit(rows) ||
+                        short_count.fit(2) || scan_in.fit(rows) || ratio.fit(rows) ||
                         ath_psy.fit(f) || ath_q.fit(f) || qstate.fit(f) || ginfo.fit(gc) || l3enc.fit(gc * 576) ||
                         xrq.fit(gc * 576) || xrpow.fit(gc * 576) || neg.fit(gc * 18) || prep.fit(gc) || dirty.fit(3 * f) ||
                         counter.fit(Q_NCOUNTERS) || scan.fit((size_t)(F / SCAN_FRAMES + S + 1));
@@ -218,7 +222,8 @@
            refusals.cap;
   }
   void release() {
-    streams.release(); bt_final.release(); bt_prev.release(); xr.release(); slab.release(); psy.release(); scan_in.release();
+    streams.release(); bt_final.release(); bt_prev.release(); xr.release(); slab.release(); psy.release(); psy_s.release(); short_list.release();
+    short_count.release(); scan_in.release();
     ratio.release(); ath_psy.release(); ath_q.release(); qstate.release(); ginfo.release(); l3enc.release(); xrq.release();
     xrpow.release(); neg.release(); prep.release(); dirty.release(); counter.release(); scan.release();
     rs_desc.release(); rs_y.release(); st_desc.release(); st_y.release(); refusals.release();
@@ -382,6 +387,7 @@
 struct LaunchOpts {
   const int32_t* force_bt = nullptr;
   bool stop_after_mdct = false;
+  bool all_short = false;
   const PcmArrival* arrival = nullptr;
   float* timings_ms = nullptr;
   bool sync = true;
@@ -529,8 +535,23 @@
     CK(cudaStreamSynchronize(st));
   }
   {
+    CK(cudaMemsetAsync(ws.short_count.p, 0, 2 * sizeof(int), st));
+    dim3 grid((cfg->host.mode_gr * max_frames + 1 + 127) / 128, S);
+    k_psy_short_list<<<grid, 128, 0, st>>>(tab, ws.streams.p, ws.bt_final.p, o.all_short ? 1 : 0, ws.short_list.p, ws.short_count.p);
+    DBG("k_psy_short_list");
+    int sms = 132;
+    CK(cudaDeviceGetAttribute(&sms, cudaDevAttrMultiProcessorCount, c.device));
+    const long long tasks = ((long long)cfg->host.mode_gr * total_frames + S) * nch;
+    const int blocks = (int)std::min<long long>(std::max<long long>(tasks, 1), (long long)sms * PSY_SHORT_BLOCKS);
+    if (f32_pcm) k_psy_short<true><<<blocks, PSY_THREADS, 0, st>>>(tab, ws.streams.p, ws.psy_s.p, ws.short_list.p, ws.short_count.p);
+    else k_psy_short<false><<<blocks, PSY_THREADS, 0, st>>>(tab, ws.streams.p, ws.psy_s.p, ws.short_list.p, ws.short_count.p);
+    g_launches += 2;
+    DBG("k_psy_short");
+  }
+  {
     dim3 grid(cfg->host.mode_gr * max_frames + 1, 1, S);
-    k_psy_masking<<<grid, MASK_THREADS, 0, st>>>(tab, ws.streams.p, ws.psy.p, ws.bt_prev.p, ws.ath_psy.p, ws.ratio.p);
+    k_psy_masking<<<grid, MASK_THREADS, 0, st>>>(tab, ws.streams.p, ws.psy.p, ws.psy_s.p, ws.bt_prev.p, ws.bt_final.p,
+                                                 o.all_short ? 1 : 0, ws.ath_psy.p, ws.ratio.p);
     g_launches++;
     DBG("k_psy_masking");
   }
@@ -1016,6 +1037,13 @@
 }
 #endif
 int64_t mp3b200_launch_count(void) { return g_launches; }
+int64_t mp3b200_debug_short_units(void) {
+  if (!t_ctx.ws.short_count.p) return -1;
+  int n = 0;
+  CK(cudaMemcpyAsync(&n, t_ctx.ws.short_count.p, sizeof n, cudaMemcpyDeviceToHost, t_ctx.st));
+  CK(cudaStreamSynchronize(t_ctx.st));
+  return n;
+}
 
 int mp3b200_set_device(int device) {
   int n = 0;
@@ -1262,7 +1290,7 @@
   uint8_t* bytes_out = tp->bytes_out;
   const int64_t bytes_cap = tp->bytes_cap;
   Config* cfg;
-  int rc = get_config(channels, tp->samplerate, tp->kbps, tp->flags, &cfg);
+  int rc = get_config(channels, tp->samplerate, tp->kbps, tp->flags & ~MP3B200_DEBUG_SKIP_SHORT, &cfg);
   if (rc || (rc = check_input(cfg, 1, &left, &right, &nsamples))) return rc;
   if (!right) right = left;
   const int nch = cfg->host.nch;
@@ -1284,6 +1312,7 @@
   LaunchOpts opts;
   opts.f32_in = std::is_same_v<T, float>;
   opts.force_bt = force_blocktype;
+  opts.all_short = !(tp->flags & MP3B200_DEBUG_SKIP_SHORT);
   opts.stop_after_mdct = !(l3_enc || bytes_out || want_gi || want_prep || want_q);
   rc = launch_streams(t_ctx, cfg, sds, d_out, opts);
   auto fetch = [](void* dst, const void* src, size_t bytes) {
diff --git a/lamejs_b200/encoder.py b/lamejs_b200/encoder.py
--- a/lamejs_b200/encoder.py
+++ b/lamejs_b200/encoder.py
@@ -827,7 +827,17 @@
     return y
 
 
-def debug_stages(channels, samplerate, kbps, left, right=None, force_blocktype=None, want=("xr",), resample=False):
+DEBUG_SKIP_SHORT = 0x10000
+
+
+def debug_short_units():
+    f = lib().mp3b200_debug_short_units
+    f.restype = ctypes.c_int64
+    return f()
+
+
+def debug_stages(channels, samplerate, kbps, left, right=None, force_blocktype=None, want=("xr",), resample=False,
+                 skip_short=False):
     L = lib()
     (left,), (right,), f32 = _rows([left], [None if channels == 1 else right])
     n = len(left)
@@ -869,7 +879,7 @@
                   xmin=alloc("xmin", (F, G, nch, 39), np.float32), max_nonzero_coeff=alloc("max_nonzero_coeff", (F, G, nch), np.int32),
                   xrpow_max=alloc("xrpow_max", (F, G, nch), np.float64), scfsi=alloc("scfsi", (F, nch, 4), np.int32),
                   old_value=alloc("old_value", (F, 3, nch), np.int32), cur_step=alloc("cur_step", (F, 3, nch), np.int32),
-                  flags=RESAMPLE if resample else 0)
+                  flags=(RESAMPLE if resample else 0) | (DEBUG_SKIP_SHORT if skip_short else 0))
     if f32:
         _check(L.mp3b200_debug_stages_f32(ctypes.byref(t), left.ctypes.data, right.ctypes.data))
     else:
```

Result: faster. 58120 (median of 6 runs) (+7.8%).
